# da03/torch-Attention-OCR

Hardware: AMD Instinct MI355X
Metric: image-lines/sec (train step) (higher is better)
Workload: dtype bf16; 1 GPU; c3: 32x256 crops, batch 256/GPU, VGG-7 + BiLSTM(256) + 2-layer attn decoder, L=24; global_batch=256, per_gpu_batch=256, img=32x256, decoder_steps=24, parallelism=dp1, input_feed=True

## Files before the change

torch-attention-ocr_amd/csrc/capi.hip:

```cpp
#include <cmath>
#include <cstdarg>
#include <cstdio>
#include <cstring>
#include <new>
#include <string>
#include "model.h"

using namespace aocr;

static thread_local std::string g_err;
static int fail(const char* fmt, ...) {
  char buf[512]; va_list ap; va_start(ap, fmt); vsnprintf(buf, sizeof buf, fmt, ap); va_end(ap);
  g_err = buf; return 1;
}
static int check_launch(const char* what) {
  hipError_t e = hipGetLastError();
  if (e != hipSuccess) return fail("%s: %s", what, hipGetErrorString(e));
  return 0;
}
#define REQUIRE(cond, ...) do { if (!(cond)) return fail(__VA_ARGS__); } while (0)

static int check_cfg(const aocr_config* c) {
  REQUIRE(c, "config is NULL");
  REQUIRE(c->batch_size >= 1 && c->img_h >= 32 && c->img_h % 16 == 0, "bad batch_size/img_h");
// ... 269 lines not shown
  REQUIRE(m, "NULL model");
  REQUIRE(bucket >= 0 && bucket < AOCR_GRAD_BUCKETS, "bucket %d outside 0..%d", bucket, AOCR_GRAD_BUCKETS - 1);
  REQUIRE(m->last_valid, "no train step has been enqueued yet");
  if (hipStreamWaitEvent((hipStream_t)stream, m->grad_ev[bucket], 0) != hipSuccess) return fail("hipStreamWaitEvent failed");
  return 0;
}

int aocr_sgd_step(aocr_model* m, float lr, float clip, float* norms_dev) {
  REQUIRE(m, "NULL model");
  prof_mark(m, AOCR_PROF_SGD);
  sgd_clip_update(m->s, m->params, m->grads, m->layout.group_off, lr, clip, norms_dev, m->sgd_scratch, m->cl_err, m->bn_snap ? m->bn_state : nullptr, m->bn_snap, (int)aocr_bn_state_count());
  prof_mark(m, -1);
  return check_launch("aocr_sgd_step");
}

int aocr_adadelta_step(aocr_model* m, float rho, float eps, float weight_decay, float* state_dev) {
  REQUIRE(m && state_dev, "NULL argument");
  REQUIRE(rho >= 0.f && rho < 1.f && eps > 0.f, "rho=%g eps=%g out of range", rho, eps);
  const int64_t n = m->layout.group_off[AOCR_NUM_GROUPS];
  adadelta_update(m->s, m->params, m->grads, state_dev, state_dev + n, n, rho, eps, weight_decay, m->cl_err, m->bn_snap ? m->bn_state : nullptr, m->bn_snap, (int)aocr_bn_state_count());
  return check_launch("aocr_adadelta_step");
}

int aocr_forward_logits(aocr_model* m, const float* images_dev, const int32_t* targets_dev, const int32_t* targets_eval_dev,
                        int32_t B, int32_t W, int32_t L, int32_t training, float* logits_dev, float* loss_dev) {
  Dims d; if (step_dims(m, B, W, L, d)) return 1;
  REQUIRE(images_dev && targets_dev, "NULL input");
  m->tab_valid = false;
  cnn_forward(m, images_dev, d, training, 0);
  encoder_forward(m, d);
  decoder_tf_forward(m, d, targets_dev, 1, L, false);
  if (targets_eval_dev) loss_and_dlogits(m, d, targets_eval_dev, 1, L, 0.f, false, loss_dev);
  if (logits_dev) copy2d(m->s, m->logits, LOGIT_LD, logits_dev, m->V, L * B, m->V);
  m->last = d; m->last_valid = 1; m->last_train = false;
  return check_launch("aocr_forward_logits");
}

__global__ void pad_targets_kernel(const int32_t* src, int32_t* dst, int B, int L, int Lt) {
  int i = blockIdx.x * blockDim.x + threadIdx.x;
  if (i >= B * Lt) return;
  int b = i / Lt, t = i - b * Lt;
  dst[i] = t < L ? src[b * L + t] : 1;
}

int aocr_decode(aocr_model* m, const float* images_dev, const int32_t* targets_dev, const int32_t* targets_eval_dev, int32_t B,
                int32_t W, int32_t L, int32_t beam, int32_t* labels_dev, float* scores_dev, float* gold_scores_dev, float* loss_dev) {
  return aocr_decode_dict(m, images_dev, targets_dev, targets_eval_dev, B, W, L, beam, nullptr, labels_dev, scores_dev, gold_scores_dev,
                          loss_dev);
}
static int check_trie(const aocr_trie* t, int V) {
  REQUIRE(t->child_mask_dev && t->child_base_dev && (t->child_dev || t->n_edges == 0), "trie: NULL array");
  REQUIRE(t->n_nodes >= 1 && t->n_edges >= 0, "trie: n_nodes=%d n_edges=%d", t->n_nodes, t->n_edges);
  REQUIRE(V <= 64, "dictionary decoding needs target_vocab_size <= 64 (got %d)", V);
  return 0;
}
int aocr_decode_dict(aocr_model* m, const float* images_dev, const int32_t* targets_dev, const int32_t* targets_eval_dev, int32_t B,
                     int32_t W, int32_t L, int32_t beam, const aocr_trie* trie, int32_t* labels_dev, float* scores_dev,
                     float* gold_scores_dev, float* loss_dev) {
  Dims d; if (step_dims(m, B, W, L, d)) return 1;
  REQUIRE(images_dev && targets_dev && targets_eval_dev && labels_dev && scores_dev, "NULL argument");
  if (trie && check_trie(trie, m->V)) return 1;
  if (beam > m->V) beam = m->V;
  REQUIRE(beam >= 1 && beam <= m->cfg.max_beam, "beam=%d outside 1..%d", beam, m->cfg.max_beam);
  const int Lt = m->cfg.max_decoder_l;
  hipLaunchKernelGGL(pad_targets_kernel, dim3(cdiv((int64_t)B * Lt, 256)), dim3(256), 0, m->s, targets_dev, m->tgt_pad, B, L, Lt);
  hipLaunchKernelGGL(pad_targets_kernel, dim3(cdiv((int64_t)B * Lt, 256)), dim3(256), 0, m->s, targets_eval_dev, m->tge_pad, B, L, Lt);
  d.L = Lt;
  prof_mark(m, AOCR_PROF_OTHER);
  m->tab_valid = false;
  cnn_forward(m, images_dev, d, 0, 0);
  encoder_forward(m, d);
  prof_mark(m, AOCR_PROF_DECODE);
  decode_beam(m, d, m->tgt_pad, beam, labels_dev, scores_dev, trie);
  d.L = L < Lt ? L : Lt;
  decoder_tf_forward(m, d, m->tgt_pad, 1, Lt, false);
  prof_mark(m, AOCR_PROF_OTHER);
  loss_and_dlogits(m, d, m->tge_pad, 1, Lt, 0.f, false, loss_dev);
  if (gold_scores_dev) gold_scores(m->s, m->nll_rows, gold_scores_dev, d.L, B);
  prof_mark(m, -1);
  m->last = d; m->last_valid = 1; m->last_train = false; m->tab_valid = false;
  return check_launch(trie ? "aocr_decode_dict" : "aocr_decode");
}

int aocr_recognize(aocr_model* m, const float* images_dev, int32_t B, int32_t W, int32_t beam, const aocr_trie* trie, int32_t* labels_dev,
                   float* scores_dev, float* char_logp_dev, float* attn_dev) {
  REQUIRE(m, "NULL model");
  const int Lt = m->cfg.max_decoder_l;
  Dims d; if (step_dims(m, B, W, Lt, d)) return 1;
  REQUIRE(images_dev && labels_dev && scores_dev, "NULL argument");
  if (trie && check_trie(trie, m->V)) return 1;
  if (beam > m->V) beam = m->V;
  REQUIRE(beam >= 1 && beam <= m->cfg.max_beam, "beam=%d outside 1..%d", beam, m->cfg.max_beam);
  const bool hist = char_logp_dev || attn_dev;
  fill_i32(m->s, m->tgt_pad, 2, (int64_t)B * Lt);
  prof_mark(m, AOCR_PROF_OTHER);
  m->tab_valid = false;
  cnn_forward(m, images_dev, d, 0, 0);
  encoder_forward(m, d);
  prof_mark(m, AOCR_PROF_DECODE);
  decode_beam(m, d, m->tgt_pad, beam, labels_dev, scores_dev, trie, hist ? m->attn_hist : nullptr, hist ? m->sc_hist : nullptr);
  if (hist) {
    const bool greedy = beam == 1;
    recognize_gather(m->s, labels_dev, greedy ? nullptr : m->hist_par, greedy ? nullptr : m->beam_scores, m->sc_hist, m->attn_hist, char_logp_dev,
                     attn_dev, Lt, B, beam, d.T);
  }
  prof_mark(m, -1);
  m->ctxa_fresh = false;
  m->last = d; m->last_valid = 1; m->last_train = false; m->tab_valid = false;
  return check_launch("aocr_recognize");
}

int aocr_get_tensor(aocr_model* m, const char* name, const void** ptr_dev, int32_t* ndim, int64_t shape[4]) {
  REQUIRE(m && name && ptr_dev && ndim && shape, "NULL argument");
  REQUIRE(m->last_valid, "no step has run yet");
  const Dims& d = m->last; std::string n = name;
  for (int i = 0; i < 4; ++i) shape[i] = 1;
  if (n == "feats") { *ptr_dev = m->X; *ndim = 3; shape[0] = d.T; shape[1] = d.B; shape[2] = 512; }
  else if (n == "dfeats") { *ptr_dev = m->dX; *ndim = 3; shape[0] = d.T; shape[1] = d.B; shape[2] = 512; }
  else if (n == "context") { *ptr_dev = m->context; *ndim = 3; shape[0] = d.B; shape[1] = d.T; shape[2] = m->Hd; }
  else if (n == "dcontext") { *ptr_dev = m->dctx; *ndim = 3; shape[0] = d.B; shape[1] = d.T; shape[2] = m->Hd; }
  else if (n == "logits") { *ptr_dev = m->logits; *ndim = 3; shape[0] = d.L; shape[1] = d.B; shape[2] = LOGIT_LD; }
  else if (n == "dlogits") { *ptr_dev = m->dlogits; *ndim = 3; shape[0] = d.L; shape[1] = d.B; shape[2] = LOGIT_LD; }
  else if (n == "dout_proj") { *ptr_dev = m->dout_proj; *ndim = 3; shape[0] = d.L; shape[1] = d.B; shape[2] = m->Hd; }
  else if (n == "outs") { *ptr_dev = m->out_all + (size_t)d.B * m->Hd; *ndim = 3; shape[0] = d.L; shape[1] = d.B; shape[2] = m->Hd; }
  else if (n == "conv1") { if (m->bf16) bf16_to_f32(m->s, m->A1b, m->A1, (int64_t)d.B * d.H1 * d.W1 * 64); *ptr_dev = m->A1; *ndim = 4; shape[0] = d.B; shape[1] = d.H1; shape[2] = d.W1; shape[3] = 64; }
  else if (n == "conv2") { if (m->bf16) bf16_to_f32(m->s, m->A2b, m->A2, (int64_t)d.B * d.H2 * d.W2 * 128); *ptr_dev = m->A2; *ndim = 4; shape[0] = d.B; shape[1] = d.H2; shape[2] = d.W2; shape[3] = 128; }
  else if (n == "conv6") { if (m->bf16) bf16_to_f32(m->s, m->A6b, m->A6, (int64_t)d.B * d.H6 * d.W2 * 512); *ptr_dev = m->A6; *ndim = 4; shape[0] = d.B; shape[1] = d.H6; shape[2] = d.W2; shape[3] = 512; }
  else if (n == "conv3") { if (m->bf16) bf16_to_f32(m->s, m->A3b, m->A3, (int64_t)d.B * d.H2 * d.W2 * 256); *ptr_dev = m->A3; *ndim = 4; shape[0] = d.B; shape[1] = d.H2; shape[2] = d.W2; shape[3] = 256; }
  else if (n == "conv4") { if (m->bf16) bf16_to_f32(m->s, m->A4b, m->A4, (int64_t)d.B * d.H4 * d.W2 * 256); *ptr_dev = m->A4; *ndim = 4; shape[0] = d.B; shape[1] = d.H4; shape[2] = d.W2; shape[3] = 256; }
  else if (n == "conv5") { if (m->bf16) bf16_to_f32(m->s, m->A5b, m->A5, (int64_t)d.B * d.H4 * d.W2 * 512); *ptr_dev = m->A5; *ndim = 4; shape[0] = d.B; shape[1] = d.H4; shape[2] = d.W2; shape[3] = 512; }
  else if (n == "idx2") { u8_to_f32(m->s, m->idx2, m->G0, (int64_t)d.B * d.H2 * d.W2 * 128); *ptr_dev = m->G0; *ndim = 4; shape[0] = d.B; shape[1] = d.H2; shape[2] = d.W2; shape[3] = 128; }
  else if (n == "idx4") { u8_to_f32(m->s, m->idx4, m->G0, (int64_t)d.B * d.H4 * d.W2 * 256); *ptr_dev = m->G0; *ndim = 4; shape[0] = d.B; shape[1] = d.H4; shape[2] = d.W2; shape[3] = 256; }
  else if (n == "idx6") { u8_to_f32(m->s, m->idx6, m->G0, (int64_t)d.B * d.H6 * d.W2 * 512); *ptr_dev = m->G0; *ndim = 4; shape[0] = d.B; shape[1] = d.H6; shape[2] = d.W2; shape[3] = 512; }
  else if (n == "enc_dz0" || n == "enc_dz1") {
    const int dir = n == "enc_dz1"; const int64_t cnt = (int64_t)d.T * d.B * 4 * m->He;
    REQUIRE(m->edz_b[dir][m->Le - 1], "no bf16 d z in this mode");
    bf16_to_f32(m->s, m->edz_b[dir][m->Le - 1], m->G0, cnt);
    *ptr_dev = m->G0; *ndim = 3; shape[0] = d.T; shape[1] = d.B; shape[2] = 4 * m->He;
  }
  else if (n == "enc_cs0") { *ptr_dev = m->ecs[0][m->Le - 1]; *ndim = 3; shape[0] = d.T + 2; shape[1] = d.B; shape[2] = m->He; }
  else if (n == "enc_gates0") { *ptr_dev = m->egates[0][m->Le - 1]; *ndim = 3; shape[0] = d.T; shape[1] = d.B; shape[2] = 4 * m->He; }
  else if (n == "cl_err") { *ptr_dev = m->cl_err; *ndim = 1; shape[0] = 8; REQUIRE(m->cl_err, "no cluster kernels in this configuration"); }
  else if (n == "dc_stamps") { REQUIRE(m->dc_xtab, "no decoder cluster kernel in this configuration"); *ptr_dev = m->dc_xtab + (size_t)((d.B + 31) / 32) * 32; *ndim = 1; shape[0] = 32; }
  else if (n == "ds_all") { *ptr_dev = m->ds_all; *ndim = 3; shape[0] = d.L; shape[1] = d.B; shape[2] = d.T; }
  else if (n == "dq_all") { *ptr_dev = m->dq_all; *ndim = 3; shape[0] = d.L; shape[1] = d.B; shape[2] = m->Hd; }
  else if (n == "dcat_all") { *ptr_dev = m->dcat_all; *ndim = 3; shape[0] = d.L; shape[1] = d.B; shape[2] = 2 * m->Hd; }
  else if (n == "dh_rec0" || n == "dh_rec1" || n == "dc_st0" || n == "dc_st1" || n == "dfeed0") {
    const int l = n.back() - '0'; *ptr_dev = n[1] == 'f' ? m->dfeed : (n[1] == 'h' ? m->dh_rec[l] : m->dc_st[l]); *ndim = 2; shape[0] = d.B; shape[1] = m->Hd; }
  else if (n == "dpre_all") { *ptr_dev = m->dpre_all; *ndim = 3; shape[0] = d.L; shape[1] = d.B; shape[2] = m->Hd; }
  else if (n == "dc_bstamps") { REQUIRE(m->dc_xtab, "no decoder cluster kernel in this configuration"); *ptr_dev = m->dc_xtab + (size_t)((d.B + 31) / 32) * 32 + 16; *ndim = 1; shape[0] = 32; }
  else if (n == "dc_times") { REQUIRE(m->cl_err, "no cluster kernels in this configuration"); *ptr_dev = m->cl_err + 16 + 2048; *ndim = 1; shape[0] = 32 * 4 * 16 * 2; }
  else if (n == "g0") {
    const char* e = getenv("AOCR_DBG_STOP"); const int stop = e ? atoi(e) : 0;
    const int64_t cnt = stop == 1 ? (int64_t)d.B * d.T * 512 : (int64_t)d.B * d.H4 * d.W2 * 512;
    if (m->bf16) bf16_to_f32(m->s, m->G0b, m->G0, cnt);
    *ptr_dev = m->G0; *ndim = 4; shape[0] = d.B; shape[1] = stop == 1 ? d.Ho7 : d.H4; shape[2] = stop == 1 ? d.Wo7 : d.W2; shape[3] = 512;
  }
  else return fail("unknown tensor '%s'", name);
  return 0;
}

int aocr_profile_kernel(aocr_model* m, int32_t which, int32_t iters, float* ms_per_launch, double* flops_per_launch) {
  REQUIRE(m && ms_per_launch && flops_per_launch, "NULL argument");
  REQUIRE(m->last_valid, "run a step first");
  REQUIRE(which >= 0 && which <= AOCR_PK_LAST, "unknown kernel id %d", which);
  REQUIRE(iters >= 1, "iters must be >= 1");
  REQUIRE(which < 2 || (m->bf16 && m->last_images && m->last_train), "the HBM-bound kernel ids replay the bf16 TRAINING step: run aocr_train_forward_backward in bf16 mode first");
  const Dims& d = m->last;
  const int64_t n5 = (int64_t)d.B * d.H4 * d.W2;
  REQUIRE((which != 1 && which != AOCR_PK_SPLITK) || (size_t)512 * 4608 <= m->gmax, "kernel id %d sums conv6's filter gradient (512 x 4608 floats) into the gradient-map scratch, which holds %zu floats in this configuration", which, m->gmax);
  REQUIRE((which != AOCR_PK_BN_FWD && which != AOCR_PK_BN_BWD && which != AOCR_PK_UNPOOL) || (n5 % 256 == 0 && n5 / 256 <= 512), "kernel id %d replays conv5's BatchNorm with the epilogue's 256-pixel statistics chunks: %lld pixels are not a multiple of 256 / more than 512 chunks", which, (long long)n5);
  hipEvent_t e0, e1; hipEventCreate(&e0); hipEventCreate(&e1);
  hipStream_t s = m->s; const int B = d.B;
  constexpr size_t SLAB = (size_t)4 << 20;
  double bytes = 0.0;
  const char* const nd = getenv("AOCR_DX16");
  const bool dx16 = (nd && nd[0] == '1') && !getenv("AOCR_BN_PARTIAL_OLD") && !getenv("AOCR_UNPOOL4") && !getenv("AOCR_HALO8") && B * d.H4 * d.W2 % 256 == 0;
  const bf16_t* const g1h = dx16 ? reinterpret_cast<const bf16_t*>(m->G1) : nullptr;
  const double dab = dx16 ? 2.0 : 4.0;
  auto run = [&]() {
    switch (which) {
    case 0:
      if (const char* const pl = getenv("AOCR_PROBE_LAYER")) {
        int bnc = 0, y16 = 0; const int l = atoi(pl);
        if (l == 3) { conv_forward(m->s, m->bf16, m->A2, m->conv[3].w, m->conv[3].b, m->Y3, nullptr, d.B, d.H2, d.W2, 128, 256, 3, 1, 0, 0, m->A2b, m->wb[3], nullptr, 1, nullptr, nullptr, nullptr, (double*)m->bn_scratch, &bnc, &y16); break; }
        if (l == 4) { conv_forward(m->s, m->bf16, m->A3, m->conv[4].w, m->conv[4].b, nullptr, m->idx4, d.B, d.H2, d.W2, 256, 256, 3, 1, 1, 2, m->A3b, m->wb[4], m->A4b, 1); break; }
        if (l == 5) { conv_forward(m->s, m->bf16, m->A4, m->conv[5].w, m->conv[5].b, m->Y5, nullptr, d.B, d.H4, d.W2, 256, 512, 3, 1, 0, 0, m->A4b, m->wb[5], nullptr, 1, nullptr, nullptr, nullptr, (double*)m->bn_scratch, &bnc, &y16); break; }
      }
      conv_forward(m->s, m->bf16, m->A5, m->conv[6].w, m->conv[6].b, m->bf16 ? nullptr : m->A6, m->idx6, d.B, d.H4, d.W2, 512, 512, 3, 1, 1, 2, m->A5b, m->wb[6],
                   m->A6b, 1);
      break;
    case 1:
      conv_backward_filter(m->s, m->bf16, m->A5, m->G0, m->G1, nullptr, d.B, d.H4, d.W2, 512, 512, 3, 1, m->A5b, m->G0b, m->wg_part, m->wg_part_floats, 1);
      break;
    case AOCR_PK_CONV1_FWD:
      conv1_forward(s, m->last_images, m->conv[1].w, m->conv[1].b, nullptr, B, d.H, d.W, m->A1b, m->route1_valid ? m->route1 : nullptr);
      bytes = (double)B * d.H * d.W * 4 + (double)B * d.H1 * d.W1 * 64 * 2 + (m->route1_valid ? (double)conv1_route_elems(B, d.H, d.W) * 2 : 0.0);
      break;
    case AOCR_PK_CONV1_BWD:
      conv1_backward(s, m->last_images, m->conv[1].w, m->conv[1].b, m->G1, m->conv[1].dw, m->conv[1].db, B, d.H, d.W,
                     (size_t)B * d.H1 * d.W1 * 128 >= (size_t)4096 * 640 ? m->G0 + 6 * SLAB : nullptr, nullptr, m->route1_valid ? m->route1 : nullptr);
      bytes = (double)B * d.H * d.W * 4 + (double)B * d.H1 * d.W1 * 64 * 4 + (m->route1_valid ? (double)conv1_route_elems(B, d.H, d.W) * 2 : 0.0);
      break;
    case AOCR_PK_BN_FWD:
      bn_relu_forward(s, m->Y5, nullptr, m->bn[5].w, m->bn[5].b, m->bn[5].rm, m->bn[5].rv, m->bn[5].save, m->bn_scratch, n5, 512, 1, 0, 0, m->A5b, nullptr, (int)(n5 / 256));
      bytes = (double)n5 * 512 * (4 + 2);
      break;
    case AOCR_PK_BN_BWD:
      bn_relu_backward(s, m->Y5, m->A5, m->G1, m->bn[5].w, m->bn[5].save, nullptr, m->bn[5].dw, m->bn[5].db, m->bn_scratch, n5, 512, 0, m->G0b, m->A5b,
                       m->conv[5].db, m->G0 + 2 * SLAB, nullptr, nullptr, nullptr, g1h);
      bytes = (double)n5 * 512 * ((4 + dab + 2) + (4 + dab + 2 + 2));
      break;
    case AOCR_PK_UNPOOL:
      unpool_relu_backward(s, m->G1, m->A6, m->idx6, nullptr, B, d.H4, d.W2, 512, 2, m->G0b, m->conv[6].db, m->G0 + 1 * SLAB, m->A6b, nullptr, g1h);
      bytes = (double)B * d.H6 * d.W2 * 512 * (dab + 1 + 2) + (double)n5 * 512 * 2;
      break;
    case AOCR_PK_ATTN_DCTX:
      attention_dctx(s, m->a_all, m->ds_all, m->dcat_all, 2 * m->Hd, m->q_all, m->dctx, d.L, B, d.T, m->Hd);
      bytes = (double)d.L * B * (2.0 * d.T + 2.0 * m->Hd) * 4 + (double)B * d.T * m->Hd * 4;
      break;
    case AOCR_PK_SPLITK:
      {
        const int ksl = (int)std::min<size_t>(8, m->wg_part_floats / ((size_t)512 * 4608));
        if (ksl >= 1) splitk_reduce(s, m->wg_part, ksl, (size_t)512 * 4608, m->G1);
        bytes = (double)512 * 4608 * 4 * (ksl + 2);
      }
      break;
    }
  };
  run();
  hipEventRecord(e0, m->s);
  for (int i = 0; i < iters; ++i) run();
  hipEventRecord(e1, m->s);
  hipEventSynchronize(e1);
  float ms = 0.f; hipEventElapsedTime(&ms, e0, e1);
  hipEventDestroy(e0); hipEventDestroy(e1);
  *ms_per_launch = ms / iters;
  if (which == 0 && getenv("AOCR_PROBE")) {
    unsigned long long pr[8] = {0}; kprobe_read(pr);
    if (getenv("AOCR_PROBE_LAYER")) for (int k = 1; k >= 0; --k) if (pr[4 * k + 1]) fprintf(stderr, "[aocr] probe: workgroup %d of the tagged launch: start -> K loop %.1f us, K loop %.1f us (%llu cycles = %.2f GHz), whole workgroup (last store acknowledged) %.1f us\n", k ? 17 : 300, pr[4 * k + 2] / 100.0, pr[4 * k + 1] / 100.0, pr[4 * k], pr[4 * k] / (pr[4 * k + 1] * 10.0) , pr[4 * k + 3] / 100.0);
    for (int k = 0; k < 2; ++k) if (pr[4 * k + 1]) fprintf(stderr, "[aocr] probe (%s halo kernel, conv6 forward): K loop of one workgroup %llu shader cycles in %.1f us = %.2f GHz\n", k ? "4-wave" : "8-wave", pr[4 * k], pr[4 * k + 1] / 100.0, pr[4 * k] / (pr[4 * k + 1] * 10.0)), fprintf(stderr, "[aocr]   prologue %.1f us, whole workgroup %.1f us (stores acknowledged)\n", pr[4 * k + 2] / 100.0, pr[4 * k + 3] / 100.0);
  }
  *flops_per_launch = which < 2 ? 2.0 * (double)d.B * d.H4 * d.W2 * 512.0 * (9.0 * 512.0) : bytes;
  return check_launch("aocr_profile_kernel");
}

int aocr_gemm(void* stream, int32_t compute, const float* A_dev, int64_t lda, int32_t a_kmajor, const float* B_dev, int64_t ldb,
              int32_t b_kmajor, float* C_dev, int64_t ldc, int32_t M, int32_t N, int32_t K, const float* bias_dev, int32_t accumulate) {
  REQUIRE(A_dev && B_dev && C_dev && M >= 0 && N >= 0 && K >= 0, "bad gemm arguments");
  REQUIRE((accumulate & ~7) == 0, "unknown gemm flag bits %d", accumulate);
  const int fl = ((accumulate & AOCR_GEMM_ACCUMULATE) ? EP_ACCUM : 0) | ((accumulate & AOCR_GEMM_RELU) ? EP_RELU : 0) | ((accumulate & AOCR_GEMM_TANH) ? EP_TANH : 0);
  REQUIRE(!((fl & EP_ACCUM) && (fl & (EP_RELU | EP_TANH))), "an activation on an accumulating product is not a module of the path");
  int rc = gemm((hipStream_t)stream, compute == AOCR_COMPUTE_BF16, A_dev, lda, a_kmajor != 0, B_dev, ldb, b_kmajor != 0, C_dev, ldc,
                M, N, K, bias_dev, nullptr, fl);
  REQUIRE(rc == 0, "gemm: the (A column-major, B row-major-by-K) combination is not supported");
  return check_launch("aocr_gemm");
}
int aocr_pointwise(void* stream, int32_t op, const float* a_dev, const float* b_dev, float* y_dev, int64_t n) {
  REQUIRE(a_dev && y_dev && n >= 0 && op >= 0 && op <= 3 && (b_dev || op == AOCR_PW_RELU), "bad arguments");
  pointwise((hipStream_t)stream, op, a_dev, b_dev, y_dev, n);
  return check_launch("aocr_pointwise");
}
int aocr_lookup_forward(void* stream, const float* weight_dev, const int32_t* ids_dev, float* out_dev, int32_t n, int32_t E) {
  REQUIRE(weight_dev && ids_dev && out_dev && n >= 0 && E > 0, "bad arguments");
  embedding_gather((hipStream_t)stream, weight_dev, ids_dev, 0, 1, out_dev, 1, n, E);
  return check_launch("aocr_lookup_forward");
}
int aocr_lookup_backward(void* stream, const float* grad_out_dev, const int32_t* ids_dev, float* grad_weight_dev, int32_t n, int32_t E, int32_t V) {
  REQUIRE(grad_out_dev && ids_dev && grad_weight_dev && n >= 0 && E > 0 && E <= 256 && V > 0, "bad arguments");
  embedding_scatter_accum((hipStream_t)stream, grad_out_dev, ids_dev, 0, 1, grad_weight_dev, 1, n, E, V);
  return check_launch("aocr_lookup_backward");
}
int aocr_conv2d_forward(void* stream, int32_t compute, const float* x_dev, const float* w_dev, const float* bias_dev, float* y_dev,
                        uint8_t* idx_dev, int32_t B, int32_t H, int32_t W, int32_t Cin, int32_t Cout, int32_t ksize, int32_t pad,
                        int32_t relu, int32_t pool) {
  REQUIRE(x_dev && w_dev && y_dev, "NULL argument");
  REQUIRE(Cin % 16 == 0 && Cout % 16 == 0, "Cin and Cout must be multiples of 16 (the 1-channel first layer has its own entry point)");
  REQUIRE(pool >= 0 && pool <= 2 && (pool == 0 || idx_dev), "bad pool mode / missing idx");
  conv_forward((hipStream_t)stream, compute == AOCR_COMPUTE_BF16, x_dev, w_dev, bias_dev, y_dev, idx_dev, B, H, W, Cin, Cout, ksize, pad,
               relu, pool);
  return check_launch("aocr_conv2d_forward");
}
int aocr_conv2d_backward_data(void* stream, int32_t compute, const float* dy_dev, const float* w_dev, float* dx_dev, int32_t B, int32_t H,
                              int32_t W, int32_t Cin, int32_t Cout, int32_t ksize, int32_t pad) {
  REQUIRE(dy_dev && w_dev && dx_dev && Cin % 16 == 0 && Cout % 16 == 0, "bad arguments");
  conv_backward_data((hipStream_t)stream, compute == AOCR_COMPUTE_BF16, dy_dev, w_dev, dx_dev, B, H, W, Cin, Cout, ksize, pad);
  return check_launch("aocr_conv2d_backward_data");
}
int aocr_conv2d_backward_filter(void* stream, int32_t compute, const float* x_dev, const float* dy_dev, float* dw_dev, float* dbias_dev,
                                int32_t B, int32_t H, int32_t W, int32_t Cin, int32_t Cout, int32_t ksize, int32_t pad) {
  REQUIRE(x_dev && dy_dev && dw_dev && Cin % 16 == 0 && Cout % 16 == 0, "bad arguments");
  conv_backward_filter((hipStream_t)stream, compute == AOCR_COMPUTE_BF16, x_dev, dy_dev, dw_dev, dbias_dev, B, H, W, Cin, Cout, ksize, pad);
  return check_launch("aocr_conv2d_backward_filter");
}
int aocr_unpool_relu_backward(void* stream, const float* dpooled_dev, const float* pooled_dev, const uint8_t* idx_dev, float* dy_dev,
                              int32_t B, int32_t Ho, int32_t Wo, int32_t C, int32_t pool) {
  REQUIRE(dpooled_dev && pooled_dev && idx_dev && dy_dev && (pool == 1 || pool == 2) && C % 4 == 0, "bad arguments");
  unpool_relu_backward((hipStream_t)stream, dpooled_dev, pooled_dev, idx_dev, dy_dev, B, Ho, Wo, C, pool);
  return check_launch("aocr_unpool_relu_backward");
}
int aocr_conv1_forward(void* stream, const float* x_dev, const float* w_dev, const float* bias_dev, float* y_dev, int32_t B, int32_t H,
                       int32_t W) {
  REQUIRE(x_dev && w_dev && bias_dev && y_dev, "NULL argument");
  conv1_forward((hipStream_t)stream, x_dev, w_dev, bias_dev, y_dev, B, H, W);
  return check_launch("aocr_conv1_forward");
}
int aocr_conv1_backward(void* stream, const float* x_dev, const float* w_dev, const float* bias_dev, const float* dy_pooled_dev,
                        float* dw_dev, float* dbias_dev, int32_t B, int32_t H, int32_t W) {
  REQUIRE(x_dev && w_dev && bias_dev && dy_pooled_dev && dw_dev && dbias_dev, "NULL argument");
// ... 160 lines not shown
```

torch-attention-ocr_amd/csrc/epilogues.h:

```cpp
#pragma once
#include "mfma_gemm.h"

namespace aocr {

enum : int { EP_RELU = 1, EP_TANH = 2, EP_ACCUM = 4, EP_ATOMIC = 8 };

__device__ __forceinline__ float fast_exp_(float x) { return __builtin_amdgcn_exp2f(x * 1.44269504088896341f); }
__device__ __forceinline__ float sigmoidf_(float x) { return __builtin_amdgcn_rcpf(1.f + fast_exp_(-x)); }
__device__ __forceinline__ float tanhf_(float x) {
  const float ax = fminf(fabsf(x), 15.f);
  const float e = fast_exp_(2.f * ax);
  const float t = 1.f - 2.f * __builtin_amdgcn_rcpf(e + 1.f);
  return copysignf(t, x);
}

__host__ __device__ __forceinline__ unsigned long long splitmix64_(unsigned long long x) {
  x += 0x9E3779B97F4A7C15ull;
  unsigned long long z = x;
  z = (z ^ (z >> 30)) * 0xBF58476D1CE4E5B9ull;
  z = (z ^ (z >> 27)) * 0x94D049BB133111EBull;
  return z ^ (z >> 31);
}
struct DropSpec {
  unsigned long long base = 0, thr = 0; float scale = 1.f; long long off = 0;
  __device__ __forceinline__ bool on() const { return thr != 0; }
  __device__ __forceinline__ float mask(long long idx) const { return ((splitmix64_(base + (unsigned long long)(off + idx)) >> 11) >= thr) ? scale : 0.f; }
};

struct EpStore {
  float* C; int64_t ldc; int M, N;
  const float* bias; const float* bias2;
  int flags;
  float* C1; int64_t ldc1; int N0;
  bf16_t* Cb = nullptr; int64_t ldcb = 0;
  const float* dg = nullptr; const float* dout = nullptr; int64_t ldd = 0;
  const float* bnb_x = nullptr; const bf16_t* bnb_yb = nullptr; const float* bnb_save = nullptr; double* bnb_part = nullptr;
  template <int NT> __device__ __forceinline__ void quad(int m, int n, int nstep, const float (&v)[NT][4]) const {
#pragma unroll
    for (int ni = 0; ni < NT; ++ni) {
      int col = n + nstep * ni;
      if (col >= N) continue;
      float bb = 0.f;
      if (bias) bb = bias[col];
      if (bias2) bb += bias2[col];
      float* base; int64_t ld; int cc;
      if (C1 && col >= N0) { base = C1; ld = ldc1; cc = col - N0; } else { base = C; ld = ldc; cc = col; }
#pragma unroll
      for (int i = 0; i < 4; ++i) {
        int row = m + i;
        if (row >= M) continue;
        float x = v[ni][i] + bb;
        if (flags & EP_RELU) x = fmaxf(x, 0.f);
        if (flags & EP_TANH) x = tanhf_(x);
        if (dg) { const float o = dout[(int64_t)row * ldd + col]; x = (x + dg[(int64_t)row * ldd + col]) * (1.f - o * o); }
        float* p = base + (int64_t)row * ld + cc;
        if (flags & EP_ATOMIC) atomicAdd(p, x);
        else if (flags & EP_ACCUM) *p += x;
        else { *p = x; if (Cb && base == C) Cb[(int64_t)row * ldcb + cc] = (bf16_t)x; }
      }
    }
  }
  struct Pre { float dg, dout, b, b2, old; };
  __device__ __forceinline__ Pre prefetch(int row, int n) const {
    Pre p; p.dg = p.dout = p.b = p.b2 = p.old = 0.f;
    const int rr = max(min(row, M - 1), 0), col = min(n, N - 1);
    if (bias) p.b = bias[col];
    if (bias2) p.b2 = bias2[col];
    if (dg) { p.dg = dg[(int64_t)rr * ldd + col]; p.dout = dout[(int64_t)rr * ldd + col]; }
    if (flags & EP_ACCUM) p.old = *((C1 && col >= N0) ? C1 + (int64_t)rr * ldc1 + (col - N0) : C + (int64_t)rr * ldc + col);
    return p;
  }
  __device__ __forceinline__ void prefetch_zx(Pre&, int, int) const {}
  static constexpr bool kCell4 = false; struct Pre4 {};
  __device__ __forceinline__ bool cell4_ok() const { return false; }
  template <int NT> __device__ __forceinline__ void elem(int row, int n, int nstep, const float (&v)[NT], const Pre& pre) const {
    if (row >= M) return;
    if constexpr (NT == 1) {
      const int col = n;
      if (col >= N) return;
      float x = v[0];
      if (bias) x += pre.b;
      if (bias2) x += pre.b2;
      if (flags & EP_RELU) x = fmaxf(x, 0.f);
      if (flags & EP_TANH) x = tanhf_(x);
      if (dg) x = (x + pre.dg) * (1.f - pre.dout * pre.dout);
      float* p = (C1 && col >= N0) ? C1 + (int64_t)row * ldc1 + (col - N0) : C + (int64_t)row * ldc + col;
      if (flags & EP_ATOMIC) atomicAdd(p, x);
      else if (flags & EP_ACCUM) *p = pre.old + x;
      else { *p = x; if (Cb && !(C1 && col >= N0)) Cb[(int64_t)row * ldcb + col] = (bf16_t)x; }
      return;
    }
#pragma unroll
    for (int ni = 0; ni < NT; ++ni) {
      int col = n + nstep * ni;
      if (col >= N) continue;
      float x = v[ni];
      if (bias) x += bias[col];
      if (bias2) x += bias2[col];
      if (flags & EP_RELU) x = fmaxf(x, 0.f);
      if (flags & EP_TANH) x = tanhf_(x);
      if (dg) { const float o = dout[(int64_t)row * ldd + col]; x = (x + dg[(int64_t)row * ldd + col]) * (1.f - o * o); }
      float* p = (C1 && col >= N0) ? C1 + (int64_t)row * ldc1 + (col - N0) : C + (int64_t)row * ldc + col;
      if (flags & EP_ATOMIC) atomicAdd(p, x);
      else if (flags & EP_ACCUM) *p += x;
      else { *p = x; if (Cb && !(C1 && col >= N0)) Cb[(int64_t)row * ldcb + col] = (bf16_t)x; }
    }
  }
};

template <int NT, class EPT>
__device__ __forceinline__ bool narrow_store_staged(const EPT& ep, const f32x16 (&acc)[2][NT], unsigned char* lds, int m_blk, int n_blk, int wm, int wn, int r, int h, int tid) {
  constexpr int BN = 64 * NT, PITCH = BN * 4;
  if ((ep.flags & (EP_ATOMIC | EP_ACCUM)) || ep.C1 || ep.dg || n_blk + BN > ep.N) return false;
  float bb[NT];
#pragma unroll
  for (int ni = 0; ni < NT; ++ni) { const int col = n_blk + wn * 32 * NT + ni * 32 + r; bb[ni] = (ep.bias ? ep.bias[col] : 0.f) + (ep.bias2 ? ep.bias2[col] : 0.f); }
  __syncthreads();
  for (int p = 0; p < 2; ++p) {
    if ((wm >> 1) == p) {
#pragma unroll
      for (int mi = 0; mi < 2; ++mi)
#pragma unroll
        for (int ni = 0; ni < NT; ++ni)
#pragma unroll
          for (int q = 0; q < 4; ++q)
#pragma unroll
            for (int i = 0; i < 4; ++i) {
              float x = acc[mi][ni][4 * q + i] + bb[ni];
              if (ep.flags & EP_RELU) x = fmaxf(x, 0.f);
              if (ep.flags & EP_TANH) x = tanhf_(x);
              *reinterpret_cast<float*>(lds + ((wm & 1) * 64 + mi * 32 + 8 * q + 4 * h + i) * PITCH + (wn * 32 * NT + ni * 32 + r) * 4) = x;
            }
    }
    __syncthreads();
    const int row_base = m_blk + p * 128;
#pragma unroll 4
    for (int it = 0; it < (128 * BN / 4) / 512; ++it) {
      const int idx = it * 512 + tid, row = idx / (BN / 4), c = idx % (BN / 4);
      if (row_base + row < ep.M) {
        const float4 v = *reinterpret_cast<const float4*>(lds + row * PITCH + c * 16);
        if (ep.C) *reinterpret_cast<float4*>(ep.C + (int64_t)(row_base + row) * ep.ldc + n_blk + c * 4) = v;
        if (ep.Cb) {
          typedef __bf16 bf16x4_ __attribute__((ext_vector_type(4)));
          bf16x4_ o; o[0] = (__bf16)v.x; o[1] = (__bf16)v.y; o[2] = (__bf16)v.z; o[3] = (__bf16)v.w;
          *reinterpret_cast<bf16x4_*>(ep.Cb + (int64_t)(row_base + row) * ep.ldcb + n_blk + c * 4) = o;
        }
      }
    }
    __syncthreads();
  }
  return true;
}

struct EpConv {
  float* y; uint8_t* idx; const float* bias; int Cout; int rows; int pmode; int relu;
  bf16_t* yb;
  const float* bn_save = nullptr; const float* bn_w = nullptr; const float* bn_b = nullptr;
  double* bn_part = nullptr;
  bf16_t* y16 = nullptr;
  template <int NT> __device__ __forceinline__ void quad(int m, int n, int nstep, const float (&v)[NT][4]) const {
#pragma unroll
    for (int ni = 0; ni < NT; ++ni) {
      int col = n + nstep * ni;
      if (col >= Cout) continue;
      float bb = bias ? bias[col] : 0.f;
      float x[4];
#pragma unroll
      for (int i = 0; i < 4; ++i) { x[i] = v[ni][i] + bb; if (relu) x[i] = fmaxf(x[i], 0.f); }
      if (bn_save) {
        const float mu = bn_save[col], iv = bn_save[Cout + col], ww = bn_w[col], b2 = bn_b[col];
#pragma unroll
        for (int i = 0; i < 4; ++i) x[i] = fmaxf((x[i] - mu) * iv * ww + b2, 0.f);
      }
      if (pmode == 0) {
#pragma unroll
        for (int i = 0; i < 4; ++i) if (m + i < rows) {
          if (y) y[(int64_t)(m + i) * Cout + col] = x[i];
          if (yb) yb[(int64_t)(m + i) * Cout + col] = (bf16_t)x[i];
        }
      } else if (pmode == 1) {
        if (m < rows) {
          float best = x[0]; int bi = 0;
#pragma unroll
          for (int i = 1; i < 4; ++i) if (x[i] > best) { best = x[i]; bi = i; }
          int64_t o = (int64_t)(m >> 2) * Cout + col;
          if (y) y[o] = best;
          if (idx) idx[o] = (uint8_t)bi; if (yb) yb[o] = (bf16_t)best;
        }
      } else {
#pragma unroll
        for (int w = 0; w < 2; ++w) {
          int row = m + 2 * w;
          if (row < rows) {
            float a = x[2 * w], b = x[2 * w + 1];
            int64_t o = (int64_t)(row >> 1) * Cout + col;
            if (y) y[o] = (b > a) ? b : a;
            if (idx) idx[o] = (uint8_t)(b > a); if (yb) yb[o] = (bf16_t)((b > a) ? b : a);
          }
        }
      }
    }
  }
};

struct EpGatesFwd {
  const float* zx; int64_t ldzx;
  const float* b1; const float* b2;
  const float* c_prev; int64_t ldcp;
  float* c_out; int64_t ldc;
  float* h_out; int64_t ldh;
  float* h_out2; int64_t ldh2;
  float* gates; int64_t ldg;
  int M, H;
  bf16_t* hb = nullptr; int64_t ldhb = 0;
  bf16_t* hb2 = nullptr; int64_t ldhb2 = 0;
  const int32_t* zx_tok = nullptr; int64_t zx_tok_stride = 1;
  DropSpec drop;
  __device__ __forceinline__ int64_t zrow(int row) const { return zx_tok ? (int64_t)(zx_tok[(int64_t)row * zx_tok_stride] - 1) : (int64_t)row; }
  template <int NT> __device__ __forceinline__ void quad(int m, int j, int, const float (&v)[NT][4]) const {
    static_assert(NT == 4, "gate epilogue needs the 4 gate tiles");
    if (j >= H) return;
    float bb[4] = {0.f, 0.f, 0.f, 0.f};
    if (b1) {
#pragma unroll
      for (int g = 0; g < 4; ++g) bb[g] = b1[g * H + j] + b2[g * H + j];
    }
#pragma unroll
    for (int i = 0; i < 4; ++i) {
      int row = m + i;
      if (row >= M) continue;
      float z[4];
#pragma unroll
      for (int g = 0; g < 4; ++g) {
        z[g] = v[g][i] + bb[g];
        if (zx) z[g] += zx[zrow(row) * ldzx + g * H + j];
      }
      float ig = sigmoidf_(z[0]), fg = sigmoidf_(z[1]), og = sigmoidf_(z[2]), gg = tanhf_(z[3]);
      float c = fg * c_prev[(int64_t)row * ldcp + j] + ig * gg;
      float hh = og * tanhf_(c);
      c_out[(int64_t)row * ldc + j] = c;
      h_out[(int64_t)row * ldh + j] = hh;
      const float hh2 = drop.on() ? hh * drop.mask((long long)row * H + j) : hh;
      if (h_out2) h_out2[(int64_t)row * ldh2 + j] = hh2;
      if (hb) hb[(int64_t)row * ldhb + j] = (bf16_t)hh;
      if (hb2) hb2[(int64_t)row * ldhb2 + j] = (bf16_t)hh2;
      if (gates) {
        float* gp = gates + (int64_t)row * ldg + j;
        gp[0] = ig; gp[H] = fg; gp[2 * H] = og; gp[3 * H] = gg;
      }
    }
  }
  struct Pre { float zx[4]; float b1[4]; float b2[4]; float cp; int32_t tok; };
  __device__ __forceinline__ Pre prefetch(int row, int j) const {
    Pre p;
    const int rr = max(min(row, M - 1), 0), jj = min(j, H - 1);
    const float* const cpp = c_prev + (int64_t)rr * ldcp + jj;
    const int32_t* const tp = zx_tok ? zx_tok + (int64_t)rr * zx_tok_stride : reinterpret_cast<const int32_t*>(cpp);
    p.tok = *tp;
    const float* const b1p = b1 ? b1 + jj : cpp; const float* const b2p = b1 ? b2 + jj : cpp; const int bs = b1 ? H : 0;
#pragma unroll
    for (int g = 0; g < 4; ++g) { p.b1[g] = b1p[g * bs]; p.b2[g] = b2p[g * bs]; }
    p.cp = *cpp;
    return p;
  }
  __device__ __forceinline__ void prefetch_zx(Pre& p, int row, int j) const {
    const int rr = max(min(row, M - 1), 0), jj = min(j, H - 1);
    const float* const cpp = c_prev + (int64_t)rr * ldcp + jj;
    const int64_t zr = zx_tok ? (int64_t)(p.tok - 1) : (int64_t)rr;
    const float* const zp = zx ? zx + zr * ldzx + jj : cpp; const int zs = zx ? H : 0;
#pragma unroll
    for (int g = 0; g < 4; ++g) p.zx[g] = zp[g * zs];
  }
  template <int NT> __device__ __forceinline__ void elem(int row, int j, int, const float (&v)[NT], const Pre& pre) const {
    static_assert(NT == 4, "gate epilogue needs the 4 gate tiles");
    if (j >= H || row >= M) return;
    float z[4];
#pragma unroll
    for (int g = 0; g < 4; ++g) {
      float zin = 0.f;
      if (b1) zin = pre.b1[g] + pre.b2[g];
      if (zx) zin += pre.zx[g];
      z[g] = v[g] + zin;
    }
    float ig = sigmoidf_(z[0]), fg = sigmoidf_(z[1]), og = sigmoidf_(z[2]), gg = tanhf_(z[3]);
    float c = fg * pre.cp + ig * gg;
    float hh = og * tanhf_(c);
    c_out[(int64_t)row * ldc + j] = c;
    h_out[(int64_t)row * ldh + j] = hh;
    const float hh2 = drop.on() ? hh * drop.mask((long long)row * H + j) : hh;
    if (h_out2) h_out2[(int64_t)row * ldh2 + j] = hh2;
    if (hb) hb[(int64_t)row * ldhb + j] = (bf16_t)hh;
    if (hb2) hb2[(int64_t)row * ldhb2 + j] = (bf16_t)hh2;
    if (gates) {
      float* gp = gates + (int64_t)row * ldg + j;
      gp[0] = ig; gp[H] = fg; gp[2 * H] = og; gp[3 * H] = gg;
    }
  }
  static constexpr bool kCell4 = true;
  typedef float v4f __attribute__((ext_vector_type(4)));
  typedef bf16_t v4h __attribute__((ext_vector_type(4)));
  struct Pre4 { v4f zx[4]; v4f b1[4]; v4f b2[4]; v4f cp; int32_t tok; };
  __device__ __forceinline__ bool cell4_ok() const {
// ... 146 lines not shown
```

torch-attention-ocr_amd/csrc/mfma_gemm.h:

```cpp
#pragma once
#include <hip/hip_runtime.h>
#include <stdint.h>
#include <type_traits>
#include <utility>

namespace aocr {

typedef float f32x16 __attribute__((ext_vector_type(16)));
typedef float f32x4 __attribute__((ext_vector_type(4)));
typedef __bf16 bf16x8 __attribute__((ext_vector_type(8)));

template <int NV> struct Frag { float v[NV]; };

template <bool BF16> struct Mode {
  static constexpr int NV = BF16 ? 8 : 4;
  static constexpr int CHUNK = BF16 ? 16 : 8;
};


struct LoadK {
  const float* p0; int64_t ld0; int K0;
  const float* p1; int64_t ld1;
  int rows; int K; int vec;
  struct Ctx { const float* b0; const float* b1; bool ok; };
// ... 776 lines not shown
#pragma unroll
      for (int i = 0; i < NI; ++i) bf[set][i] = *reinterpret_cast<const float4*>(lb + i * 32 * PITCH + 32 * c);
    };
    rd(0, 0);
#pragma unroll
    for (int c = 0; c < 4; ++c) {
      if (c < 3) rd((c + 1) & 1, c + 1);
#pragma unroll
      for (int s = 0; s < 4; ++s)
#pragma unroll
        for (int mi = 0; mi < MI; ++mi)
#pragma unroll
          for (int ni = 0; ni < NI; ++ni) {
            const float4& A = af[c & 1][mi]; const float4& B = bf[c & 1][ni];
            const float x = s == 0 ? A.x : s == 1 ? A.y : s == 2 ? A.z : A.w;
            const float y = s == 0 ? B.x : s == 1 ? B.y : s == 2 ? B.z : B.w;
            acc[mi][ni] = __builtin_amdgcn_mfma_f32_32x32x2f32(x, y, acc[mi][ni], 0, 0, 0);
          }
    }
    if (kt + 1 < nk) { sa.store(&lds[buf ^ 1][0]); sb.store(&lds[buf ^ 1][BM * PITCH]); }
    __syncthreads();
  }
  const int m0 = m_blk + wm * (BM / 2), n0 = n_blk + wn * (BN / 2);
#pragma unroll
  for (int mi = 0; mi < MI; ++mi)
#pragma unroll
    for (int q = 0; q < 4; ++q) {
      float v[NI][4];
#pragma unroll
      for (int ni = 0; ni < NI; ++ni)
#pragma unroll
        for (int i = 0; i < 4; ++i) v[ni][i] = acc[mi][ni][4 * q + i];
      ep.template quad<NI>(m0 + 32 * mi + 8 * q + 4 * h, n0 + r, 32, v);
    }
}
constexpr int F32W_PITCH = 136 * 4;
template <class LD> struct StagerW;
template <> struct StagerW<LoadMN> {
  const float* pk; int64_t ld8; bool mok; int k; f32x4 reg[4]; bool ok[4];
  __device__ __forceinline__ void init(const LoadMN& l, int mbase, int tid, int kbeg) {
    const int m = mbase + 4 * (tid & 31); mok = m + 3 < l.rows; k = kbeg + (tid >> 5);
    pk = l.p + (mok ? m : 0) + (int64_t)k * l.ld; ld8 = 8 * l.ld;
  }
  __device__ __forceinline__ void load(const LoadMN& l) {
    const float* q = pk;
#pragma unroll
    for (int i = 0; i < 4; ++i) {
      ok[i] = mok && k + 8 * i < l.K;
      reg[i] = *reinterpret_cast<const f32x4*>(ok[i] ? q : l.p);
      q += ld8;
    }
    pk = q; k += 32;
  }
};
template <> struct StagerW<LoadConvXcol> {
  LoadConvXcol::Ctx4 c; int px, py, k, linc, cbase, dxc, dyc; f32x4 reg[4]; bool ok[4];
  __device__ __forceinline__ void init(const LoadConvXcol& l, int nbase, int tid, int kbeg) {
    c = l.row4(nbase + 4 * (tid & 31)); k = kbeg + (tid >> 5);
    px = k % l.Wo; const int t = k / l.Wo; py = t % l.Ho; const int b = t / l.Ho;
    linc = ((b * l.H + py) * l.W + px) * l.Cin; cbase = ((c.kh - l.pad) * l.W + (c.kw - l.pad)) * l.Cin + c.ci;
    dxc = (l.W - l.Wo) * l.Cin; dyc = (l.H - l.Ho) * l.W * l.Cin;
  }
  __device__ __forceinline__ void load(const LoadConvXcol& l) {
#pragma unroll
    for (int i = 0; i < 4; ++i) {
      const int sy = py + c.kh - l.pad, sx = px + c.kw - l.pad;
      ok[i] = c.ok && k < l.K && (unsigned)sy < (unsigned)l.H && (unsigned)sx < (unsigned)l.W;
      reg[i] = *reinterpret_cast<const f32x4*>(l.x + (ok[i] ? linc + cbase : 0));
      k += 8; px += 8; linc += 8 * l.Cin;
      const bool wx = px >= l.Wo; px -= wx ? l.Wo : 0; py += wx ? 1 : 0; linc += wx ? dxc : 0;
      const bool wy = py >= l.Ho; py = wy ? 0 : py; linc += wy ? dyc : 0;
    }
  }
};
template <class ST> __device__ __forceinline__ void stagerw_store(const ST& st, unsigned char* tile, int tid) {
  const f32x4 z = {0.f, 0.f, 0.f, 0.f};
#pragma unroll
  for (int i = 0; i < 4; ++i) *reinterpret_cast<f32x4*>(tile + ((tid >> 5) + 8 * i) * F32W_PITCH + (tid & 31) * 16) = st.ok[i] ? st.reg[i] : z;
}
template <class AL, class BL, class EP>
__global__ __launch_bounds__(256, 2) void gemm_f32w_kernel(AL a, BL b, EP ep, int K, int kper, int gx, int gy) {
  constexpr int PK = F32W_PITCH, OPB = 32 * PK;
  __shared__ __attribute__((aligned(16))) unsigned char lds[2][2 * OPB];
  const int nwg = gx * gy, orig = blockIdx.x;
  const int q8 = nwg >> 3, r8 = nwg & 7, xcd = orig & 7;
  const int bid = (xcd < r8 ? xcd * (q8 + 1) : r8 * (q8 + 1) + (xcd - r8) * q8) + (orig >> 3);
  const int m_blk = (bid / gx) * 128, n_blk = (bid % gx) * 128;
  const int kbeg = blockIdx.z * kper, kend = min(K, kbeg + kper);
  const int tid = threadIdx.x, lane = tid & 63, wave = tid >> 6;
  const int r = lane & 31, h = lane >> 5;
  const int wm = wave >> 1, wn = wave & 1;
  const int nk = (kend - kbeg + 31) / 32;
  StagerW<AL> sa; StagerW<BL> sb;
  sa.init(a, m_blk, tid, kbeg); sb.init(b, n_blk, tid, kbeg);
  f32x16 acc[2][2];
#pragma unroll
  for (int i = 0; i < 2; ++i)
#pragma unroll
    for (int j = 0; j < 2; ++j)
#pragma unroll
      for (int e = 0; e < 16; ++e) acc[i][j][e] = 0.f;
  if (nk > 0) { sa.load(a); sb.load(b); stagerw_store(sa, &lds[0][0], tid); stagerw_store(sb, &lds[0][OPB], tid); }
  __syncthreads();
  for (int kt = 0; kt < nk; ++kt) {
    const int buf = kt & 1;
    if (kt + 1 < nk) { sa.load(a); sb.load(b); }
    const unsigned char* la = &lds[buf][h * PK + (wm * 64 + r) * 4];
    const unsigned char* lb = &lds[buf][OPB + h * PK + (wn * 64 + r) * 4];
#pragma unroll
    for (int j = 0; j < 16; ++j) {
      float av[2], bv[2];
#pragma unroll
      for (int i = 0; i < 2; ++i) { av[i] = *reinterpret_cast<const float*>(la + 2 * j * PK + i * 128); bv[i] = *reinterpret_cast<const float*>(lb + 2 * j * PK + i * 128); }
#pragma unroll
      for (int mi = 0; mi < 2; ++mi)
#pragma unroll
        for (int ni = 0; ni < 2; ++ni) acc[mi][ni] = __builtin_amdgcn_mfma_f32_32x32x2f32(av[mi], bv[ni], acc[mi][ni], 0, 0, 0);
    }
    if (kt + 1 < nk) { stagerw_store(sa, &lds[buf ^ 1][0], tid); stagerw_store(sb, &lds[buf ^ 1][OPB], tid); }
    __syncthreads();
  }
  const int m0 = m_blk + wm * 64, n0 = n_blk + wn * 64;
#pragma unroll
  for (int mi = 0; mi < 2; ++mi)
#pragma unroll
    for (int q = 0; q < 4; ++q) {
      float v[2][4];
#pragma unroll
      for (int ni = 0; ni < 2; ++ni)
#pragma unroll
        for (int i = 0; i < 4; ++i) v[ni][i] = acc[mi][ni][4 * q + i];
      ep.template quad<2>(m0 + 32 * mi + 8 * q + 4 * h, n0 + r, 32, v);
    }
}
template <class L> struct HasStagerW { static constexpr bool v = false; };
template <> struct HasStagerW<LoadMN> { static constexpr bool v = true; };
template <> struct HasStagerW<LoadConvXcol> { static constexpr bool v = true; };

template <class L> struct HasPtr8 { static constexpr bool v = false; };
template <> struct HasPtr8<LoadK> { static constexpr bool v = true; };
template <> struct HasPtr8<LoadConvK> { static constexpr bool v = true; };

template <class AL, class BL, class EP, int BK = 32>
__global__ __launch_bounds__(256, (SrcBf16<AL>::v && SrcBf16<BL>::v) ? 4 : 1)
void gemm_lds_bf16_kernel(AL a, BL b, EP ep, int K, int kper, int gx, int gy) {
  __shared__ __attribute__((aligned(16))) unsigned char lds[2][2][128 * (BK * 2 + 16)];
  const int nwg = gx * gy, orig = blockIdx.x;
  const int q8 = nwg >> 3, r8 = nwg & 7, xcd = orig & 7;
  const int bid = (xcd < r8 ? xcd * (q8 + 1) : r8 * (q8 + 1) + (xcd - r8) * q8) + (orig >> 3);
  const int kbeg = blockIdx.z * kper;
  lds_tile<BK>(a, b, ep, (bid / gx) * 128, (bid % gx) * 128, kbeg, min(K, kbeg + kper), lds);
}

struct EpConv; struct EpStore;
template <int NI, int NTH>
__device__ __forceinline__ void tile256_store_f32(float* dst, int64_t ldc, const float* bias, bool relu, const f32x16 (&acc)[4][NI], unsigned char* lds,
                                                  int m_blk, int n_blk, int wm, int wn, int r, int h, int tid, double* part = nullptr, int C = 0, const float* bias2 = nullptr,
                                                  const float* bnb_x = nullptr, const bf16_t* bnb_yb = nullptr, const float* bnb_save = nullptr) {
  constexpr int PITCH = 1024;
  float bmean[4] = {0.f, 0.f, 0.f, 0.f}, binv[4] = {0.f, 0.f, 0.f, 0.f};
  if (bnb_x) {
    const float4 m4 = *reinterpret_cast<const float4*>(bnb_save + n_blk + (tid & 63) * 4), i4 = *reinterpret_cast<const float4*>(bnb_save + C + n_blk + (tid & 63) * 4);
    bmean[0] = m4.x; bmean[1] = m4.y; bmean[2] = m4.z; bmean[3] = m4.w; binv[0] = i4.x; binv[1] = i4.y; binv[2] = i4.z; binv[3] = i4.w;
  }
  float bb[NI];
#pragma unroll
  for (int ni = 0; ni < NI; ++ni) bb[ni] = (bias ? bias[n_blk + wn * 32 * NI + ni * 32 + r] : 0.f) + (bias2 ? bias2[n_blk + wn * 32 * NI + ni * 32 + r] : 0.f);
  float ps[8] = {0.f, 0.f, 0.f, 0.f, 0.f, 0.f, 0.f, 0.f};
  __syncthreads();
  for (int p = 0; p < 2; ++p) {
    if (wm == p) {
#pragma unroll
      for (int mi = 0; mi < 4; ++mi)
#pragma unroll
        for (int ni = 0; ni < NI; ++ni)
#pragma unroll
          for (int q = 0; q < 4; ++q)
#pragma unroll
            for (int i = 0; i < 4; ++i) {
              float x = acc[mi][ni][4 * q + i] + bb[ni];
              if (relu) x = fmaxf(x, 0.f);
              *reinterpret_cast<float*>(lds + (mi * 32 + 8 * q + 4 * h + i) * PITCH + (wn * 32 * NI + ni * 32 + r) * 4) = x;
            }
    }
    __syncthreads();
    float* const d0 = dst + (int64_t)(m_blk + p * 128) * ldc + n_blk;
#pragma unroll 4
    for (int it = 0; it < 8192 / NTH; ++it) {
      const int idx = it * NTH + tid, row = idx >> 6, c = idx & 63;
      const float4 v = *reinterpret_cast<const float4*>(lds + row * PITCH + c * 16);
      *reinterpret_cast<float4*>(d0 + (int64_t)row * ldc + c * 4) = v;
      if (part && bnb_x) {
        const int64_t gofs = (int64_t)(m_blk + p * 128 + row) * C + n_blk + c * 4;
        const float4 x4 = *reinterpret_cast<const float4*>(bnb_x + gofs);
        typedef __bf16 bf16x4_ __attribute__((ext_vector_type(4)));
        const bf16x4_ y4 = *reinterpret_cast<const bf16x4_*>(bnb_yb + gofs);
        const float dv[4] = {(float)y4[0] > 0.f ? v.x : 0.f, (float)y4[1] > 0.f ? v.y : 0.f, (float)y4[2] > 0.f ? v.z : 0.f, (float)y4[3] > 0.f ? v.w : 0.f};
        const float xs[4] = {x4.x, x4.y, x4.z, x4.w};
#pragma unroll
        for (int k = 0; k < 4; ++k) { ps[k] += dv[k]; ps[4 + k] = fmaf(dv[k], (xs[k] - bmean[k]) * binv[k], ps[4 + k]); }
      } else if (part) {
        ps[0] += v.x; ps[1] += v.y; ps[2] += v.z; ps[3] += v.w;
        ps[4] = fmaf(v.x, v.x, ps[4]); ps[5] = fmaf(v.y, v.y, ps[5]); ps[6] = fmaf(v.z, v.z, ps[6]); ps[7] = fmaf(v.w, v.w, ps[7]);
      }
    }
    __syncthreads();
  }
  if (part) {
    float* const red = reinterpret_cast<float*>(lds);
#pragma unroll
    for (int k = 0; k < 8; ++k) red[((tid >> 6) * 64 + (tid & 63)) * 8 + k] = ps[k];
    __syncthreads();
    if (tid < 64) {
      double S[8] = {0, 0, 0, 0, 0, 0, 0, 0};
      for (int g = 0; g < NTH / 64; ++g)
#pragma unroll
        for (int k = 0; k < 8; ++k) S[k] += (double)red[(g * 64 + tid) * 8 + k];
      double* o = part + ((int64_t)(m_blk >> 8) * C + n_blk + tid * 4) * 2;
#pragma unroll
      for (int j = 0; j < 4; ++j) { o[2 * j] = S[j]; o[2 * j + 1] = S[4 + j]; }
    }
  }
}
template <int NI, int NTH>
__device__ __forceinline__ void tile256_store_pooled(bf16_t* yb, uint8_t* idxp, int Cout, const float* bias, bool relu, const f32x16 (&acc)[4][NI], unsigned char* lds,
                                                     int m_blk, int n_blk, int wm, int wn, int r, int h, int tid) {
  constexpr int PB = 528, PI = 272, IOFF = 128 * PB;
  float bb[NI];
#pragma unroll
  for (int ni = 0; ni < NI; ++ni) bb[ni] = bias ? bias[n_blk + wn * 32 * NI + ni * 32 + r] : 0.f;
  __syncthreads();
#pragma unroll
  for (int mi = 0; mi < 4; ++mi)
#pragma unroll
    for (int ni = 0; ni < NI; ++ni)
#pragma unroll
      for (int q = 0; q < 4; ++q) {
        float x[4];
#pragma unroll
        for (int i = 0; i < 4; ++i) { x[i] = acc[mi][ni][4 * q + i] + bb[ni]; if (relu) x[i] = fmaxf(x[i], 0.f); }
#pragma unroll
        for (int w = 0; w < 2; ++w) {
          const float a_ = x[2 * w], b_ = x[2 * w + 1];
          const int prow = wm * 64 + mi * 16 + 4 * q + 2 * h + w, col = wn * 32 * NI + ni * 32 + r;
          *reinterpret_cast<bf16_t*>(lds + prow * PB + col * 2) = (bf16_t)((b_ > a_) ? b_ : a_);
          *reinterpret_cast<uint8_t*>(lds + IOFF + prow * PI + col) = (uint8_t)(b_ > a_);
        }
      }
  __syncthreads();
  const int64_t prow0 = m_blk >> 1;
#pragma unroll 4
  for (int it = 0; it < 4096 / NTH; ++it) {
    const int idx = it * NTH + tid, row = idx >> 5, c = idx & 31;
    const uint4 v = *reinterpret_cast<const uint4*>(lds + row * PB + c * 16);
    *reinterpret_cast<uint4*>(yb + (prow0 + row) * Cout + n_blk + c * 8) = v;
  }
#pragma unroll 4
  for (int it = 0; it < 2048 / NTH; ++it) {
    const int idx = it * NTH + tid, row = idx >> 4, c = idx & 15;
    const uint4 v = *reinterpret_cast<const uint4*>(lds + IOFF + row * PI + c * 16);
    *reinterpret_cast<uint4*>(idxp + (prow0 + row) * Cout + n_blk + c * 16) = v;
  }
}
template <int NI, int NTH>
__device__ __forceinline__ void tile256_store_bf16(bf16_t* yb, int Cout, const float* bias, bool relu, const float* bn_save, const float* bn_w, const float* bn_b,
                                                   const f32x16 (&acc)[4][NI], unsigned char* lds, int m_blk, int n_blk, int wm, int wn, int r, int h, int tid, double* part = nullptr) {
  float bb[NI], mu[NI], iv[NI], ww[NI], b2[NI];
#pragma unroll
  for (int ni = 0; ni < NI; ++ni) {
    const int col = n_blk + wn * 32 * NI + ni * 32 + r;
    bb[ni] = bias ? bias[col] : 0.f;
    mu[ni] = bn_save ? bn_save[col] : 0.f; iv[ni] = bn_save ? bn_save[Cout + col] : 1.f; ww[ni] = bn_save ? bn_w[col] : 1.f; b2[ni] = bn_save ? bn_b[col] : 0.f;
  }
  float ps[NI], pss[NI];
#pragma unroll
  for (int ni = 0; ni < NI; ++ni) { ps[ni] = 0.f; pss[ni] = 0.f; }
  __syncthreads();
#pragma unroll
  for (int mi = 0; mi < 4; ++mi)
#pragma unroll
    for (int ni = 0; ni < NI; ++ni)
#pragma unroll
      for (int q = 0; q < 4; ++q)
#pragma unroll
        for (int i = 0; i < 4; ++i) {
          float x = acc[mi][ni][4 * q + i] + bb[ni];
          if (relu) x = fmaxf(x, 0.f);
          if (bn_save) x = fmaxf((x - mu[ni]) * iv[ni] * ww[ni] + b2[ni], 0.f);
          ps[ni] += x; pss[ni] = fmaf(x, x, pss[ni]);
          *reinterpret_cast<bf16_t*>(lds + (wm * 128 + mi * 32 + 8 * q + 4 * h + i) * 512 + (wn * 32 * NI + ni * 32 + r) * 2) = (bf16_t)x;
        }
  __syncthreads();
#pragma unroll 4
  for (int it = 0; it < 8192 / NTH; ++it) {
    const int idx = it * NTH + tid, row = idx >> 5, c = idx & 31;
    const uint4 v = *reinterpret_cast<const uint4*>(lds + row * 512 + c * 16);
    *reinterpret_cast<uint4*>(yb + (int64_t)(m_blk + row) * Cout + n_blk + c * 8) = v;
  }
  if (part) {
    __syncthreads();
    float* const red = reinterpret_cast<float*>(lds);
#pragma unroll
    for (int ni = 0; ni < NI; ++ni) {
      float* o = red + (((wm * 2 + h) * 256) + wn * 32 * NI + ni * 32 + r) * 2;
      o[0] = ps[ni]; o[1] = pss[ni];
    }
    __syncthreads();
    if (tid < 256) {
      double S = 0.0, SS = 0.0;
#pragma unroll
      for (int g = 0; g < 4; ++g) { S += (double)red[((g * 256) + tid) * 2]; SS += (double)red[((g * 256) + tid) * 2 + 1]; }
      double* o = part + ((int64_t)(m_blk >> 8) * Cout + n_blk + tid) * 2;
      o[0] = S; o[1] = SS;
    }
  }
}
template <int NI, int NTH, class EP>
__device__ __forceinline__ bool tile256_store_staged(const EP& ep, const f32x16 (&acc)[4][NI], unsigned char* lds, int m_blk, int n_blk, int wm, int wn, int r, int h, int tid, int opt) {
  if constexpr (std::is_same<EP, EpConv>::value) {
    if (m_blk + 256 > ep.rows || n_blk + 256 > ep.Cout) return false;
    if (ep.pmode == 0 && ep.y16 && ep.bn_part && !ep.yb && !ep.bn_save && (opt & 2)) {
      tile256_store_bf16<NI, NTH>(ep.y16, ep.Cout, ep.bias, ep.relu != 0, nullptr, nullptr, nullptr, acc, lds, m_blk, n_blk, wm, wn, r, h, tid, ep.bn_part); return true; }
    if (ep.pmode == 0 && ep.yb && !ep.y && (opt & 2)) { tile256_store_bf16<NI, NTH>(ep.yb, ep.Cout, ep.bias, ep.relu != 0, ep.bn_save, ep.bn_w, ep.bn_b, acc, lds, m_blk, n_blk, wm, wn, r, h, tid); return true; }
    if (ep.bn_save) return false;
    if (ep.pmode == 2 && ep.yb && ep.idx && !ep.y && (opt & 4)) { tile256_store_pooled<NI, NTH>(ep.yb, ep.idx, ep.Cout, ep.bias, ep.relu != 0, acc, lds, m_blk, n_blk, wm, wn, r, h, tid); return true; }
    if (ep.pmode == 0 && ep.y && !ep.yb && (opt & 2)) { tile256_store_f32<NI, NTH>(ep.y, ep.Cout, ep.bias, ep.relu != 0, acc, lds, m_blk, n_blk, wm, wn, r, h, tid, ep.bn_part, ep.Cout); return true; }
    return false;
  } else if constexpr (std::is_same<EP, EpStore>::value) {
    if (!ep.C && ep.Cb && !ep.flags && !ep.bias && !ep.bias2 && !ep.C1 && !ep.dg) {
      tile256_store_bf16<NI, NTH>(ep.Cb, (int)ep.ldcb, nullptr, false, nullptr, nullptr, nullptr, acc, lds, m_blk, n_blk, wm, wn, r, h, tid); return true; }
    if (ep.flags || ep.bias || ep.bias2 || ep.C1 || ep.Cb || ep.dg || !(opt & 1) || m_blk + 256 > ep.M || n_blk + 256 > ep.N) return false;
    if (ep.bnb_part) tile256_store_f32<NI, NTH>(ep.C, ep.ldc, nullptr, false, acc, lds, m_blk, n_blk, wm, wn, r, h, tid, ep.bnb_part, ep.N, nullptr, ep.bnb_x, ep.bnb_yb, ep.bnb_save);
    else tile256_store_f32<NI, NTH>(ep.C, ep.ldc, nullptr, false, acc, lds, m_blk, n_blk, wm, wn, r, h, tid);
    return true;
  } else return false;
}

template <int NT, class EPT>
__device__ __forceinline__ bool narrow_store_staged(const EPT& ep, const f32x16 (&acc)[2][NT], unsigned char* lds, int m_blk, int n_blk, int wm, int wn, int r, int h, int tid);

__device__ __forceinline__ void dma16(const void* g, unsigned char* l) {
  __builtin_amdgcn_global_load_lds((const __attribute__((address_space(1))) void*)g, (__attribute__((address_space(3))) void*)l, 16, 0, 0);
}

template <class AL, class BL, class EP, int ABL = 0, bool PIPE = false, bool PAIRS = false, int TAG = 0>
__global__ __launch_bounds__(512, 1)
void gemm_dma_bf16_kernel(AL a, BL b, EP ep, int K, int gx, int gy, const bf16_t* zero, int opt = 0) {
  __shared__ __attribute__((aligned(1024))) unsigned char lds[4 * 32768];
  const int nwg = gx * gy, orig = blockIdx.x;
  const int q8 = nwg >> 3, r8 = nwg & 7, xcd = orig & 7;
  const int bid = (xcd < r8 ? xcd * (q8 + 1) : r8 * (q8 + 1) + (xcd - r8) * q8) + (orig >> 3);
  const int m_blk = (bid / gx) * 256, n_blk = (bid % gx) * 256;
  const int tid = threadIdx.x, lane = tid & 63, wave = tid >> 6;
  const int r = lane & 31, h = lane >> 5, wm = wave >> 2, wn = wave & 3;

  const int srow = tid >> 2, chunk = (tid & 3) ^ ((tid >> 4) & 3);
  typename AL::DRow ra[2]; typename BL::DRow rb[2];
#pragma unroll
  for (int j = 0; j < 2; ++j) { ra[j] = a.drow(m_blk + 128 * j + srow, chunk); rb[j] = b.drow(n_blk + 128 * j + srow, chunk); }
  typename AL::DCur ca = a.dseek(0); typename BL::DCur cb = b.dseek(0);
  const int nk = K >> 5;
  unsigned char* const wbase = lds + __builtin_amdgcn_readfirstlane(wave) * 1024;
  int slot = 0;
  auto issue_a = [&]() {
#pragma unroll
    for (int j = 0; j < 2; ++j) if constexpr (!(ABL & 32)) dma16((ABL & 16) ? zero : a.dsrc(ra[j], ca, zero), wbase + slot * 32768 + j * 8192);
    a.dadvance(ca);
  };
  auto issue_b = [&]() {
#pragma unroll
    for (int j = 0; j < 2; ++j) dma16((ABL & 128) ? zero : b.dsrc(rb[j], cb, zero), wbase + slot * 32768 + 16384 + j * 8192);
    b.dadvance(cb); slot = (slot + 1) & 3;
  };

  f32x16 acc[4][2];
#pragma unroll
  for (int i = 0; i < 4; ++i)
#pragma unroll
    for (int j = 0; j < 2; ++j)
#pragma unroll
      for (int e = 0; e < 16; ++e) acc[i][j][e] = 0.f;

  const int swz = (r >> 2) & 3;
  unsigned aoff[2], boff[2];
#pragma unroll
  for (int s = 0; s < 2; ++s) {
    aoff[s] = (wm * 128 + r) * 64 + (((2 * s + h) ^ swz) << 4);
    boff[s] = 16384 + (wn * 64 + r) * 64 + (((2 * s + h) ^ swz) << 4);
  }

  const unsigned lbase = (unsigned)(uintptr_t)((__attribute__((address_space(3))) unsigned char*)lds);
  bf16x8 fa0[4], fb0[2], fa1[4], fb1[2];
#define AOCR_DSR(dst, addr, OFF) asm volatile("ds_read_b128 %0, %1 offset:" #OFF : "=v"(dst) : "v"(addr))
  auto read0 = [&](int sl) {
    const unsigned pa = lbase + sl * 32768 + aoff[0], pb = lbase + sl * 32768 + boff[0];
    AOCR_DSR(fa0[0], pa, 0); AOCR_DSR(fa0[1], pa, 2048); AOCR_DSR(fb0[0], pb, 0); AOCR_DSR(fb0[1], pb, 2048);
    AOCR_DSR(fa0[2], pa, 4096); AOCR_DSR(fa0[3], pa, 6144);
  };
  auto read1 = [&](int sl) {
    const unsigned pa = lbase + sl * 32768 + aoff[1], pb = lbase + sl * 32768 + boff[1];
    AOCR_DSR(fa1[0], pa, 0); AOCR_DSR(fa1[1], pa, 2048); AOCR_DSR(fb1[0], pb, 0); AOCR_DSR(fb1[1], pb, 2048);
    AOCR_DSR(fa1[2], pa, 4096); AOCR_DSR(fa1[3], pa, 6144);
  };
#undef AOCR_DSR
  if constexpr (!PIPE && PAIRS) {
    const int npairs = (nk + 1) >> 1;
    issue_a(); issue_b(); issue_a(); issue_b();
    for (int pr = 0; pr < npairs; ++pr) {
      asm volatile("s_waitcnt vmcnt(0)" ::: "memory");
      __builtin_amdgcn_s_barrier();
      if constexpr (!(ABL & 1)) { issue_a(); issue_b(); issue_a(); issue_b(); }
#pragma unroll
      for (int half = 0; half < 2; ++half) {
        const unsigned char* L = lds + (((pr & 1) << 1) + half) * 32768;
        bf16x8 af[2][4], bf[2][2];
#pragma unroll
        for (int s2 = 0; s2 < 2; ++s2) {
#pragma unroll
          for (int mi = 0; mi < 4; ++mi) af[s2][mi] = *reinterpret_cast<const bf16x8*>(L + aoff[s2] + mi * 2048);
#pragma unroll
          for (int ni = 0; ni < 2; ++ni) bf[s2][ni] = *reinterpret_cast<const bf16x8*>(L + boff[s2] + ni * 2048);
        }
#pragma unroll
        for (int s2 = 0; s2 < 2; ++s2)
#pragma unroll
          for (int mi = 0; mi < 4; ++mi)
#pragma unroll
            for (int ni = 0; ni < 2; ++ni)
              acc[mi][ni] = __builtin_amdgcn_mfma_f32_32x32x16_bf16(af[s2][mi], bf[s2][ni], acc[mi][ni], 0, 0, 0);
      }
    }
  } else if constexpr (!PIPE) {
#pragma unroll
    for (int t = 0; t < 3; ++t) { issue_a(); issue_b(); }
    for (int kt = 0; kt < nk; ++kt) {
      if constexpr (ABL & 32) asm volatile("s_waitcnt vmcnt(4)" ::: "memory"); else
      asm volatile("s_waitcnt vmcnt(8)" ::: "memory");
      __builtin_amdgcn_s_barrier();
      const unsigned char* L = lds + (kt & 3) * 32768;
      bf16x8 af[2][4], bf[2][2];
#pragma unroll
      for (int s2 = 0; s2 < 2; ++s2) {
#pragma unroll
        for (int mi = 0; mi < 4; ++mi) af[s2][mi] = *reinterpret_cast<const bf16x8*>(L + aoff[s2] + mi * 2048);
#pragma unroll
        for (int ni = 0; ni < 2; ++ni) bf[s2][ni] = *reinterpret_cast<const bf16x8*>(L + boff[s2] + ni * 2048);
      }
      if constexpr (!(ABL & 1)) issue_a();
      if constexpr (ABL & 8) __builtin_amdgcn_s_setprio(1);
#pragma unroll
      for (int mi = 0; mi < 4; ++mi)
#pragma unroll
        for (int ni = 0; ni < 2; ++ni)
          acc[mi][ni] = __builtin_amdgcn_mfma_f32_32x32x16_bf16(af[0][mi], bf[0][ni], acc[mi][ni], 0, 0, 0);
      if constexpr (ABL & 8) __builtin_amdgcn_s_setprio(0);
      if constexpr (!(ABL & 1)) issue_b();
      if constexpr (ABL & 8) __builtin_amdgcn_s_setprio(1);
#pragma unroll
      for (int mi = 0; mi < 4; ++mi)
#pragma unroll
        for (int ni = 0; ni < 2; ++ni)
          acc[mi][ni] = __builtin_amdgcn_mfma_f32_32x32x16_bf16(af[1][mi], bf[1][ni], acc[mi][ni], 0, 0, 0);
      if constexpr (ABL & 8) __builtin_amdgcn_s_setprio(0);
    }
  } else {
#pragma unroll
  for (int t = 0; t < 3; ++t) { issue_a(); issue_b(); }
  asm volatile("s_waitcnt vmcnt(8)" ::: "memory");
  __builtin_amdgcn_s_barrier();
  issue_a(); issue_b();
  read0(0);
  for (int kt = 0; kt < nk; ++kt) {
    if constexpr (!(ABL & 4)) read1(kt & 3);
    asm volatile("s_waitcnt lgkmcnt(6)" ::: "memory");
    __builtin_amdgcn_sched_barrier(0);
    if constexpr (!(ABL & 2)) {
#pragma unroll
      for (int mi = 0; mi < 4; ++mi)
#pragma unroll
        for (int ni = 0; ni < 2; ++ni)
          acc[mi][ni] = __builtin_amdgcn_mfma_f32_32x32x16_bf16(fa0[mi], fb0[ni], acc[mi][ni], 0, 0, 0);
    }
    __builtin_amdgcn_sched_barrier(0);
    asm volatile("s_waitcnt vmcnt(8) lgkmcnt(0)" ::: "memory");
    __builtin_amdgcn_s_barrier();
    __builtin_amdgcn_sched_barrier(0);
    if constexpr (!(ABL & 1)) issue_a();
    if constexpr (!(ABL & 4)) read0((kt + 1) & 3);
    if constexpr (!(ABL & 1)) issue_b();
    __builtin_amdgcn_sched_barrier(0);
    if constexpr (!(ABL & 2)) {
#pragma unroll
// ... 275 lines not shown
  unsigned long long pc0 = 0, pw0 = 0; if constexpr (TAG == 1) { pc0 = __builtin_readcyclecounter(); pw0 = wall_clock64(); }
  for (int chunk = 0; chunk < NC; ++chunk) {
    const unsigned hb = (chunk & 1) * HMAX, hbn = ((chunk + 1) & 1) * HMAX;
    const int chn = chunk + 1 < NC ? chunk + 1 : chunk;
    auto step_fn = [&](auto tapc) {
      constexpr int TAP = decltype(tapc)::value;
      constexpr int TN = (TAP + 1) % 9;
      constexpr int HT = TAP <= 4, HT1 = ((TAP + 8) % 9) <= 4, HT2 = ((TAP + 7) % 9) <= 4;
      constexpr int NVM = 6 + HT2 + 2 * HT1 + HT;
      const int step = chunk * 9 + TAP;
      constexpr int T3 = (TAP + 3) % 9, DC3 = (TAP + 3) / 9;
      const unsigned k3 = chunk + DC3 < NC ? (unsigned)(T3 * C + ((chunk + DC3) << 5)) * 2u : (unsigned)(8 * C + ((NC - 1) << 5)) * 2u;
      const unsigned bs1 = (unsigned)((step & 3) * BSLOT), bs0n = (unsigned)(((step + 1) & 3) * BSLOT);
      asm volatile("s_waitcnt lgkmcnt(0)" ::: "memory");
      AOCR_SB();
#pragma unroll
      for (int mi = 0; mi < 4; ++mi) {
#pragma unroll
        for (int ni = 0; ni < 4; ++ni) {
          acc[mi][ni] = __builtin_amdgcn_mfma_f32_32x32x16_bf16(a0[mi], b0[ni], acc[mi][ni], 0, 0, 0);
          AOCR_SB();
          if (ni == 0) AOCR_DSR(a1[mi], a_addr(mi, TAP, 1), 0);
          if (ni == 2) { if (mi == 0) AOCR_DSR(b1[0], boff[1] + bs1, 0); else if (mi == 1) AOCR_DSR(b1[1], boff[1] + bs1, 2048); else if (mi == 2) AOCR_DSR(b1[2], boff[1] + bs1, 4096); else AOCR_DSR(b1[3], boff[1] + bs1, 6144); }
          if (ni == 3 && mi < 2) issue_b1(step + 3, k3, mi);
          if (ni == 3 && mi == 2 && HT) issue_halo_i(2 * TAP, chn, hbn);
          AOCR_SB();
        }
      }
      asm volatile("s_waitcnt vmcnt(%0) lgkmcnt(0)" ::"n"(NVM) : "memory");
      __builtin_amdgcn_s_barrier();
      AOCR_SB();
      if (TN % 3 == 0) { set_ab(TN == 0 ? hbn : hb, TN / 3); AOCR_SB(); }
#pragma unroll
      for (int mi = 0; mi < 4; ++mi) {
#pragma unroll
        for (int ni = 0; ni < 4; ++ni) {
          acc[mi][ni] = __builtin_amdgcn_mfma_f32_32x32x16_bf16(a1[mi], b1[ni], acc[mi][ni], 0, 0, 0);
          AOCR_SB();
          if (ni == 0) AOCR_DSR(a0[mi], a_addr(mi, TN, 0), 0);
          if (ni == 2) { if (mi == 0) AOCR_DSR(b0[0], boff[0] + bs0n, 0); else if (mi == 1) AOCR_DSR(b0[1], boff[0] + bs0n, 2048); else if (mi == 2) AOCR_DSR(b0[2], boff[0] + bs0n, 4096); else AOCR_DSR(b0[3], boff[0] + bs0n, 6144); }
          if (ni == 3 && mi < 2) issue_b1(step + 3, k3, 2 + mi);
          if (ni == 3 && mi == 2 && HT) issue_halo_i(2 * TAP + 1, chn, hbn);
          AOCR_SB();
        }
      }
    };
    step_fn(std::integral_constant<int, 0>{}); step_fn(std::integral_constant<int, 1>{}); step_fn(std::integral_constant<int, 2>{});
    step_fn(std::integral_constant<int, 3>{}); step_fn(std::integral_constant<int, 4>{}); step_fn(std::integral_constant<int, 5>{});
    step_fn(std::integral_constant<int, 6>{}); step_fn(std::integral_constant<int, 7>{}); step_fn(std::integral_constant<int, 8>{});
  }
#undef AOCR_DSR
#undef AOCR_SB
  asm volatile("s_waitcnt vmcnt(0) lgkmcnt(0)" ::: "memory");
#pragma unroll
  for (int i = 0; i < 4; ++i) asm volatile("" ::"v"(a0[i]), "v"(b0[i]), "v"(a1[i]), "v"(b1[i]));
  if constexpr (TAG == 1) { if ((blockIdx.x == 17 || blockIdx.x == 300) && tid == 0) { const int o = blockIdx.x == 17 ? 4 : 0; g_kprobe[o] = __builtin_readcyclecounter() - pc0; g_kprobe[o + 1] = wall_clock64() - pw0; g_kprobe[o + 2] = pw0 - pe0; } }
  const int m0 = m_blk + wm * 128, n0 = n_blk + wn * 128;
  if (tile256_store_staged<4, 256>(ep, acc, lds, m_blk, n_blk, wm, wn, r, h, tid, opt)) {
    if constexpr (TAG == 1) { asm volatile("s_waitcnt vmcnt(0)" ::: "memory"); if ((blockIdx.x == 17 || blockIdx.x == 300) && tid == 0) g_kprobe[blockIdx.x == 17 ? 7 : 3] = wall_clock64() - pe0; }
    return;
  }
  auto store_mi = [&](auto mic) {
    constexpr int mi = decltype(mic)::value;
#pragma unroll
    for (int q = 0; q < 4; ++q) {
      float v[4][4];
#pragma unroll
      for (int ni = 0; ni < 4; ++ni)
#pragma unroll
        for (int i = 0; i < 4; ++i) v[ni][i] = acc[mi][ni][4 * q + i];
      ep.template quad<4>(m0 + 32 * mi + 8 * q + 4 * h, n0 + r, 32, v);
    }
  };
  store_mi(std::integral_constant<int, 0>{}); store_mi(std::integral_constant<int, 1>{});
  store_mi(std::integral_constant<int, 2>{}); store_mi(std::integral_constant<int, 3>{});
  if constexpr (TAG == 1) { asm volatile("s_waitcnt vmcnt(0)" ::: "memory"); if (blockIdx.x == 17 && tid == 0) g_kprobe[7] = wall_clock64() - pe0; }
}

template <class AL, class BL, class EP, int NT>
__global__ __launch_bounds__(512, 2)
void gemm_dma_narrow_kernel(AL a, BL b, EP ep, int K, int gx, int gy, const bf16_t* zero, int staged) {
  constexpr int BN = 64 * NT, SLOT = 16384 + BN * 64;
  __shared__ __attribute__((aligned(1024))) unsigned char lds[3 * SLOT];
  const int nwg = gx * gy, orig = blockIdx.x;
  const int q8 = nwg >> 3, r8 = nwg & 7, xcd = orig & 7;
  const int bid = (xcd < r8 ? xcd * (q8 + 1) : r8 * (q8 + 1) + (xcd - r8) * q8) + (orig >> 3);
  const int m_blk = (bid / gx) * 256, n_blk = (bid % gx) * BN;
  const int tid = threadIdx.x, lane = tid & 63, wave = __builtin_amdgcn_readfirstlane(tid >> 6);
  const int r = lane & 31, h = lane >> 5, wm = wave >> 1, wn = wave & 1;

  const int srow = tid >> 2, chunk = (tid & 3) ^ ((tid >> 4) & 3);
  const bool stage_b = NT == 2 || wave < 4;
  typename AL::DRow ra[2]; typename BL::DRow rb;
#pragma unroll
  for (int j = 0; j < 2; ++j) ra[j] = a.drow(m_blk + 128 * j + srow, chunk);
  rb = b.drow(n_blk + srow, chunk);
  typename AL::DCur ca = a.dseek(0); typename BL::DCur cb = b.dseek(0);
  const int nk = K >> 5;
  unsigned char* const wbase = lds + wave * 1024;
  int slot = 0;
  auto issue = [&]() {
#pragma unroll
    for (int j = 0; j < 2; ++j) dma16(a.dsrc(ra[j], ca, zero), wbase + slot * SLOT + j * 8192);
    a.dadvance(ca);
    if (stage_b) dma16(b.dsrc(rb, cb, zero), wbase + slot * SLOT + 16384);
    b.dadvance(cb);
    slot = slot == 2 ? 0 : slot + 1;
  };

  f32x16 acc[2][NT];
#pragma unroll
  for (int i = 0; i < 2; ++i)
#pragma unroll
    for (int j = 0; j < NT; ++j)
#pragma unroll
      for (int e = 0; e < 16; ++e) acc[i][j][e] = 0.f;

  const int swz = (r >> 2) & 3;
  unsigned aoff[2], boff[2];
#pragma unroll
  for (int s = 0; s < 2; ++s) {
    aoff[s] = (wm * 64 + r) * 64 + (((2 * s + h) ^ swz) << 4);
    boff[s] = 16384 + (wn * 32 * NT + r) * 64 + (((2 * s + h) ^ swz) << 4);
  }

  issue(); issue();
  int rslot = 0;
  for (int kt = 0; kt < nk; ++kt) {
    if (stage_b) asm volatile("s_waitcnt vmcnt(3)" ::: "memory");
    else asm volatile("s_waitcnt vmcnt(2)" ::: "memory");
    __builtin_amdgcn_s_barrier();
    const unsigned char* L = lds + rslot * SLOT;
    rslot = rslot == 2 ? 0 : rslot + 1;
    bf16x8 af[2][2], bf[2][NT];
#pragma unroll
    for (int s2 = 0; s2 < 2; ++s2) {
#pragma unroll
      for (int mi = 0; mi < 2; ++mi) af[s2][mi] = *reinterpret_cast<const bf16x8*>(L + aoff[s2] + mi * 2048);
#pragma unroll
      for (int ni = 0; ni < NT; ++ni) bf[s2][ni] = *reinterpret_cast<const bf16x8*>(L + boff[s2] + ni * 2048);
    }
    issue();
#pragma unroll
    for (int s2 = 0; s2 < 2; ++s2)
#pragma unroll
      for (int mi = 0; mi < 2; ++mi)
#pragma unroll
        for (int ni = 0; ni < NT; ++ni)
          acc[mi][ni] = __builtin_amdgcn_mfma_f32_32x32x16_bf16(af[s2][mi], bf[s2][ni], acc[mi][ni], 0, 0, 0);
  }
  asm volatile("s_waitcnt vmcnt(0)" ::: "memory");
  if constexpr (std::is_same<EP, EpStore>::value) {
    if (staged && narrow_store_staged<NT, EP>(ep, acc, lds, m_blk, n_blk, wm, wn, r, h, tid)) return;
  }
  const int m0 = m_blk + wm * 64, n0 = n_blk + wn * 32 * NT;
#pragma unroll
  for (int mi = 0; mi < 2; ++mi)
#pragma unroll
    for (int q = 0; q < 4; ++q) {
      float v[NT][4];
#pragma unroll
      for (int ni = 0; ni < NT; ++ni)
#pragma unroll
        for (int i = 0; i < 4; ++i) v[ni][i] = acc[mi][ni][4 * q + i];
      ep.template quad<NT>(m0 + 32 * mi + 8 * q + 4 * h, n0 + r, 32, v);
    }
}

template <class AL, class BL, class EP, int NS, int NW>
__global__ __launch_bounds__(64 * NW, (NS == 4 && NW == 4) ? 2 : 1)
void gemm_dma128_kernel(AL a, BL b, EP ep, int K, int gx, int gy, const bf16_t* zero) {
  constexpr int SLOT = 16384, NI = NW == 4 ? 2 : 1, PPW = 16 / NW;
  __shared__ __attribute__((aligned(1024))) unsigned char lds[NS * SLOT];
  const int nwg = gx * gy, orig = blockIdx.x;
  const int q8 = nwg >> 3, r8 = nwg & 7, xcd = orig & 7;
  const int bid = (xcd < r8 ? xcd * (q8 + 1) : r8 * (q8 + 1) + (xcd - r8) * q8) + (orig >> 3);
  const int m_blk = (bid / gx) * 128, n_blk = (bid % gx) * 128;
  const int tid = threadIdx.x, lane = tid & 63, wave = __builtin_amdgcn_readfirstlane(tid >> 6);
  const int r = lane & 31, h = lane >> 5, wm = NW == 4 ? wave >> 1 : wave >> 2, wn = NW == 4 ? wave & 1 : wave & 3;

  constexpr int NJ = 8 / NW;
  const int srow = tid >> 2, chunk = (tid & 3) ^ ((tid >> 4) & 3);
  typename AL::DRow ra[NJ]; typename BL::DRow rb[NJ];
#pragma unroll
  for (int j = 0; j < NJ; ++j) { ra[j] = a.drow(m_blk + 16 * NW * j + srow, chunk); rb[j] = b.drow(n_blk + 16 * NW * j + srow, chunk); }
  typename AL::DCur ca = a.dseek(0); typename BL::DCur cb = b.dseek(0);
  const int nk = K >> 5;
  unsigned char* const wbase = lds + wave * 1024;
  int slot = 0;
  auto issue = [&]() {
#pragma unroll
    for (int j = 0; j < NJ; ++j) dma16(a.dsrc(ra[j], ca, zero), wbase + slot * SLOT + j * (1024 * NW));
    a.dadvance(ca);
#pragma unroll
    for (int j = 0; j < NJ; ++j) dma16(b.dsrc(rb[j], cb, zero), wbase + slot * SLOT + 8192 + j * (1024 * NW));
    b.dadvance(cb);
    slot = slot == NS - 1 ? 0 : slot + 1;
  };
  (void)PPW;

  f32x16 acc[2][NI];
#pragma unroll
  for (int i = 0; i < 2; ++i)
#pragma unroll
    for (int j = 0; j < NI; ++j)
#pragma unroll
      for (int e = 0; e < 16; ++e) acc[i][j][e] = 0.f;

  const int swz = (r >> 2) & 3;
  unsigned aoff[2], boff[2];
#pragma unroll
  for (int s = 0; s < 2; ++s) {
    aoff[s] = (wm * 64 + r) * 64 + (((2 * s + h) ^ swz) << 4);
    boff[s] = 8192 + (wn * 32 * NI + r) * 64 + (((2 * s + h) ^ swz) << 4);
  }

#pragma unroll
  for (int i = 0; i < NS - 1; ++i) issue();
  int rslot = 0;
  for (int kt = 0; kt < nk; ++kt) {
    asm volatile("s_waitcnt vmcnt(%0)" ::"n"(2 * NJ * (NS - 2)) : "memory");
    __builtin_amdgcn_s_barrier();
    const unsigned char* L = lds + rslot * SLOT;
    rslot = rslot == NS - 1 ? 0 : rslot + 1;
    bf16x8 af[2][2], bf[2][NI];
#pragma unroll
    for (int s2 = 0; s2 < 2; ++s2) {
#pragma unroll
      for (int mi = 0; mi < 2; ++mi) af[s2][mi] = *reinterpret_cast<const bf16x8*>(L + aoff[s2] + mi * 2048);
#pragma unroll
      for (int ni = 0; ni < NI; ++ni) bf[s2][ni] = *reinterpret_cast<const bf16x8*>(L + boff[s2] + ni * 2048);
    }
    issue();
#pragma unroll
    for (int s2 = 0; s2 < 2; ++s2)
#pragma unroll
      for (int mi = 0; mi < 2; ++mi)
#pragma unroll
        for (int ni = 0; ni < NI; ++ni)
          acc[mi][ni] = __builtin_amdgcn_mfma_f32_32x32x16_bf16(af[s2][mi], bf[s2][ni], acc[mi][ni], 0, 0, 0);
  }
  asm volatile("s_waitcnt vmcnt(0)" ::: "memory");
  const int m0 = m_blk + wm * 64, n0 = n_blk + wn * 32 * NI;
#pragma unroll
  for (int mi = 0; mi < 2; ++mi)
#pragma unroll
    for (int q = 0; q < 4; ++q) {
      float v[NI][4];
#pragma unroll
      for (int ni = 0; ni < NI; ++ni)
#pragma unroll
        for (int i = 0; i < 4; ++i) v[ni][i] = acc[mi][ni][4 * q + i];
      ep.template quad<NI>(m0 + 32 * mi + 8 * q + 4 * h, n0 + r, 32, v);
    }
}

constexpr int TR_PITCH = 320;
typedef short s16x4 __attribute__((ext_vector_type(4)));
__device__ __forceinline__ s16x4 lds_tr_read(const unsigned char* p) {
  return __builtin_amdgcn_ds_read_tr16_b64_v4i16((s16x4 __attribute__((address_space(3)))*)p);
}

template <class BL, class EP>
__device__ __forceinline__ void tr_tile(const LoadMNh& a, const BL& b, const EP& ep, int m_blk, int n_blk, int kbeg, int kend,
                                        unsigned char (&lds)[2][2][32 * TR_PITCH]) {
  const int tid = threadIdx.x, lane = tid & 63, wave = tid >> 6;
  const int h = lane >> 5, wm = wave >> 1, wn = wave & 1;
  const int nk = (kend - kbeg + 31) >> 5;

  const int krow = tid >> 4, piece = tid & 15;
  LoadMNh::Ctx8 ca = a.row8(m_blk + piece * 8);
  typename BL::Ctx8 cb = b.row8(n_blk + piece * 8);
  typename BL::Cur cur0 = b.seek(cb, kbeg + krow), cur1 = b.seek(cb, kbeg + krow + 16);
  int ka = kbeg + krow;
  const bf16_t* pa = ca.b + (int64_t)ka * a.ld;
  const int64_t a16 = 16 * a.ld;
  uint4 ra[2], rb[2];
  auto gload = [&]() {
    ra[0] = (ca.ok && ka < a.K) ? *reinterpret_cast<const uint4*>(pa) : make_uint4(0, 0, 0, 0);
    ra[1] = (ca.ok && ka + 16 < a.K) ? *reinterpret_cast<const uint4*>(pa + a16) : make_uint4(0, 0, 0, 0);
    rb[0] = b.load8(cb, cur0); rb[1] = b.load8(cb, cur1);
    ka += 32; pa += 2 * a16; b.advance(cb, cur0); b.advance(cb, cur1);
  };
  auto lwrite = [&](int buf) {
    *reinterpret_cast<uint4*>(&lds[buf][0][krow * TR_PITCH + piece * 16]) = ra[0];
    *reinterpret_cast<uint4*>(&lds[buf][0][(krow + 16) * TR_PITCH + piece * 16]) = ra[1];
    *reinterpret_cast<uint4*>(&lds[buf][1][krow * TR_PITCH + piece * 16]) = rb[0];
    *reinterpret_cast<uint4*>(&lds[buf][1][(krow + 16) * TR_PITCH + piece * 16]) = rb[1];
  };

  f32x16 acc[2][2];
#pragma unroll
  for (int i = 0; i < 2; ++i)
#pragma unroll
    for (int j = 0; j < 2; ++j)
#pragma unroll
      for (int e = 0; e < 16; ++e) acc[i][j][e] = 0.f;

  const int g = lane >> 4, q = (lane >> 2) & 3, p = lane & 3;
  const int tr_off = (8 * h + q) * TR_PITCH + (16 * (g & 1) + 4 * p) * 2;

  if (nk > 0) { gload(); lwrite(0); }
  __syncthreads();
  for (int kt = 0; kt < nk; ++kt) {
    const int buf = kt & 1;
    if (kt + 1 < nk) gload();
// ... 839 lines not shown
```

torch-attention-ocr_amd/csrc/model.h:

```cpp
#pragma once
#include <string>
#include <vector>
#include "../../include/aocr.h"
#include "ops.h"

namespace aocr {

constexpr int MAXL = 4;
constexpr int LOGIT_LD = 40;

struct ParamEntry { std::string name; int group; int64_t offset; int ndim; int64_t shape[4]; int64_t numel; };
struct Layout { std::vector<ParamEntry> e; int64_t group_off[AOCR_NUM_GROUPS + 1]; };
Layout build_layout(const aocr_config& c);

struct ConvP { float *w, *b, *dw, *db; int cin, cout, ks, pad; };
struct BnP { float *w, *b, *dw, *db, *rm, *rv, *save; int C; };
struct ShW { const float* w; int64_t ld; int R, C; bf16_t* wb; bf16_t* wtb; float* wtf; };
struct LstmP { float *wi, *bi, *wh, *bh, *dwi, *dbi, *dwh, *dbh; int in; ShW swi, swh; };

struct Arena {
  char* base; size_t off;
  template <class T> T* get(size_t n) {
    off = (off + 255) & ~(size_t)255;
    T* p = base ? reinterpret_cast<T*>(base + off) : nullptr;
    off += n * sizeof(T);
    return p;
  }
};

struct CommState {
  int nranks = 1; bool sync_bn = false; int provider = 0;
  void* rccl = nullptr; void* rccl_bn = nullptr; aocr_allreduce_fn fn = nullptr; void* user = nullptr;
  hipStream_t stream = nullptr; hipEvent_t done = nullptr;
  hipEvent_t wait0 = nullptr, wait1 = nullptr; bool timed = false;
};

struct Dims {
  int B, H, W, L, T;
  int H1, W1, H2, W2, H4, H6, Ho7, Wo7;
};
bool make_dims(const aocr_config& c, int B, int W, int L, Dims& d);

}

struct aocr_model {
  aocr_config cfg;
  hipStream_t s;
  bool bf16;
  float *params, *grads, *bn_state;
  aocr::Layout layout;
  aocr::ConvP conv[8];
  aocr::BnP bn[8];
  aocr::LstmP enc[2][aocr::MAXL], dec[aocr::MAXL];
  float *lookup, *dlookup, *wa, *dwa, *wc, *dwc, *wo, *bo, *dwo, *dbo;
  aocr::ShW swa, swc;
  int He, Hd, Le, Ld, E, V;

  size_t ws_bytes;
  float *A1, *A2, *Y3, *A3, *A4, *Y5, *A5, *A6, *Y7, *X;
  uint8_t *idx2, *idx4, *idx6;
  uint16_t* route1 = nullptr; bool route1_valid = false;
  float *G0, *G1, *dX; size_t gmax = 0;
  aocr::bf16_t *A1b, *A2b, *A3b, *A4b, *A5b, *A6b, *G0b, *G2b = nullptr;
  hipEvent_t cw_map[2] = {nullptr, nullptr}, cw_done[2] = {nullptr, nullptr}, cw_main = nullptr;
  aocr::bf16_t *wb[8], *wtb[8];
  float* wtf[8];
  aocr::bf16_t *Xb, *ehs_b[2][aocr::MAXL], *edz_b[2][aocr::MAXL], *dhs_b[aocr::MAXL], *ddz_b[aocr::MAXL], *out_b, *cat_b, *dpre_b, *dq_b;
  void* bn_scratch; float* bn_save;
  int y16[2] = {0, 0};
  float *ezx[2][aocr::MAXL], *ehs[2][aocr::MAXL], *ecs[2][aocr::MAXL], *egates[2][aocr::MAXL], *edz[2][aocr::MAXL], *edc[2][aocr::MAXL];
  float *edxl[2];
  float *context, *dctx;
  aocr::bf16_t* context_b;
  float* emb_seg = nullptr; int* emb_index = nullptr; bool emb_table = false, tab_valid = false;
  hipEvent_t tab_done = nullptr, zero_done = nullptr, shadow_done = nullptr, shadow2_done = nullptr; bool tab_ready = false, zero_pending = false, shadow_pending = false, shadow2_pending = false;
  int shadow_tiles_conv2 = 0;
  bool proj_fused = false, dout_ready = false;
  float* loss_pending = nullptr;
  hipEvent_t q_go = nullptr, q_done = nullptr; bool q_pending = false;
  hipEvent_t enc_ev = nullptr;
  float *emb_all, *zx1_all, *dhs[aocr::MAXL], *dcs[aocr::MAXL], *dgates[aocr::MAXL], *ddz[aocr::MAXL];
  float *out_all, *cat_all, *q_all, *a_all, *logits, *dlogits, *nll_rows;
  float *dout_proj, *dpre_all, *dcat_all, *ds_all, *dq_all, *demb_all;
  float *dh_rec[aocr::MAXL], *dc_st[aocr::MAXL], *dfeed, *loss_tmp;
  float *bc[2][aocr::MAXL], *bh[2][aocr::MAXL], *bfeed[2], *bc_new[aocr::MAXL], *bh_new[aocr::MAXL];
  aocr::bf16_t *bh_b[2][aocr::MAXL] = {}, *bfeed_b[2] = {}, *bh_new_b[aocr::MAXL] = {}, *bcat_b = nullptr;
  float *bzx1, *bzx_tab, *bq, *ba, *bcat, *bout, *blogits, *blogp, *beam_scores;
  int32_t *hist_tok, *hist_par, *tgt_pad, *tge_pad, *trie_loc[2];
  float *attn_hist = nullptr, *sc_hist = nullptr;
  void* sgd_scratch;
  float* wg_part = nullptr; size_t wg_part_floats = 0;

  std::vector<aocr::ShadowJob> shadow_host;
  aocr::ShadowJob* shadow_dev; int shadow_tiles;
  hipEvent_t grad_ev[4];
  hipStream_t lay_s[aocr::MAXL] = {}; std::vector<hipEvent_t> lay_ev;
  hipStream_t side2 = nullptr; hipEvent_t side2_done = nullptr;
  hipStream_t side = nullptr; hipEvent_t side_go = nullptr, side_done = nullptr; bool side_busy = false;
  int64_t conv5_off;
  aocr::Dims last;
  int last_valid;
  const float* last_images = nullptr; bool last_train = false;
  unsigned long long *cl_xbuf = nullptr, *cl_pbuf = nullptr, *cl_xtab = nullptr; int* cl_err = nullptr; size_t cl_xbytes = 0, cl_pbytes = 0, cl_tbytes = 0; unsigned cl_epoch = 0;
  unsigned long long *dc_xbuf = nullptr, *dc_xtab = nullptr; size_t dc_xbytes = 0, dc_tbytes = 0; aocr::bf16_t* ctxa_b = nullptr; bool ctxa_fresh = false;  bool dgates_il = false; unsigned long long* dc_bxbuf = nullptr; size_t dc_bxbytes = 0; float* dc_pbuf = nullptr;
  double drop_p = 0.0; unsigned long long drop_thr = 0, drop_seed = 0, drop_step = 0; bool drop_on = false;
  float* dhm[aocr::MAXL] = {}; aocr::bf16_t* dhm_b[aocr::MAXL] = {}; float* ehm[2][aocr::MAXL] = {}; aocr::bf16_t* ehm_b[2][aocr::MAXL] = {};
  aocr::CommState comm;
  float* bn_snap = nullptr;
  bool prof_on = false;
  std::vector<hipEvent_t> prof_ev; std::vector<int> prof_tag; size_t prof_n = 0;
};

namespace aocr {
const char* comm_unique_id(char id[128]);
const char* comm_init_rccl(aocr_model* m, const char id[128], int nranks, int rank, int sync_bn);
const char* comm_init_callback(aocr_model* m, aocr_allreduce_fn fn, void* user, int nranks, int sync_bn);
void comm_destroy(aocr_model* m);
int comm_allreduce(aocr_model* m, void* buf, int64_t count, int dtype, hipStream_t stream, int channel);
int comm_allreduce_grads(aocr_model* m, float* loss_dev);
inline bool sync_bn_on(const aocr_model* m) { return m->comm.provider != 0 && m->comm.sync_bn; }
inline bool env_on(const char* name) { const char* e = getenv(name); return e && e[0] == '1'; }
inline bool comm_early_bucket0() { return env_on("AOCR_COMM_EARLY_BUCKET0"); }
inline bool comm_holds_bucket0(const aocr_model* m) { return m->comm.provider != 0 && !comm_early_bucket0(); }
inline int comm_reserved_cus(const aocr_model* m) {
  if (m->comm.provider == 0 || !comm_early_bucket0()) return 0;
  const char* e = getenv("AOCR_COMM_RESERVE_CUS");
  const int n = e ? atoi(e) : 32;
  return n < 0 ? 0 : (n > 128 ? 128 : n);
}
void prof_mark_slow(aocr_model* m, int tag);
inline void prof_mark(aocr_model* m, int tag) { if (m->prof_on) prof_mark_slow(m, tag); }
void step_prologue(aocr_model* m, size_t grad_bytes);
void build_shadow_jobs(aocr_model* m);
int model_carve(aocr_model* m, void* base, size_t bytes);
void cnn_forward(aocr_model* m, const float* images, const Dims& d, int training, int update_running);
void encoder_forward(aocr_model* m, const Dims& d);
void decoder_tf_forward(aocr_model* m, const Dims& d, const int32_t* tgt, int64_t st, int64_t sb, bool keep_gates);
void loss_and_dlogits(aocr_model* m, const Dims& d, const int32_t* tge, int64_t st, int64_t sb, float grad_scale, bool want_grad,
                      float* loss_dev);
void backward_all(aocr_model* m, const float* images, const int32_t* tgt, const Dims& d);
void decode_beam(aocr_model* m, const Dims& d, const int32_t* tgt, int beam, int32_t* labels, float* scores,
                 const aocr_trie* trie = nullptr, float* attn_hist = nullptr, float* sc_hist = nullptr);
}
```

torch-attention-ocr_amd/csrc/model.hip:

```cpp
#include "model.h"
#include <cmath>
#include <cstdio>
#include <cstring>
#include <cstdlib>

namespace aocr {

static void add_entry(Layout& L, int64_t& off, const std::string& name, int group, std::initializer_list<int64_t> shape) {
  ParamEntry e; e.name = name; e.group = group; e.offset = off; e.ndim = (int)shape.size(); e.numel = 1;
  int i = 0; for (int64_t v : shape) { e.shape[i++] = v; e.numel *= v; }
  for (; i < 4; ++i) e.shape[i] = 1;
  off += e.numel; L.e.push_back(e);
}
Layout build_layout(const aocr_config& c) {
  Layout L; int64_t off = 0;
  const int He = c.enc_hidden, Hd = 2 * He;
  static const int convs[7][4] = {{1, 64, 3, 1}, {64, 128, 3, 1}, {128, 256, 3, 1}, {256, 256, 3, 1},
                                  {256, 512, 3, 1}, {512, 512, 3, 1}, {512, 512, 2, 0}};
  L.group_off[0] = 0;
  for (int i = 0; i < 7; ++i) {
    char nm[64];
    snprintf(nm, 64, "cnn.conv%d.w", i + 1); add_entry(L, off, nm, 0, {convs[i][1], convs[i][2], convs[i][2], convs[i][0]});
    snprintf(nm, 64, "cnn.conv%d.b", i + 1); add_entry(L, off, nm, 0, {convs[i][1]});
    if (i == 2 || i == 4 || i == 6) {
// ... 187 lines not shown
  for (int dir = 0; dir < 2; ++dir) for (int l = 0; l < m->Le; ++l) { up(m->enc[dir][l].swh); up(m->enc[dir][l].swi); }
  for (int l = 0; l < m->Ld; ++l) { if (l > 0 || m->cfg.input_feed) up(m->dec[l].swi); up(m->dec[l].swh); }
  up(m->swa); up(m->swc);
}
static LoadK bnt_f(const ShW* w0, const ShW* w1) {
  return w1 ? make_loadk2(w0->w, w0->ld, w0->C, w1->w, w1->ld, w1->C, w0->R) : make_loadk(w0->w, w0->ld, w0->R, w0->C);
}
static LoadKh2 bnt_h(const ShW* w0, const ShW* w1) {
  return w1 ? make_loadkh2(w0->wb, w0->C, w0->C, w1->wb, w1->C, w1->C, w0->R) : make_loadkh(w0->wb, w0->C, w0->R, w0->C);
}
static bool hh_ok(const LoadKh2* ah, int nz, int ncols) {
  if (!ah || ncols % 32 != 0) return false;
  for (int i = 0; i < nz; ++i) if (!ah[i].p0 || ah[i].K <= 0 || ah[i].K % 64 != 0 || ah[i].K0 % 64 != 0) return false;
  return true;
}
static void run_gates_fwd(aocr_model* m, int nz, const LoadK* a, const ShW* const* w0, const ShW* const* w1, const EpGatesFwd* ep,
                          int M, int H, const LoadKh2* ah = nullptr) {
  if (m->bf16 && hh_ok(ah, nz, H)) {
    if (nz == 1 && big_step_gates_fwd(m->s, ah[0], bnt_h(w0[0], w1[0]), ep[0], M, H, m->ddz[0], (size_t)m->cfg.max_decoder_l * m->cfg.batch_size * 4 * m->Hd)) return;
    GatesFwdArgsHH z[2];
    for (int i = 0; i < nz; ++i) { z[i].a = ah[i]; z[i].b = bnt_h(w0[i], w1[i]); z[i].ep = ep[i]; z[i].K = ah[i].K; }
    launch_small_gates_fwd_hh(m->s, nz, z, M, H);
  } else if (m->bf16) {
    GatesFwdArgsH z[2];
    for (int i = 0; i < nz; ++i) { z[i].a = a[i]; z[i].b = bnt_h(w0[i], w1[i]); z[i].ep = ep[i]; z[i].K = a[i].K; }
    launch_small_gates_fwd_h(m->s, nz, z, M, H);
  } else {
    GatesFwdArgs z[2];
    for (int i = 0; i < nz; ++i) { z[i].a = a[i]; z[i].b = bnt_f(w0[i], w1[i]); z[i].ep = ep[i]; z[i].K = a[i].K; }
    launch_small_gates_fwd(m->s, false, nz, z, M, H);
  }
}
static void run_store_nt(aocr_model* m, const LoadK& a, const ShW& w, const EpStore& ep, int M, const LoadKh2* ah = nullptr) {
  if (m->bf16 && hh_ok(ah, 1, w.R)) { if (big_step_store(m->s, *ah, bnt_h(&w, nullptr), ep, M, w.R)) return; SmallArgsHH z; z.a = *ah; z.b = bnt_h(&w, nullptr); z.ep = ep; z.K = ah->K; launch_small_hh(m->s, 1, &z, M, w.R); }
  else if (m->bf16) { SmallArgsH z; z.a = a; z.b = bnt_h(&w, nullptr); z.ep = ep; z.K = a.K; launch_small_h(m->s, 1, &z, M, w.R); }
  else { SmallKKArgs z; z.a = a; z.b = bnt_f(&w, nullptr); z.ep = ep; z.K = a.K; launch_small_kk(m->s, false, 1, &z, M, w.R); }
}
static void run_store_nn(aocr_model* m, const LoadK& a, const ShW& w, const EpStore& ep, int M, const LoadKh2* ah = nullptr) {
  if (m->bf16 && hh_ok(ah, 1, w.C)) { if (big_step_store(m->s, *ah, make_loadkh(w.wtb, w.R, w.C, w.R), ep, M, w.C)) return; SmallArgsHH z; z.a = *ah; z.b = make_loadkh(w.wtb, w.R, w.C, w.R); z.ep = ep; z.K = ah->K; launch_small_hh(m->s, 1, &z, M, w.C); }
  else if (m->bf16) { SmallArgsH z; z.a = a; z.b = make_loadkh(w.wtb, w.R, w.C, w.R); z.ep = ep; z.K = a.K; launch_small_h(m->s, 1, &z, M, w.C); }
  else if (w.wtf) { SmallKKArgs z; z.a = a; z.b = make_loadk(w.wtf, w.R, w.C, w.R); z.ep = ep; z.K = a.K; launch_small_kk(m->s, false, 1, &z, M, w.C); }
  else { SmallKMNArgs z; z.a = a; z.b = make_loadmn(w.w, w.ld, w.C, a.K); z.ep = ep; z.K = a.K; launch_small_kmn(m->s, false, 1, &z, M, w.C); }
}
static void run_store_nn_group(aocr_model* m, int n, const LoadK* a, const ShW* const* w, const EpStore* ep, int M, const LoadKh2* ah) {
  bool same = m->bf16 && hh_ok(ah, n, w[0]->C);
  for (int i = 1; i < n && same; ++i) same = w[i]->C == w[0]->C;
  if (same) {
    SmallArgsHH z[3];
    for (int i = 0; i < n; ++i) { z[i].a = ah[i]; z[i].b = make_loadkh(w[i]->wtb, w[i]->R, w[i]->C, w[i]->R); z[i].ep = ep[i]; z[i].K = ah[i].K; }
    launch_small_hh(m->s, n, z, M, w[0]->C);
    return;
  }
  bool same32 = !m->bf16;
  for (int i = 0; i < n && same32; ++i) same32 = w[i]->wtf != nullptr && w[i]->C == w[0]->C;
  if (same32) {
    SmallKKArgs z[3];
    for (int i = 0; i < n; ++i) { z[i].a = a[i]; z[i].b = make_loadk(w[i]->wtf, w[i]->R, w[i]->C, w[i]->R); z[i].ep = ep[i]; z[i].K = a[i].K; }
    launch_small_kk(m->s, false, n, z, M, w[0]->C);
    return;
  }
  for (int i = 0; i < n; ++i) run_store_nn(m, a[i], *w[i], ep[i], M, ah ? &ah[i] : nullptr);
}
static void run_gates_bwd(aocr_model* m, int nz, const LoadK* a, const ShW* const* w, const EpGatesBwd* ep, int M, int H,
                          const LoadKh2* ah = nullptr) {
  if (nz == 1 && a[0].K == 0 && ep[0].drop.thr == 0) { gates_elem_bwd(m->s, ep[0], M, H); return; }
  if (m->bf16 && hh_ok(ah, nz, H)) {
    GatesBwdArgsHH z[2];
    for (int i = 0; i < nz; ++i) { z[i].a = ah[i]; z[i].b = make_loadkh(w[i]->wtb, w[i]->R, w[i]->C, ah[i].K); z[i].ep = ep[i]; z[i].K = ah[i].K; }
    launch_small_gates_bwd_hh(m->s, nz, z, M, H);
  } else if (m->bf16) {
    GatesBwdArgsH z[2];
    for (int i = 0; i < nz; ++i) { z[i].a = a[i]; z[i].b = make_loadkh(w[i]->wtb, w[i]->R, w[i]->C, a[i].K); z[i].ep = ep[i]; z[i].K = a[i].K; }
    launch_small_gates_bwd_h(m->s, nz, z, M, H);
  } else {
    if (w[0]->wtf) {
      GatesBwdKKArgs z[2];
      for (int i = 0; i < nz; ++i) { z[i].a = a[i]; z[i].b = make_loadk(w[i]->wtf, w[i]->R, w[i]->C, a[i].K); z[i].ep = ep[i]; z[i].K = a[i].K; }
      launch_small_gates_bwd_kk(m->s, nz, z, M, H);
      return;
    }
    GatesBwdArgs z[2];
    for (int i = 0; i < nz; ++i) { z[i].a = a[i]; z[i].b = make_loadmn(w[i]->w, w[i]->ld, w[i]->C, a[i].K); z[i].ep = ep[i]; z[i].K = a[i].K; }
    launch_small_gates_bwd(m->s, false, nz, z, M, H);
  }
}

static int bn_sync_allreduce(void* ctx, void* buf, int64_t count, int dtype, hipStream_t s) { return comm_allreduce((aocr_model*)ctx, buf, count, dtype, s, 1); }

void cnn_forward(aocr_model* m, const float* images, const Dims& d, int training, int update_running) {
  hipStream_t s = m->s; const bool bf = m->bf16; const int B = d.B;
  m->y16[0] = m->y16[1] = 0;
  const BnSync bsync_v{bn_sync_allreduce, m}; const BnSync* bsync = (training && sync_bn_on(m)) ? &bsync_v : nullptr;
  if (bf && !m->shadow_host.empty()) {
    if (!m->shadow_pending) shadow_jobs(s, m->shadow_dev, (int)m->shadow_host.size(), m->shadow_tiles);
  } else {
    refresh_rnn_shadows(m);
    for (int i = 2; i <= 7; ++i) {
      if (bf) conv_weight_shadows(s, m->conv[i].w, m->wb[i], m->wtb[i], m->conv[i].cout, m->conv[i].ks * m->conv[i].ks, m->conv[i].cin);
      else conv_weight_transpose_f32(s, m->conv[i].w, m->wtf[i], m->conv[i].cout, m->conv[i].ks * m->conv[i].ks, m->conv[i].cin);
    }
  }
  prof_mark(m, AOCR_PROF_POOL_CONV1); conv1_forward(s, images, m->conv[1].w, m->conv[1].b, bf ? nullptr : m->A1, B, d.H, d.W, m->A1b, training ? m->route1 : nullptr);
  m->route1_valid = training;
  if (m->shadow_pending && m->shadow2_pending) { hipStreamWaitEvent(s, m->shadow2_done, 0); m->shadow2_pending = false; }
  else if (m->shadow_pending) { hipStreamWaitEvent(s, m->shadow_done, 0); m->shadow_pending = false; }
  prof_mark(m, AOCR_PROF_CONV_FWD); conv_forward(s, bf, m->A1, m->conv[2].w, m->conv[2].b, bf ? nullptr : m->A2, m->idx2, B, d.H1, d.W1, 64, 128, 3, 1, 1, 1, m->A1b, m->wb[2], m->A2b);
  if (m->shadow_pending) { hipStreamWaitEvent(s, m->shadow_done, 0); m->shadow_pending = false; }
  const bool fold = bf && !training && !getenv("AOCR_NO_BN_FOLD");
  if (fold) {
    prof_mark(m, AOCR_PROF_BN); bn_eval_prepare(s, m->bn[3].rm, m->bn[3].rv, m->bn[3].save, 256);
    prof_mark(m, AOCR_PROF_CONV_FWD); conv_forward(s, bf, m->A2, m->conv[3].w, m->conv[3].b, nullptr, nullptr, B, d.H2, d.W2, 128, 256, 3, 1, 0, 0, m->A2b, m->wb[3], m->A3b, 0,
                                                   m->bn[3].save, m->bn[3].w, m->bn[3].b);
  } else {
  int bnc = 0;
  prof_mark(m, AOCR_PROF_CONV_FWD); conv_forward(s, bf, m->A2, m->conv[3].w, m->conv[3].b, m->Y3, nullptr, B, d.H2, d.W2, 128, 256, 3, 1, 0, 0, m->A2b, m->wb[3], nullptr, 0,
                                                 nullptr, nullptr, nullptr, training ? (double*)m->bn_scratch : nullptr, &bnc, &m->y16[0]);
  prof_mark(m, AOCR_PROF_BN); bn_relu_forward(s, m->Y3, bf ? nullptr : m->A3, m->bn[3].w, m->bn[3].b, m->bn[3].rm, m->bn[3].rv, m->bn[3].save, m->bn_scratch,
                  (int64_t)B * d.H2 * d.W2, 256, training, update_running, 0, m->A3b, bsync, bnc, m->y16[0] ? reinterpret_cast<const bf16_t*>(m->Y3) : nullptr);
  }
  prof_mark(m, AOCR_PROF_CONV_FWD); conv_forward(s, bf, m->A3, m->conv[4].w, m->conv[4].b, bf ? nullptr : m->A4, m->idx4, B, d.H2, d.W2, 256, 256, 3, 1, 1, 2, m->A3b, m->wb[4], m->A4b);
  if (fold) {
    prof_mark(m, AOCR_PROF_BN); bn_eval_prepare(s, m->bn[5].rm, m->bn[5].rv, m->bn[5].save, 512);
    prof_mark(m, AOCR_PROF_CONV_FWD); conv_forward(s, bf, m->A4, m->conv[5].w, m->conv[5].b, nullptr, nullptr, B, d.H4, d.W2, 256, 512, 3, 1, 0, 0, m->A4b, m->wb[5], m->A5b, 0,
                                                   m->bn[5].save, m->bn[5].w, m->bn[5].b);
  } else {
  int bnc = 0;
  prof_mark(m, AOCR_PROF_CONV_FWD); conv_forward(s, bf, m->A4, m->conv[5].w, m->conv[5].b, m->Y5, nullptr, B, d.H4, d.W2, 256, 512, 3, 1, 0, 0, m->A4b, m->wb[5], nullptr, 0,
                                                 nullptr, nullptr, nullptr, training ? (double*)m->bn_scratch : nullptr, &bnc, &m->y16[1]);
  prof_mark(m, AOCR_PROF_BN); bn_relu_forward(s, m->Y5, bf ? nullptr : m->A5, m->bn[5].w, m->bn[5].b, m->bn[5].rm, m->bn[5].rv, m->bn[5].save, m->bn_scratch,
                  (int64_t)B * d.H4 * d.W2, 512, training, update_running, 0, m->A5b, bsync, bnc, m->y16[1] ? reinterpret_cast<const bf16_t*>(m->Y5) : nullptr);
  }
  prof_mark(m, AOCR_PROF_CONV_FWD); conv_forward(s, bf, m->A5, m->conv[6].w, m->conv[6].b, bf ? nullptr : m->A6, m->idx6, B, d.H4, d.W2, 512, 512, 3, 1, 1, 2, m->A5b, m->wb[6], m->A6b);
  prof_mark(m, AOCR_PROF_CONV_FWD); conv_forward(s, bf, m->A6, m->conv[7].w, m->conv[7].b, m->Y7, nullptr, B, d.H6, d.W2, 512, 512, 2, 0, 0, 0, m->A6b, m->wb[7], nullptr);
  prof_mark(m, AOCR_PROF_BN); bn_relu_forward(s, m->Y7, m->X, m->bn[7].w, m->bn[7].b, m->bn[7].rm, m->bn[7].rv, m->bn[7].save, m->bn_scratch,
                  (int64_t)B * d.T, 512, training, update_running, B, m->Xb, bsync);
}

static bool cnn_wgrad_on_side(aocr_model* m) {
  auto evok = [](hipEvent_t& e) { return e || hipEventCreateWithFlags(&e, hipEventDisableTiming) == hipSuccess; };
  return m->bf16 && m->G2b && !getenv("AOCR_DBG_STOP") && !m->prof_on && m->side && m->side_done && !getenv("AOCR_NO_SIDE_WGRAD") && !env_on("AOCR_NO_CNN_WGRAD_SIDE") &&
         evok(m->cw_map[0]) && evok(m->cw_map[1]) && evok(m->cw_done[0]) && evok(m->cw_done[1]) && evok(m->cw_main);
}

static void cnn_backward(aocr_model* m, const float* images, const Dims& d) {
  hipStream_t s = m->s; const bool bf = m->bf16; const int B = d.B;
  const BnSync bsync_v{bn_sync_allreduce, m}; const BnSync* bsync = sync_bn_on(m) ? &bsync_v : nullptr;
  float *G0 = m->G0, *G1 = m->G1;
  bf16_t* Gb[2] = {m->G0b, m->G2b}; int gp = 0;
  const char* dbg_stop = getenv("AOCR_DBG_STOP");
  const int stop = dbg_stop ? atoi(dbg_stop) : 0;
  const bool ws = !stop && cnn_wgrad_on_side(m);
  hipStream_t sw = ws ? m->side : s;
  const bool wg_after = ws && env_on("AOCR_CNN_WGRAD_AFTER_DGRAD");
  if (!ws) Gb[1] = Gb[0];
  auto map_ready = [&]() { if (ws) { hipEventRecord(m->cw_map[gp], s); hipStreamWaitEvent(sw, m->cw_map[gp], 0); } };
  auto wgrad_done = [&]() { if (ws) hipEventRecord(m->cw_done[gp], sw); };
  auto next_map = [&]() { if (ws) { gp ^= 1; hipStreamWaitEvent(s, m->cw_done[gp], 0); } };
  int bnbc = 0;
  int g16 = 0; const bf16_t* const G1h = reinterpret_cast<const bf16_t*>(G1);
  constexpr size_t SLAB = (size_t)4 << 20;
  ColsumJobs cj; cj.n = 0; cj.total = 0;
  ColsumJobs* defer = (bf && m->gmax >= 8 * SLAB && !getenv("AOCR_NO_COLSUM_DEFER")) ? &cj : nullptr;
  auto slab = [&](int k) { return defer ? G0 + (size_t)k * SLAB : G0; };
  prof_mark(m, AOCR_PROF_BN); bn_relu_backward(s, m->Y7, m->X, m->dX, m->bn[7].w, m->bn[7].save, bf ? nullptr : G0, m->bn[7].dw, m->bn[7].db, m->bn_scratch,
                   (int64_t)B * d.T, 512, B, Gb[gp], bf ? m->Xb : nullptr, bf ? m->conv[7].db : nullptr, bf ? slab(0) : nullptr, bsync, defer);
  if (stop == 1) { if (defer) colsum_flush(s, cj); return; }
  { auto W = [&]() { prof_mark(m, AOCR_PROF_CONV_WGRAD); conv_backward_filter(sw, bf, m->A6, G0, m->conv[7].dw, bf ? nullptr : m->conv[7].db, B, d.H6, d.W2, 512, 512, 2, 0, m->A6b, Gb[gp], m->wg_part, m->wg_part_floats); };
    auto D = [&]() { prof_mark(m, AOCR_PROF_CONV_DGRAD); conv_backward_data(s, bf, G0, m->conv[7].w, G1, B, d.H6, d.W2, 512, 512, 2, 0, Gb[gp], m->wtb[7], m->wtf[7], bf ? &g16 : nullptr); };
    if (wg_after) { D(); map_ready(); W(); wgrad_done(); } else { map_ready(); W(); wgrad_done(); D(); } }
  next_map(); prof_mark(m, AOCR_PROF_POOL_CONV1); unpool_relu_backward(s, G1, m->A6, m->idx6, bf ? nullptr : G0, B, d.H4, d.W2, 512, 2, Gb[gp], bf ? m->conv[6].db : nullptr, bf ? slab(1) : nullptr, bf ? m->A6b : nullptr, defer, g16 ? G1h : nullptr);
  if (stop == 2) { if (defer) colsum_flush(s, cj); return; }
  { auto W = [&]() { prof_mark(m, AOCR_PROF_CONV_WGRAD); conv_backward_filter(sw, bf, m->A5, G0, m->conv[6].dw, bf ? nullptr : m->conv[6].db, B, d.H4, d.W2, 512, 512, 3, 1, m->A5b, Gb[gp], m->wg_part, m->wg_part_floats); };
    auto D = [&]() { prof_mark(m, AOCR_PROF_CONV_DGRAD); { const BnBwdFuse bf5{m->Y5, m->A5b, m->bn[5].save, (double*)m->bn_scratch}; conv_backward_data(s, bf, G0, m->conv[6].w, G1, B, d.H4, d.W2, 512, 512, 3, 1, Gb[gp], m->wtb[6], m->wtf[6], bf ? &g16 : nullptr, (bf && !m->y16[1]) ? &bf5 : nullptr, &bnbc); } };
    if (wg_after) { D(); map_ready(); W(); wgrad_done(); } else { map_ready(); W(); wgrad_done(); D(); } }
  next_map(); prof_mark(m, AOCR_PROF_BN); bn_relu_backward(s, m->Y5, m->A5, G1, m->bn[5].w, m->bn[5].save, bf ? nullptr : G0, m->bn[5].dw, m->bn[5].db, m->bn_scratch,
                   (int64_t)B * d.H4 * d.W2, 512, 0, Gb[gp], bf ? m->A5b : nullptr, bf ? m->conv[5].db : nullptr, bf ? slab(2) : nullptr, bsync, defer, m->y16[1] ? reinterpret_cast<const bf16_t*>(m->Y5) : nullptr, g16 ? G1h : nullptr, bnbc); bnbc = 0;
  { auto W = [&]() { prof_mark(m, AOCR_PROF_CONV_WGRAD); conv_backward_filter(sw, bf, m->A4, G0, m->conv[5].dw, bf ? nullptr : m->conv[5].db, B, d.H4, d.W2, 256, 512, 3, 1, m->A4b, Gb[gp], m->wg_part, m->wg_part_floats); };
    auto D = [&]() { prof_mark(m, AOCR_PROF_CONV_DGRAD); conv_backward_data(s, bf, G0, m->conv[5].w, G1, B, d.H4, d.W2, 256, 512, 3, 1, Gb[gp], m->wtb[5], m->wtf[5], bf ? &g16 : nullptr); };
    if (wg_after) { D(); map_ready(); W(); wgrad_done(); } else { map_ready(); W(); wgrad_done(); }
  if (defer) colsum_flush(s, cj);
  if (ws) { hipEventRecord(m->cw_main, s); hipStreamWaitEvent(sw, m->cw_main, 0); hipEventRecord(m->grad_ev[2], sw); }
  else hipEventRecord(m->grad_ev[2], s);
    if (!wg_after) D(); }
  next_map(); prof_mark(m, AOCR_PROF_POOL_CONV1); unpool_relu_backward(s, G1, m->A4, m->idx4, bf ? nullptr : G0, B, d.H2, d.W2, 256, 2, Gb[gp], bf ? m->conv[4].db : nullptr, bf ? slab(3) : nullptr, bf ? m->A4b : nullptr, defer, g16 ? G1h : nullptr);
  { auto W = [&]() { prof_mark(m, AOCR_PROF_CONV_WGRAD); conv_backward_filter(sw, bf, m->A3, G0, m->conv[4].dw, bf ? nullptr : m->conv[4].db, B, d.H2, d.W2, 256, 256, 3, 1, m->A3b, Gb[gp], m->wg_part, m->wg_part_floats); };
    auto D = [&]() { prof_mark(m, AOCR_PROF_CONV_DGRAD); { const BnBwdFuse bf3{m->Y3, m->A3b, m->bn[3].save, (double*)m->bn_scratch}; conv_backward_data(s, bf, G0, m->conv[4].w, G1, B, d.H2, d.W2, 256, 256, 3, 1, Gb[gp], m->wtb[4], m->wtf[4], bf ? &g16 : nullptr, (bf && !m->y16[0]) ? &bf3 : nullptr, &bnbc); } };
    if (wg_after) { D(); map_ready(); W(); wgrad_done(); } else { map_ready(); W(); wgrad_done(); D(); } }
  next_map(); prof_mark(m, AOCR_PROF_BN); bn_relu_backward(s, m->Y3, m->A3, G1, m->bn[3].w, m->bn[3].save, bf ? nullptr : G0, m->bn[3].dw, m->bn[3].db, m->bn_scratch,
                   (int64_t)B * d.H2 * d.W2, 256, 0, Gb[gp], bf ? m->A3b : nullptr, bf ? m->conv[3].db : nullptr, bf ? slab(4) : nullptr, bsync, defer, m->y16[0] ? reinterpret_cast<const bf16_t*>(m->Y3) : nullptr, g16 ? G1h : nullptr, bnbc); bnbc = 0;
  { auto W = [&]() { prof_mark(m, AOCR_PROF_CONV_WGRAD); conv_backward_filter(sw, bf, m->A2, G0, m->conv[3].dw, bf ? nullptr : m->conv[3].db, B, d.H2, d.W2, 128, 256, 3, 1, m->A2b, Gb[gp], m->wg_part, m->wg_part_floats); };
    auto D = [&]() { prof_mark(m, AOCR_PROF_CONV_DGRAD); conv_backward_data(s, bf, G0, m->conv[3].w, G1, B, d.H2, d.W2, 128, 256, 3, 1, Gb[gp], m->wtb[3], m->wtf[3]); };
    if (wg_after) { D(); map_ready(); W(); wgrad_done(); } else { map_ready(); W(); wgrad_done(); D(); } }
  next_map(); prof_mark(m, AOCR_PROF_POOL_CONV1); unpool_relu_backward(s, G1, m->A2, m->idx2, bf ? nullptr : G0, B, d.H1, d.W1, 128, 1, Gb[gp], bf ? m->conv[2].db : nullptr, bf ? slab(5) : nullptr, bf ? m->A2b : nullptr, defer);
  { auto W = [&]() { prof_mark(m, AOCR_PROF_CONV_WGRAD); conv_backward_filter(sw, bf, m->A1, G0, m->conv[2].dw, bf ? nullptr : m->conv[2].db, B, d.H1, d.W1, 64, 128, 3, 1, m->A1b, Gb[gp], m->wg_part, m->wg_part_floats); };
    auto D = [&]() { prof_mark(m, AOCR_PROF_CONV_DGRAD); conv_backward_data(s, bf, G0, m->conv[2].w, G1, B, d.H1, d.W1, 64, 128, 3, 1, Gb[gp], m->wtb[2], m->wtf[2]); };
    if (wg_after) { D(); map_ready(); W(); wgrad_done(); } else { map_ready(); W(); wgrad_done(); D(); } }
  prof_mark(m, AOCR_PROF_POOL_CONV1); conv1_backward(s, images, m->conv[1].w, m->conv[1].b, G1, m->conv[1].dw, m->conv[1].db, B, d.H, d.W,
                 (size_t)B * d.H1 * d.W1 * 128 >= (size_t)4096 * 640 ? slab(6) : nullptr, defer,
                 m->route1_valid && !getenv("AOCR_CONV1_RECOMPUTE") ? m->route1 : nullptr);
  if (defer) colsum_flush(s, cj);
  if (ws) { hipEventRecord(m->side_done, sw); hipStreamWaitEvent(s, m->side_done, 0); }
}

static bool seq_kernels_ok(const aocr_model* m, int B) {
  if (!m->bf16 || !m->ehs_b[0][0] || !m->enc[0][0].swh.wb) return false;
  const char* e = getenv("AOCR_NO_SEQ");
  if (e && e[0] == '1') return false;
  static const int cus = [] { int n = 0, dev = 0; (void)hipGetDevice(&dev); (void)hipDeviceGetAttribute(&n, hipDeviceAttributeMultiprocessorCount, dev); return n; }();
  return enc_seq_supported(B, m->He, cus);
}

static bool cluster_ok(const aocr_model* m, int B, int T, int& G, int& RT, int& groups) {
  if (!m->bf16 || !m->cl_xbuf || !m->ehs_b[0][0] || !m->enc[0][0].swh.wb || !m->edz_b[0][0]) return false;
  const char* e = getenv("AOCR_NO_CLUSTER");
  if (e && e[0] == '1') return false;
  e = getenv("AOCR_NO_SEQ");
  if (e && e[0] == '1') return false;
  static const int cus = [] { int n = 0, dev = 0; (void)hipGetDevice(&dev); (void)hipDeviceGetAttribute(&n, hipDeviceAttributeMultiprocessorCount, dev); return n; }();
  return enc_cluster_plan(B, m->He, T, cus - comm_reserved_cus(m), G, RT, groups);
}
static unsigned next_epoch(aocr_model* m) {
  if (++m->cl_epoch >= (1u << 20)) {
    hipMemsetAsync(m->cl_xbuf, 0, m->cl_xbytes, m->s); hipMemsetAsync(m->cl_pbuf, 0, m->cl_pbytes, m->s); m->cl_epoch = 1;
    hipMemsetAsync(m->cl_xtab, 0, m->cl_tbytes, m->s);
    if (m->dc_xbuf) { hipMemsetAsync(m->dc_xbuf, 0, m->dc_xbytes, m->s); hipMemsetAsync(m->dc_xtab, 0, m->dc_tbytes, m->s); hipMemsetAsync(m->dc_bxbuf, 0, m->dc_bxbytes, m->s); }
  }
  return m->cl_epoch;
}

static DropSpec drop_site(const aocr_model* m, int site, long long off) {
  DropSpec d;
  if (!m->drop_on) return d;
  const unsigned long long stream = m->drop_step * 64ull + (unsigned long long)site;
  d.base = splitmix64_(m->drop_seed ^ (stream * 0xD1342543DE82EF95ull)); d.thr = m->drop_thr; d.scale = (float)(1.0 / (1.0 - m->drop_p)); d.off = off;
  return d;
}

static int layer_pipe_chunks(const aocr_model* m, int T, int G, int groups) {
  if (m->Le < 2 || m->prof_on || getenv("AOCR_NO_LAYER_PIPE")) return 0;
  static const int cus = [] { int n = 0, dev = 0; (void)hipGetDevice(&dev); (void)hipDeviceGetAttribute(&n, hipDeviceAttributeMultiprocessorCount, dev); return n; }();
  if (2 * groups * G * m->Le > cus) return 0;
  int C = std::min(8, T / 48);
  if (const char* e = getenv("AOCR_LAYER_PIPE_CHUNKS")) C = std::min(atoi(e), T);
  return C >= 2 ? C : 0;
}
static bool layer_pipe_streams(aocr_model* m, int n_events) {
  for (int l = 1; l < m->Le; ++l)
    if (!m->lay_s[l] && hipStreamCreateWithFlags(&m->lay_s[l], hipStreamNonBlocking) != hipSuccess) { m->lay_s[l] = nullptr; return false; }
  while ((int)m->lay_ev.size() < n_events) {
    hipEvent_t e; if (hipEventCreateWithFlags(&e, hipEventDisableTiming) != hipSuccess) return false;
    m->lay_ev.push_back(e);
  }
  return true;
}
static void reserve_epochs(aocr_model* m, unsigned n) { if (m->cl_epoch + n + 1 >= (1u << 20)) { m->cl_epoch = (1u << 20); (void)next_epoch(m); } }

static void encoder_forward_pipe(aocr_model* m, const Dims& d, int C, int clG, int clRT, int clGroups) {
  hipStream_t s0 = m->s;
  const int B = d.B, T = d.T, He = m->He, Hd = m->Hd, Le = m->Le;
  const size_t slot = (size_t)B * He;
  for (int l = 0; l < Le; ++l) {
    ZeroList zl;
    for (int dir = 0; dir < 2; ++dir) {
      zl.add(m->ehs[dir][l], slot * sizeof(float)); zl.add(m->ehs[dir][l] + (size_t)(T + 1) * slot, slot * sizeof(float));
      zl.add(m->ecs[dir][l], slot * sizeof(float)); zl.add(m->ecs[dir][l] + (size_t)(T + 1) * slot, slot * sizeof(float));
      zl.add(m->ehs_b[dir][l], slot * sizeof(bf16_t)); zl.add(m->ehs_b[dir][l] + (size_t)(T + 1) * slot, slot * sizeof(bf16_t));
    }
    zero_many(s0, zl);
  }
  for (int dir = 0; dir < 2; ++dir) {
    const LstmP& p = m->enc[dir][0];
    gemm_hh(s0, m->Xb, p.in, p.swi.wb, p.in, m->ezx[dir][0], 4 * He, T * B, 4 * He, p.in, p.bi, p.bh, 0);
  }
  reserve_epochs(m, (unsigned)(C * Le));
  hipEvent_t* ev = m->lay_ev.data();
  hipEventRecord(ev[Le * C], s0);
  for (int l = 1; l < Le; ++l) hipStreamWaitEvent(m->lay_s[l], ev[Le * C], 0);
  const int Tc = (T + C - 1) / C;
  for (int c = 0; c < C; ++c) {
    const int it0 = c * Tc, it1 = std::min(T, it0 + Tc);
    if (it0 >= it1) break;
    for (int l = 0; l < Le; ++l) {
      hipStream_t sl = l == 0 ? s0 : m->lay_s[l];
      if (l > 0) {
        hipStreamWaitEvent(sl, ev[(l - 1) * C + c], 0);
        for (int dir = 0; dir < 2; ++dir) {
          const LstmP& p = m->enc[dir][l];
          const int t_lo = dir ? T - it1 : it0, n = it1 - it0;
          const bf16_t* xinb = m->ehs_b[dir][l - 1] + (size_t)(t_lo + 1) * slot;
          if (m->drop_on) {
            dropout_apply_b(sl, xinb, m->ehm[dir][l - 1] + (size_t)t_lo * slot, m->ehm_b[dir][l - 1] + (size_t)t_lo * slot, (int64_t)n * slot,
                            drop_site(m, (dir ? 48 : 32) + l + 1, (long long)t_lo * (long long)slot));
            xinb = m->ehm_b[dir][l - 1] + (size_t)t_lo * slot;
          }
          gemm_hh(sl, xinb, p.in, p.swi.wb, p.in, m->ezx[dir][l] + (size_t)t_lo * B * 4 * He, 4 * He, n * B, 4 * He, p.in, p.bi, p.bh, 0);
        }
      }
      const bool top = l == Le - 1;
      EncClFwdArgs a; a.B = B; a.T = T; a.He = He; a.Hd = Hd; a.groups = clGroups; a.epoch = next_epoch(m); a.xbuf = m->cl_xbuf; a.err = m->cl_err; a.xtab = m->cl_xtab;
      a.it0 = it0; a.it1 = it1; a.gslot = l * 2 * clGroups;
      for (int dir = 0; dir < 2; ++dir) {
        EncSeqDir& e = a.d[dir];
        e.w = m->enc[dir][l].swh.wb; e.zx = m->ezx[dir][l]; e.hs = m->ehs[dir][l]; e.cs = m->ecs[dir][l]; e.hsb = m->ehs_b[dir][l];
        e.gates = m->egates[dir][l]; e.ctx = top ? m->context + dir * He : nullptr; e.reverse = dir;
      }
      enc_cluster_forward(sl, a, clG, clRT, comm_reserved_cus(m), Le);
      if (!top) hipEventRecord(ev[l * C + c], sl);
    }
  }
  for (int l = 1; l < Le; ++l) { hipEventRecord(ev[Le * C + l], m->lay_s[l]); hipStreamWaitEvent(s0, ev[Le * C + l], 0); }
}

void encoder_forward(aocr_model* m, const Dims& d) {
  m->ctxa_fresh = false;
  hipStream_t s = m->s; const bool bf = m->bf16;
  const int B = d.B, T = d.T, He = m->He, Hd = m->Hd;
  const size_t slot = (size_t)B * He;
  int clG = 0, clRT = 0, clGroups = 0;
  const bool cluster = cluster_ok(m, B, T, clG, clRT, clGroups);
  const int pipeC = cluster ? layer_pipe_chunks(m, T, clG, clGroups) : 0;
  if (pipeC && layer_pipe_streams(m, (m->Le + 1) * pipeC + m->Le + 1)) {
    if (getenv("AOCR_TRACE")) fprintf(stderr, "[aocr] encoder forward: cluster kernels, layer wavefront of %d chunks\n", pipeC);
    encoder_forward_pipe(m, d, pipeC, clG, clRT, clGroups);
    if (m->context_b) copy2d_bf16(s, m->context, Hd, m->context_b, Hd, B * T, Hd);
    return;
  }
  for (int l = 0; l < m->Le; ++l) {
    ZeroList zl;
    for (int dir = 0; dir < 2; ++dir) {
      const LstmP& p = m->enc[dir][l];
      const float* xin = l == 0 ? m->X : m->ehs[dir][l - 1] + slot;
      const bf16_t* xinb = l == 0 ? m->Xb : (m->ehs_b[dir][l - 1] ? m->ehs_b[dir][l - 1] + slot : nullptr);
      prof_mark(m, AOCR_PROF_RNN_GEMM);
      if (l > 0 && m->drop_on) {
        if (cluster && xinb)
          dropout_apply_b(s, xinb, m->ehm[dir][l - 1], m->ehm_b[dir][l - 1], (int64_t)T * B * He, drop_site(m, (dir ? 48 : 32) + l + 1, 0));
        else
        dropout_apply(s, xin, m->ehm[dir][l - 1], m->ehm_b[dir][l - 1], (int64_t)T * B * He, drop_site(m, (dir ? 48 : 32) + l + 1, 0));
        xin = m->ehm[dir][l - 1]; xinb = m->ehm_b[dir][l - 1];
      }
      if (bf && xinb && p.swi.wb && p.in % 32 == 0)
        gemm_hh(s, xinb, p.in, p.swi.wb, p.in, m->ezx[dir][l], 4 * He, T * B, 4 * He, p.in, p.bi, p.bh, 0);
      else
        gemm(s, bf, xin, p.in, true, p.wi, p.in, true, m->ezx[dir][l], 4 * He, T * B, 4 * He, p.in, p.bi, p.bh, 0);
      zl.add(m->ehs[dir][l], slot * sizeof(float)); zl.add(m->ehs[dir][l] + (size_t)(T + 1) * slot, slot * sizeof(float));
      zl.add(m->ecs[dir][l], slot * sizeof(float)); zl.add(m->ecs[dir][l] + (size_t)(T + 1) * slot, slot * sizeof(float));
// ... 749 lines not shown
```

torch-attention-ocr_amd/csrc/ops.h:

```cpp
#pragma once
#include <hip/hip_runtime.h>
#include <stdint.h>
#include "aocr.h"
#include "epilogues.h"
#include "mfma_gemm.h"

namespace aocr {

inline int cdiv(int64_t a, int64_t b) { return (int)((a + b - 1) / b); }

inline LoadK make_loadk(const float* p, int64_t ld, int rows, int K) {
  LoadK l; l.p0 = p; l.ld0 = ld; l.K0 = K; l.p1 = nullptr; l.ld1 = 0; l.rows = rows; l.K = K;
  l.vec = (((uintptr_t)p & 15) == 0) && (ld % 4 == 0);
  return l;
}
inline LoadK make_loadk2(const float* p0, int64_t ld0, int K0, const float* p1, int64_t ld1, int K1, int rows) {
  LoadK l; l.p0 = p0; l.ld0 = ld0; l.K0 = K0; l.p1 = p1; l.ld1 = ld1; l.rows = rows; l.K = K0 + K1;
  l.vec = (((uintptr_t)p0 & 15) == 0) && (ld0 % 4 == 0) && (((uintptr_t)p1 & 15) == 0) && (ld1 % 4 == 0) && (K0 % 16 == 0);
  return l;
}
inline LoadMN make_loadmn(const float* p, int64_t ld, int rows, int K) {
  LoadMN l; l.p = p; l.ld = ld; l.rows = rows; l.K = K;
  l.vec = (((uintptr_t)p & 15) == 0) && (ld % 4 == 0);
  return l;
}
inline EpStore make_store(float* C, int64_t ldc, int M, int N, const float* bias = nullptr, const float* bias2 = nullptr,
                          int flags = 0) {
  EpStore e; e.C = C; e.ldc = ldc; e.M = M; e.N = N; e.bias = bias; e.bias2 = bias2; e.flags = flags;
  e.C1 = nullptr; e.ldc1 = 0; e.N0 = N; return e;
}

void launch_big_kk(hipStream_t s, bool bf16, const LoadK& a, const LoadK& b, const EpStore& ep, int M, int N, int K, int ksplit);
void launch_big_kmn(hipStream_t s, bool bf16, const LoadK& a, const LoadMN& b, const EpStore& ep, int M, int N, int K, int ksplit);
void launch_big_mnmn(hipStream_t s, bool bf16, const LoadMN& a, const LoadMN& b, const EpStore& ep, int M, int N, int K, int ksplit);
void launch_conv_fwd(hipStream_t s, bool bf16, const LoadConvK& a, const LoadK& b, const EpConv& ep, int M, int N, int K);
void launch_conv_dgrad(hipStream_t s, bool bf16, const LoadConvK& a, const LoadConvWT& b, const EpStore& ep, int M, int N, int K);
void launch_conv_wgrad(hipStream_t s, bool bf16, const LoadMN& a, const LoadConvXcol& b, const EpStore& ep, int M, int N, int K, int ksplit);

typedef SmallArgs<LoadK, LoadK, EpGatesFwd> GatesFwdArgs;
typedef SmallArgs<LoadK, LoadK, EpStore> SmallKKArgs;
typedef SmallArgs<LoadK, LoadMN, EpStore> SmallKMNArgs;
typedef SmallArgs<LoadK, LoadMN, EpGatesBwd> GatesBwdArgs;
void launch_small_gates_fwd(hipStream_t s, bool bf16, int nz, const GatesFwdArgs* z, int M, int H);
void launch_small_kk(hipStream_t s, bool bf16, int nz, const SmallKKArgs* z, int M, int N);
void launch_small_kmn(hipStream_t s, bool bf16, int nz, const SmallKMNArgs* z, int M, int N);
void launch_small_gates_bwd(hipStream_t s, bool bf16, int nz, const GatesBwdArgs* z, int M, int H);
typedef SmallArgs<LoadK, LoadK, EpGatesBwd> GatesBwdKKArgs;
void launch_small_gates_bwd_kk(hipStream_t s, int nz, const GatesBwdKKArgs* z, int M, int H);
typedef SmallArgs<LoadK, LoadKh2, EpGatesFwd> GatesFwdArgsH;
typedef SmallArgs<LoadK, LoadKh2, EpStore> SmallArgsH;
typedef SmallArgs<LoadK, LoadKh2, EpGatesBwd> GatesBwdArgsH;
typedef SmallArgs<LoadKh2, LoadKh2, EpGatesFwd> GatesFwdArgsHH;
typedef SmallArgs<LoadKh2, LoadKh2, EpStore> SmallArgsHH;
typedef SmallArgs<LoadKh2, LoadKh2, EpGatesBwd> GatesBwdArgsHH;
void launch_small_gates_fwd_hh(hipStream_t s, int nz, const GatesFwdArgsHH* z, int M, int H);
bool big_step_store(hipStream_t s, const LoadKh2& a, const LoadKh2& b, const EpStore& ep, int M, int N);
bool big_step_gates_fwd(hipStream_t s, const LoadKh2& a, const LoadKh2& b, const EpGatesFwd& ep, int M, int H, float* zbuf, size_t zbuf_floats);
void launch_small_hh(hipStream_t s, int nz, const SmallArgsHH* z, int M, int N);
void launch_small_gates_bwd_hh(hipStream_t s, int nz, const GatesBwdArgsHH* z, int M, int H);
void launch_small_gates_fwd_h(hipStream_t s, int nz, const GatesFwdArgsH* z, int M, int H);
void launch_small_h(hipStream_t s, int nz, const SmallArgsH* z, int M, int N);
void launch_small_gates_bwd_h(hipStream_t s, int nz, const GatesBwdArgsH* z, int M, int H);
inline LoadKh2 make_loadkh(const bf16_t* p, int64_t ld, int rows, int K) {
  LoadKh2 l; l.p0 = p; l.ld0 = ld; l.K0 = K; l.p1 = nullptr; l.ld1 = 0; l.rows = rows; l.K = K; return l;
}
inline LoadKh2 make_loadkh2(const bf16_t* p0, int64_t ld0, int K0, const bf16_t* p1, int64_t ld1, int K1, int rows) {
  LoadKh2 l; l.p0 = p0; l.ld0 = ld0; l.K0 = K0; l.p1 = p1; l.ld1 = ld1; l.rows = rows; l.K = K0 + K1; return l;
}
void weight_shadows(hipStream_t s, const float* w, int64_t ld, int R, int C, bf16_t* wb, bf16_t* wtb);
void transpose_f32(hipStream_t s, const float* w, int64_t ld, int R, int C, float* wt);
void conv_weight_transpose_f32(hipStream_t s, const float* w, float* wt, int Cout, int KK, int Cin);

bool project_loss_ok(int rows, int V, int Hd);
void project_loss(hipStream_t s, const float* out, int64_t ldo, const float* wo, const float* bo, float* logits, float* dlogits, int64_t ld, float* nll, float* dout,
                  const int32_t* tgt, int64_t st, int64_t sb, int Bt, int rows, int V, int Hd, float scale);
int gemm(hipStream_t s, bool bf16, const float* A, int64_t lda, bool a_kmajor, const float* B, int64_t ldb, bool b_kmajor,
          float* C, int64_t ldc, int M, int N, int K, const float* bias, const float* bias2, int flags);

struct WGradProblem { const float* A; int64_t lda; const float* B; int64_t ldb; float* C; int64_t ldc; int M, N, K;
                      const bf16_t* Ab = nullptr; const bf16_t* Bb = nullptr; };
void grouped_wgrad(hipStream_t s, bool bf16, const WGradProblem* p, int n, float* part = nullptr, size_t part_floats = 0);
void kprobe_read(unsigned long long out[8]);

bool gemm_hh_cat(hipStream_t s, const bf16_t* A0, const bf16_t* A1, int64_t lda, const bf16_t* B0, const bf16_t* B1, int64_t ldb, float* C, int64_t ldc, int M, int N, int K0, int K1);
void gemm_hh(hipStream_t s, const bf16_t* A, int64_t lda, const bf16_t* B, int64_t ldb, float* C, int64_t ldc, int M, int N, int K,
             const float* bias, const float* bias2, int flags);
void gemm_hh_shadow(hipStream_t s, const bf16_t* A, int64_t lda, const bf16_t* B, int64_t ldb, float* C, int64_t ldc, bf16_t* Cb, int64_t ldcb,
                    int M, int N, int K);

void conv_forward(hipStream_t s, bool bf16, const float* x, const float* w, const float* bias, float* y, uint8_t* idx,
                  int B, int H, int W, int Cin, int Cout, int ks, int pad, int relu, int pool,
                  const bf16_t* xb = nullptr, const bf16_t* wb = nullptr, bf16_t* yb = nullptr, int profile_tag = 0,
                  const float* bn_save = nullptr, const float* bn_w = nullptr, const float* bn_b = nullptr,
                  double* bn_part = nullptr, int* bn_chunks = nullptr, int* y_bf16 = nullptr);
void bn_eval_prepare(hipStream_t s, const float* rm, const float* rv, float* save, int C);
struct BnBwdFuse { const float* x; const bf16_t* yb; const float* save; double* part; };
void conv_backward_data(hipStream_t s, bool bf16, const float* dy, const float* w, float* dx, int B, int H, int W, int Cin,
                        int Cout, int ks, int pad, const bf16_t* dyb = nullptr, const bf16_t* wtb = nullptr, const float* wtf = nullptr,
                        int* dx16 = nullptr ,
                        const struct BnBwdFuse* bnb = nullptr, int* bnb_chunks = nullptr );
void conv_backward_filter(hipStream_t s, bool bf16, const float* x, const float* dy, float* dw, float* dbias, int B, int H,
                          int W, int Cin, int Cout, int ks, int pad, const bf16_t* xb = nullptr, const bf16_t* dyb = nullptr,
                          float* part = nullptr, size_t part_floats = 0, int profile_tag = 0);
void splitk_reduce(hipStream_t s, const float* part, int ks, size_t n, float* out);

void conv1_forward(hipStream_t s, const float* x, const float* w, const float* bias, float* y, int B, int H, int W,
                   bf16_t* yb = nullptr, uint16_t* route = nullptr);
size_t conv1_route_elems(int B, int H, int W);
void conv_weight_shadows(hipStream_t s, const float* w, bf16_t* wb, bf16_t* wtb, int Cout, int KK, int Cin);
struct ColsumJobs;
void conv1_backward(hipStream_t s, const float* x, const float* w, const float* bias, const float* dyp, float* dw, float* db,
                    int B, int H, int W, float* scratch = nullptr, ColsumJobs* defer = nullptr,
                    const uint16_t* route = nullptr );
void unpool_relu_backward(hipStream_t s, const float* dpooled, const float* pooled, const uint8_t* idx, float* dy, int B,
                          int Ho, int Wo, int C, int pool, bf16_t* dyb = nullptr, float* dbias = nullptr,
                          float* partial = nullptr, const bf16_t* pooledb = nullptr, ColsumJobs* defer = nullptr,
                          const bf16_t* dpooled16 = nullptr );
void bf16_to_f32(hipStream_t s, const bf16_t* src, float* dst, int64_t n);
size_t bn_scratch_bytes(int C);
struct BnSync { int (*allreduce)(void* ctx, void* buf, int64_t count, int dtype, hipStream_t s); void* ctx; };
void bn_relu_forward(hipStream_t s, const float* x, float* y, const float* w, const float* b, float* rm, float* rv,
                     float* save, void* scratch, int64_t rows, int C, int training, int update_running, int tb_rows,
                     bf16_t* yb = nullptr, const BnSync* sync = nullptr, int stats_chunks = 0 ,
                     const bf16_t* xh = nullptr );
void bn_relu_backward(hipStream_t s, const float* x, const float* y, const float* dA, const float* w, const float* save,
                      float* dx, float* dw, float* db, void* scratch, int64_t rows, int C, int tb_rows, bf16_t* dxb = nullptr,
                      const bf16_t* yb = nullptr, float* conv_dbias = nullptr, float* partial = nullptr, const BnSync* sync = nullptr,
                      ColsumJobs* defer = nullptr, const bf16_t* xh = nullptr ,
                      const bf16_t* dAh = nullptr ,
                      int sums_chunks = 0 );
void attention_forward(hipStream_t s, const float* ctx, const float* q, float* a, float* c, int64_t ldc, int B, int T, int Hd,
                       int ctx_div = 1, bf16_t* cb = nullptr, int64_t ldcb = 0, const bf16_t* ctxb = nullptr);
void gates_elem_bwd(hipStream_t s, const EpGatesBwd& ep, int M, int H);
bool attention_dual_ok(int T, int Hd, const bf16_t* ctxb, const bf16_t* ctxab);
void attention_forward_dual(hipStream_t s, const float* h_top, int64_t ldh, float* a, float* c, int64_t ldc, int B, int T, int ctx_div, bf16_t* cb, int64_t ldcb,
                            const bf16_t* ctxb, const bf16_t* ctxab);
void attention_backward_dual(hipStream_t s, const float* a, const float* dc, int64_t lddc, float* ds, float* dq, bf16_t* dqb, float* dh_attn, int B, int T,
                             const bf16_t* ctxb, const bf16_t* ctxab);
void attention_backward(hipStream_t s, const float* ctx, const float* q, const float* a, const float* dc, int64_t lddc,
                        float* ds, float* dq, int B, int T, int Hd, bf16_t* dqb = nullptr, const bf16_t* ctxb = nullptr,
                        const float* cfwd = nullptr, int64_t ldcf = 0);
void attention_dctx(hipStream_t s, const float* a_all, const float* ds_all, const float* dc_all, int64_t lddc,
                    const float* q_all, float* dctx, int L, int B, int T, int Hd);
void logsoftmax_nll(hipStream_t s, const float* logits, int64_t ld, const int32_t* tgt, int64_t tgt_stride_t,
                    int64_t tgt_stride_b, int Bt, float* logp, float* dlogits, float* nll_rows, int64_t rows, int V,
                    float grad_scale);
void sum_to_scalar(hipStream_t s, const float* x, int64_t n, float* out);
void gold_scores(hipStream_t s, const float* nll_rows, float* gold, int L, int B);
struct ZeroList { void* p[16]; size_t bytes[16]; int n = 0;
  void add(void* q, size_t b) { if (q && b && n < 16) { p[n] = q; bytes[n] = b; ++n; } } };
void zero_many(hipStream_t s, const ZeroList& z);
void colsum_accum(hipStream_t s, const float* A, int64_t ld, int64_t rows, int N, float* out, float* out2 = nullptr);
struct ColsumJob { const float* A; int64_t ld, rows; int N; float* out; float* out2; int first, nb, chunks; };
struct ColsumJobs { int n, total; ColsumJob j[8]; };
void colsum_defer(ColsumJobs& g, const float* A, int64_t ld, int64_t rows, int N, float* out, float* out2 = nullptr);
void colsum_flush(hipStream_t s, ColsumJobs& g);
void embedding_gather(hipStream_t s, const float* table, const int32_t* tok, int64_t stride_t, int64_t stride_b, float* out,
                      int L, int B, int E);
bool segsum_supported(int ncols, int V, int E);
size_t segsum_index_ints(int rows, int V);
void segsum_by_token(hipStream_t s, const float* dz, int64_t ld, const int32_t* tok, int64_t st, int64_t sb, int L, int B, int ncols, int V, float* S, int* index,
                     float* db1, float* db2, const float* W, int64_t ldw, const float* lookup, int E, float* dlookup, float* dW);
void embedding_scatter_accum(hipStream_t s, const float* demb, const int32_t* tok, int64_t stride_t, int64_t stride_b,
                             float* dtable, int L, int B, int E, int V);
void dpre_tanh(hipStream_t s, const float* g1, const float* g2, const float* out, float* dpre, int64_t n, bf16_t* dpreb = nullptr, const DropSpec* drop = nullptr);
void pointwise(hipStream_t s, int op, const float* a, const float* b, float* y, int64_t n);
void u8_to_f32(hipStream_t s, const uint8_t* src, float* dst, int64_t n);
void dropout_apply(hipStream_t s, const float* src, float* dst, bf16_t* dstb, int64_t n, const DropSpec& drop);
void dropout_apply_b(hipStream_t s, const bf16_t* src, float* dst, bf16_t* dstb, int64_t n, const DropSpec& drop);
void copy2d_bf16(hipStream_t s, const float* src, int64_t lds, bf16_t* dst, int64_t ldd, int rows, int cols);
void copy2d(hipStream_t s, const float* src, int64_t lds, float* dst, int64_t ldd, int rows, int cols);
void copy2d_pair(hipStream_t s, const float* s0, const float* s1, int64_t lds, float* d0, float* d1, int64_t ldd, int rows, int cols);
struct DecInitArgs { float* c0[4]; float* h0[4]; bf16_t* hb[4]; float* feed0; bf16_t* outb; const float *cfw, *cbw, *hfw, *hbw; int B, He, Hd, Ld, copy_h; };
void dec_init(hipStream_t s, const DecInitArgs& a);
void sgd_clip_update(hipStream_t s, float* params, float* grads, const int64_t* group_off , float lr,
                     float clip, float* norms_out, void* scratch, int* err = nullptr,
                     float* bn_state = nullptr, const float* bn_snap = nullptr, int bn_n = 0);
constexpr int CL_ERR_LATCH = 12, CL_ERR_STICKY = 13;
void step_snapshot(hipStream_t s, const float* bn_state, float* bn_snap, int n, int* err);
size_t sgd_scratch_bytes();
void adadelta_update(hipStream_t s, float* params, float* grads, float* var, float* acc, int64_t n, float rho, float eps, float wd, int* err = nullptr,
                     float* bn_state = nullptr, const float* bn_snap = nullptr, int bn_n = 0);
struct ShadowJob { const float* w; bf16_t* wb; bf16_t* wtb; int64_t ld, ldb, ldt; int R, C, tile0, tx; };
void shadow_jobs(hipStream_t s, const ShadowJob* jobs_dev, int njobs, int total_tiles, int tile_off = 0);
struct TrieView { const unsigned long long* mask; const int32_t* base; const int32_t* child; const int32_t* loc_in; int32_t* loc_out; };
void beam_select(hipStream_t s, const float* logp, const int32_t* prev_tok, float* beam_scores, int32_t* tokens,
                 int32_t* parents, int B, int kin, int kout, int V, const float* logits = nullptr, int64_t ldl = 0,
                 const TrieView* tv = nullptr, float* sc_out = nullptr);
void project_select(hipStream_t s, const float* h, int64_t ldh, const float* wo, const float* bo, int Hd, const int32_t* prev_tok,
                    float* beam_scores, int32_t* tokens, int32_t* parents, int B, int kin, int kout, int V,
                    const TrieView* tv = nullptr, float* sc_out = nullptr);
void token_rows(hipStream_t s, const float* table, const int32_t* tok, int64_t stride, float* dst, int R, int width);
void gather_beam_rows_many(hipStream_t s, int n, const float* const* src, float* const* dst, int64_t ld, const int32_t* parents, int B, int kin, int kout, int width,
                           bf16_t* const* dstb = nullptr);
void gather_beam_rows(hipStream_t s, const float* src, int64_t lds, float* dst, int64_t ldd, const int32_t* parents, int B,
                      int kin, int kout, int width);
void beam_backtrace(hipStream_t s, const int32_t* hist_tok, const int32_t* hist_par, const float* beam_scores,
                    int32_t* labels, float* scores, int Lt, int B, int k);
void recognize_gather(hipStream_t s, const int32_t* labels, const int32_t* hist_par, const float* beam_scores, const float* sc_hist,
                      const float* attn_hist, float* char_logp, float* attn, int Lt, int B, int k, int T);
void fill_i32(hipStream_t s, int32_t* p, int32_t v, int64_t n);
void edit_distance(hipStream_t s, const int32_t* labels, const int32_t* targets, int B, int L, int32_t* dist, int32_t* target_len);
int lexicon_slices(int n_words);
void lexicon_nearest(hipStream_t s, const int32_t* labels, int B, int L, const uint8_t* words, int n_words, int stride,
                     const int32_t* row_begin, void* scratch, int32_t* index, int32_t* dist);

struct EncSeqDir {
  const bf16_t* w;
  const float* zx;
  float* hs; float* cs;
  bf16_t* hsb;
  float* gates;
  float* ctx;
  int reverse;
};
struct EncSeqFwdArgs { EncSeqDir d[2]; int B, T, He, Hd; int abl = 0; unsigned long long* dbg = nullptr; };
struct EncSeqBwdDir {
  const bf16_t* wt;
  const float* dh1;
  int64_t dh1_row, dh1_t;
  const float* dh2;
  int64_t dh2_row;
  float* dc;
  const float* dc_in = nullptr; int64_t dc_in_row = 0;
  const float* gates;
  const float* cs;
  float* dz; bf16_t* dzb;
  float* dbi = nullptr; float* dbh = nullptr;
  int forward_dir;
};
struct EncSeqBwdArgs { EncSeqBwdDir d[2]; int B, T, He; };
bool enc_seq_supported(int B, int He, int blocks_limit);
struct EncClFwdArgs { EncSeqDir d[2]; int B, T, He, Hd, groups; unsigned epoch; unsigned long long* xbuf; int* err; int gid0 = 0, ngid = 0; unsigned long long* xtab = nullptr; int force_remote = 0; int it0 = 0, it1 = 0 , gslot = 0 ; int rh = 16 ; };
struct EncClBwdArgs { EncSeqBwdDir d[2]; int B, T, He, groups; unsigned epoch; unsigned long long* pbuf; int* err; int gid0 = 0, ngid = 0; unsigned long long* xtab = nullptr; int force_remote = 0; int it0 = 0, it1 = 0, gslot = 0; int rh = 16 ; };
bool enc_cluster_plan(int B, int He, int T, int cus, int& G, int& RT, int& groups);
size_t enc_cluster_xbuf_bytes(int B, int He);
size_t enc_cluster_pbuf_bytes(int B, int He);
void enc_cluster_forward(hipStream_t s, const EncClFwdArgs& a, int G, int RT, int reserve_cus = 0, int concurrent = 1);
void enc_cluster_backward(hipStream_t s, const EncClBwdArgs& a, int G, int RT, int reserve_cus = 0, int concurrent = 1);
struct DecClFwdArgs {
  int B, T, L; unsigned epoch; int group0 = 0, ngroups = 0, force_remote = 0; int no_early = 0;
  const bf16_t *w1i, *w1h, *w2i, *w2h, *wc;
  const float *b2i, *b2h;
  const float* zx1;
  const bf16_t *ctxb, *ctxa;
  float* cs[2]; bf16_t* hsb[2];
  float* gates[2];
  float *a_all, *out; bf16_t *cat_b, *out_b;
  unsigned long long *xbuf, *xtab; int* err; unsigned long long* stamps = nullptr;
  const int32_t* tok0 = nullptr; int tok0_stride = 0; const float *wo = nullptr, *bo = nullptr; int V = 0;
  float* pbuf = nullptr; unsigned* tokx = nullptr; int32_t* labels = nullptr; float* scores = nullptr; int pgroups = 0;
  const unsigned long long* trie_mask = nullptr; const int32_t* trie_base = nullptr; const int32_t* trie_child = nullptr;
  int beam = 0, rows_slot = 0; int32_t *hist_tok = nullptr, *hist_par = nullptr; float* beam_scores = nullptr;
// ... 40 lines not shown
```

torch-attention-ocr_amd/csrc/ops_gemm.hip:

```cpp
#include "ops.h"
#include "stepl.h"

namespace aocr {

static void split_k(int K, int chunk, int& ksplit, int& kper) {
  if (ksplit < 1) ksplit = 1;
  kper = cdiv(cdiv(K, ksplit), chunk) * chunk;
  if (kper < chunk) kper = chunk;
  ksplit = cdiv(K, kper); if (ksplit < 1) ksplit = 1;
}
static thread_local const char* t_trace_fn = nullptr;
struct TraceScope { explicit TraceScope(const char* fn) { t_trace_fn = fn; } ~TraceScope() { t_trace_fn = nullptr; } };
static void trace_launch(const char* kernel, const char* inst, long long M, long long N, long long K) {
  if (t_trace_fn && getenv("AOCR_TRACE")) fprintf(stderr, "[aocr] %s: %s[%s] %lld %lld %lld\n", t_trace_fn, kernel, inst, M, N, K);
}
static void trace_step(int nt, int gates, int waves, int mt, long long M, long long N, long long K) {
  if (!t_trace_fn || !getenv("AOCR_TRACE")) return;
  char inst[32]; snprintf(inst, sizeof inst, "%d,%d,w%d%s", nt, gates, waves, mt == 2 ? ",mt2" : "");
  trace_launch("gemm_step_kernel", inst, M, N, K);
}
template <class AL, class BL, class EP>
static void launch_lds(hipStream_t s, const AL& a, const BL& b, const EP& ep, int M, int N, int K, int ksplit) {
  if (M <= 0 || N <= 0) return;
  int kper; split_k(K, 32, ksplit, kper);
// ... 529 lines not shown
                  const int32_t* tgt, int64_t st, int64_t sb, int Bt, int rows, int V, int Hd, float scale) {
  ProjLossArgs g; g.a = make_loadk(out, ldo, rows, Hd); g.b = make_loadk(wo, Hd, V, Hd); g.bias = bo; g.wo = wo; g.ldw = Hd;
  g.logits = logits; g.dlogits = dlogits; g.ld = ld; g.nll = nll; g.dout = dout; g.lddo = Hd; g.tgt = tgt; g.st = st; g.sb = sb; g.Bt = Bt; g.rows = rows; g.V = V; g.K = Hd; g.scale = scale;
  hipLaunchKernelGGL(project_loss_kernel, dim3(1, cdiv(rows, 32)), dim3(256), 0, s, g);
}

void gemm_hh(hipStream_t s, const bf16_t* A, int64_t lda, const bf16_t* B, int64_t ldb, float* C, int64_t ldc, int M, int N, int K,
             const float* bias, const float* bias2, int flags) {
  const TraceScope ts("gemm_hh");
  LoadKh a; a.p = A; a.ld = lda; a.rows = M; a.K = K;
  LoadKh b; b.p = B; b.ld = ldb; b.rows = N; b.K = K;
  if (!getenv("AOCR_NO_HH_NARROW") && !dma_disabled() && (M % 256 == 0 || (M >= 256 && !env_is_1("AOCR_HH_NARROW_FULL_ONLY"))) && N % 128 == 0 && K % 32 == 0 && cdiv(M, 256) * (N / 128) >= 200) { launch_dma_narrow(s, a, b, make_store(C, ldc, M, N, bias, bias2, flags), M, N, K); return; }
  if (dma128_eligible(M, N, K, 32)) { launch_dma128(s, a, b, make_store(C, ldc, M, N, bias, bias2, flags), M, N, K); return; }
  launch_lds(s, a, b, make_store(C, ldc, M, N, bias, bias2, flags), M, N, K, 1);
}

bool gemm_hh_cat(hipStream_t s, const bf16_t* A0, const bf16_t* A1, int64_t lda, const bf16_t* B0, const bf16_t* B1, int64_t ldb, float* C, int64_t ldc, int M, int N, int K0, int K1) {
  if (getenv("AOCR_NO_HH_NARROW") || env_is_1("AOCR_NO_HH_CAT") || dma_disabled() || (M % 256 && (M < 256 || env_is_1("AOCR_HH_NARROW_FULL_ONLY"))) || N % 128 || K0 % 32 || K1 % 32 || cdiv(M, 256) * (N / 128) < 200) return false;
  const TraceScope ts("gemm_hh_cat");
  LoadKhCat a; a.p0 = A0; a.p1 = A1; a.ld0 = a.ld1 = lda; a.rows = M; a.K0 = K0; a.K = K0 + K1;
  LoadKhCat b; b.p0 = B0; b.p1 = B1; b.ld0 = b.ld1 = ldb; b.rows = N; b.K0 = K0; b.K = K0 + K1;
  launch_dma_narrow(s, a, b, make_store(C, ldc, M, N, nullptr, nullptr, 0), M, N, K0 + K1);
  return true;
}

void gemm_hh_shadow(hipStream_t s, const bf16_t* A, int64_t lda, const bf16_t* B, int64_t ldb, float* C, int64_t ldc, bf16_t* Cb, int64_t ldcb,
                    int M, int N, int K) {
  const TraceScope ts("gemm_hh_shadow");
  LoadKh a; a.p = A; a.ld = lda; a.rows = M; a.K = K;
  LoadKh b; b.p = B; b.ld = ldb; b.rows = N; b.K = K;
  EpStore e = make_store(C, ldc, M, N, nullptr, nullptr, 0); e.Cb = Cb; e.ldcb = ldcb;
  if (!getenv("AOCR_NO_HH_NARROW") && !dma_disabled() && (M % 256 == 0 || (M >= 256 && !env_is_1("AOCR_HH_NARROW_FULL_ONLY"))) && N % 128 == 0 && K % 32 == 0 && cdiv(M, 256) * (N / 128) >= 200) {
    if (!env_is_1("AOCR_NO_NARROW_STAGED")) e.C = nullptr;
    launch_dma_narrow(s, a, b, e, M, N, K); return;
  }
  if (dma128_eligible(M, N, K, 32)) { launch_dma128(s, a, b, e, M, N, K); return; }
  launch_lds(s, a, b, e, M, N, K, 1);
}

template <class LD, class KERNEL>
static void grouped_launch(hipStream_t s, const WGradProblem* const* q, int cnt, int slots, bool shadows, KERNEL kernel) {
  int64_t tiles = 0;
  for (int i = 0; i < cnt; ++i) tiles += (int64_t)cdiv(q[i]->M, 128) * cdiv(q[i]->N, 128);
  int ks = (int)(slots / tiles); if (ks < 1) ks = 1;
  GroupArgs<LD, LD, EpStore> g; g.n = cnt; int first = 0;
  for (int i = 0; i < cnt; ++i) {
    auto& P = g.p[i];
    int ksplit = ks, kper; split_k(q[i]->K, 32, ksplit, kper);
    if constexpr (std::is_same<LD, LoadMNh>::value) {
      P.a.p = q[i]->Ab; P.a.ld = q[i]->lda; P.a.rows = q[i]->M; P.a.K = q[i]->K;
      P.b.p = q[i]->Bb; P.b.ld = q[i]->ldb; P.b.rows = q[i]->N; P.b.K = q[i]->K;
    } else {
      P.a = make_loadmn(q[i]->A, q[i]->lda, q[i]->M, q[i]->K); P.b = make_loadmn(q[i]->B, q[i]->ldb, q[i]->N, q[i]->K);
    }
    P.ep = make_store(q[i]->C, q[i]->ldc, q[i]->M, q[i]->N, nullptr, nullptr, ksplit > 1 ? EP_ATOMIC : EP_ACCUM);
    P.K = q[i]->K; P.kper = kper; P.gx = cdiv(q[i]->N, 128); P.ksplit = ksplit; P.first = first;
    first += cdiv(q[i]->M, 128) * P.gx * ksplit;
  }
  g.total = first; (void)shadows;
  for (int i = 0; i < cnt; ++i) trace_launch(shadows ? "wgrad_tr_grouped_kernel" : "gemm_lds_grouped_kernel", "", q[i]->M, q[i]->N, q[i]->K);
  hipLaunchKernelGGL(kernel, dim3(first), dim3(256), 0, s, g);
}

static int grouped_launch_dma(hipStream_t s, const WGradProblem* const* q, int cnt, float* part, size_t part_floats) {
  if (cnt <= 0 || !part) return 0;
  if (cnt > 8) cnt = 8;
  long long tiles = 0; int kmin = 1 << 30;
  for (int i = 0; i < cnt; ++i) { tiles += (long long)(q[i]->M / 256) * (q[i]->N / 256); kmin = std::min(kmin, q[i]->K); }
  const char* tg = getenv("AOCR_WGRAD_DMA_WGS");
  int ks = (int)((tg ? atoi(tg) : 256) / tiles); if (ks < 1) ks = 1;
  ks = std::min(ks, std::max(1, kmin / 768));
  while (ks > 1 && (size_t)tiles * 65536 * ks > part_floats) --ks;
  if ((size_t)tiles * 65536 * ks > part_floats) return 0;
  WgDmaArgs g; g.n = cnt; int first = 0; long long f4 = 0; size_t off = 0;
  for (int i = 0; i < cnt; ++i) {
    WgDmaProblem& P = g.p[i];
    int ksplit = ks, kper; split_k(q[i]->K, 32, ksplit, kper);
    P.A = q[i]->Ab; P.B = q[i]->Bb; P.lda = q[i]->lda; P.ldb = q[i]->ldb; P.M = q[i]->M; P.N = q[i]->N; P.K = q[i]->K;
    P.gx = q[i]->N / 256; P.tiles = (q[i]->M / 256) * P.gx; P.ks = ksplit; P.kper = kper; P.first = first; first += P.tiles * ksplit;
    P.part = part + off; off += (size_t)P.M * P.N * ksplit;
    P.C = q[i]->C; P.ldc = q[i]->ldc; P.f4first = f4; f4 += (long long)P.M * (P.N / 4);
  }
  g.total = first; g.f4total = f4;
  for (int i = 0; i < cnt; ++i) trace_launch("wgrad_dma_grouped_kernel", "slab_reduce", q[i]->M, q[i]->N, q[i]->K);
  hipLaunchKernelGGL((wgrad_dma_grouped_kernel<0>), dim3(first), dim3(512), 0, s, g, zero_page());
  hipLaunchKernelGGL((wgrad_slab_reduce_kernel<0>), dim3((unsigned)((f4 + 255) / 256)), dim3(256), 0, s, g);
  return cnt;
}
void grouped_wgrad(hipStream_t s, bool bf16, const WGradProblem* p, int n, float* part, size_t part_floats) {
  const TraceScope ts("grouped_wgrad");
  if (!bf16) {
    for (int i = 0; i < n; ++i)
      gemm(s, false, p[i].A, p[i].lda, false, p[i].B, p[i].ldb, false, p[i].C, p[i].ldc, p[i].M, p[i].N, p[i].K, nullptr, nullptr, EP_ATOMIC);
    return;
  }
  const WGradProblem* hs[16]; const WGradProblem* fs[16]; const WGradProblem* ds[16]; int nh = 0, nf = 0, nd = 0;
  const bool dma_ok = part && !dma_disabled() && !env_is_1("AOCR_NO_WGRAD_DMA_GROUPED");
  const char* dmk = getenv("AOCR_WGRAD_DMA_MINK"); const int dma_mink = dmk ? atoi(dmk) : 2048;
  for (int i = 0; i < n && i < 16; ++i) {
    const bool ok = p[i].Ab && p[i].Bb && p[i].M % 8 == 0 && p[i].N % 8 == 0 && p[i].lda % 8 == 0 && p[i].ldb % 8 == 0;
    const bool deep = ok && dma_ok && p[i].M % 256 == 0 && p[i].N % 256 == 0 && p[i].K % 32 == 0 && p[i].K >= dma_mink &&
                      ((reinterpret_cast<uintptr_t>(p[i].Ab) | reinterpret_cast<uintptr_t>(p[i].Bb)) & 15) == 0;
    if (deep && nd < 8) ds[nd++] = &p[i]; else if (ok) hs[nh++] = &p[i]; else fs[nf++] = &p[i];
  }
  if (nd > 0 && grouped_launch_dma(s, ds, nd, part, part_floats) != nd)
    for (int i = 0; i < nd; ++i) hs[nh++] = ds[i];
  for (int base = 0; base < nh; base += 8)
    grouped_launch<LoadMNh>(s, hs + base, std::min(8, nh - base), 1024, true, wgrad_tr_grouped_kernel<EpStore>);
  for (int base = 0; base < nf; base += 8)
    grouped_launch<LoadMN>(s, fs + base, std::min(8, nf - base), 768, false, gemm_lds_grouped_kernel<LoadMN, LoadMN, EpStore>);
}

static LoadConvK make_convk(const float* src, int B, int Hs, int Ws, int C, int ks, int sgn, int off, int Hr, int Wr, int pool) {
  LoadConvK a; a.src = src; a.H = Hs; a.W = Ws; a.C = C; a.KW = ks; a.sgn = sgn; a.off = off; a.Hr = Hr; a.Wr = Wr;
  a.pmode = pool; a.Hp = Hr / 2; a.Wp = Wr / 2;
  if (pool == 1) a.rows = B * a.Hp * a.Wp * 4; else if (pool == 2) a.rows = B * a.Hp * Wr * 2; else a.rows = B * Hr * Wr;
  a.K = ks * ks * C;
  return a;
}

void conv_forward(hipStream_t s, bool bf16, const float* x, const float* w, const float* bias, float* y, uint8_t* idx, int B,
                  int H, int W, int Cin, int Cout, int ks, int pad, int relu, int pool, const bf16_t* xb, const bf16_t* wb,
                  bf16_t* yb, int profile_tag, const float* bn_save, const float* bn_w, const float* bn_b, double* bn_part, int* bn_chunks, int* y_bf16) {
  const TraceScope ts("conv_forward");
  const int Ho = H + 2 * pad - ks + 1, Wo = W + 2 * pad - ks + 1;
  LoadConvK a = make_convk(x, B, H, W, Cin, ks, 1, -pad, Ho, Wo, pool);
  EpConv ep; ep.y = y; ep.idx = idx; ep.bias = bias; ep.Cout = Cout; ep.rows = a.rows; ep.pmode = pool; ep.relu = relu; ep.yb = yb;
  ep.bn_save = bn_save; ep.bn_w = bn_w; ep.bn_b = bn_b;
  if (bn_chunks) *bn_chunks = 0;
  if (y_bf16) *y_bf16 = 0;
  if (bf16 && xb && wb) {
    LoadConvKh ah; ah.src = xb; ah.g = a;
    LoadKh bh; bh.p = wb; bh.ld = a.K; bh.rows = Cout; bh.K = a.K;
    if (bn_part && bn_chunks && y && !yb && !bn_save && pool == 0 && dma_eligible(a.rows, Cout, a.K, Cin) && a.rows % 256 == 0 && a.rows / 256 <= 512 && !getenv("AOCR_NO_BN_STATS_FUSE")) {
      const char* const so = getenv("AOCR_HALO4_STAGED");
      const bool staged = ((so ? atoi(so) : 7) & 2) != 0;
      const bool halo = pad == 1 && halo_eligible(a, Cout, 256, 256);
      if (staged && !(halo && getenv("AOCR_HALO8"))) {
        ep.bn_part = bn_part; *bn_chunks = a.rows / 256;
        if (y_bf16 && getenv("AOCR_BN_Y16") && Cout % 4 == 0 && !getenv("AOCR_BN_PARTIAL_OLD")) {
          ep.y16 = reinterpret_cast<bf16_t*>(y); ep.y = nullptr; *y_bf16 = 1; }
      }
    }
    if (dma_eligible(a.rows, Cout, a.K, Cin) && pad == 1 && halo_eligible(a, Cout, 256, 256)) launch_halo<1, 256, 256>(s, ah, bh, ep, a.rows, Cout, profile_tag);
    else if (dma_eligible(a.rows, Cout, a.K, Cin)) launch_dma(s, ah, bh, ep, a.rows, Cout, a.K, profile_tag);
    else if (dma_narrow_eligible(a.rows, Cout, a.K, Cin) || dma_mid_eligible(a.rows, Cout, a.K, Cin)) launch_dma_narrow(s, ah, bh, ep, a.rows, Cout, a.K);
    else if (dma128_eligible(a.rows, Cout, a.K, Cin)) launch_dma128(s, ah, bh, ep, a.rows, Cout, a.K);
    else launch_lds(s, ah, bh, ep, a.rows, Cout, a.K, 1);
  } else {
    launch_conv_fwd(s, bf16, a, make_loadk(w, a.K, Cout, a.K), ep, a.rows, Cout, a.K);
  }
}

void conv_backward_data(hipStream_t s, bool bf16, const float* dy, const float* w, float* dx, int B, int H, int W, int Cin,
                        int Cout, int ks, int pad, const bf16_t* dyb, const bf16_t* wtb, const float* wtf, int* dx16, const BnBwdFuse* bnb, int* bnb_chunks) {
  const TraceScope ts("conv_backward_data");
  const int Ho = H + 2 * pad - ks + 1, Wo = W + 2 * pad - ks + 1;
  LoadConvK a = make_convk(dy, B, Ho, Wo, Cout, ks, -1, pad, H, W, 0);
  EpStore ep = make_store(dx, Cin, a.rows, Cin);
  if (dx16) *dx16 = 0;
  if (bnb_chunks) *bnb_chunks = 0;
  if (bf16 && dyb && wtb) {
    LoadConvKh ah; ah.src = dyb; ah.g = a;
    LoadKh bh; bh.p = wtb; bh.ld = a.K; bh.rows = Cin; bh.K = a.K;
    if (dx16 && dma_eligible(a.rows, Cin, a.K, Cout) && a.rows % 256 == 0 && Cin % 256 == 0 && env_is_1("AOCR_DX16") && !getenv("AOCR_BN_PARTIAL_OLD") && !getenv("AOCR_UNPOOL4")) {
      const char* const so = getenv("AOCR_HALO4_STAGED");
      const bool halo = pad == 1 && halo_eligible(a, Cin, 256, 256);
      if (((so ? atoi(so) : 7) & 1) && !(halo && getenv("AOCR_HALO8"))) { ep.C = nullptr; ep.Cb = reinterpret_cast<bf16_t*>(dx); ep.ldcb = Cin; *dx16 = 1; }
    }
    if (bnb && bnb_chunks && ep.C && dma_eligible(a.rows, Cin, a.K, Cout) && a.rows % 256 == 0 && Cin % 256 == 0 && a.rows / 256 <= 512 && env_is_1("AOCR_BNB_FUSE")) {
      const char* const so = getenv("AOCR_HALO4_STAGED");
      const bool halo = pad == 1 && halo_eligible(a, Cin, 256, 256);
      if (((so ? atoi(so) : 7) & 1) && !(halo && getenv("AOCR_HALO8"))) {
        ep.bnb_x = bnb->x; ep.bnb_yb = bnb->yb; ep.bnb_save = bnb->save; ep.bnb_part = bnb->part; *bnb_chunks = a.rows / 256;
      }
    }
    if (dma_eligible(a.rows, Cin, a.K, Cout) && pad == 1 && halo_eligible(a, Cin, 256, 256)) launch_halo<-1, 256, 256>(s, ah, bh, ep, a.rows, Cin);
    else if (dma_eligible(a.rows, Cin, a.K, Cout)) launch_dma(s, ah, bh, ep, a.rows, Cin, a.K);
    else if (dma_narrow_eligible(a.rows, Cin, a.K, Cout)) launch_dma_narrow(s, ah, bh, ep, a.rows, Cin, a.K);
    else if (dma128_eligible(a.rows, Cin, a.K, Cout)) launch_dma128(s, ah, bh, ep, a.rows, Cin, a.K);
    else launch_lds(s, ah, bh, ep, a.rows, Cin, a.K, 1);
  } else if (wtf) {
    launch_big(s, bf16, a, make_loadk(wtf, a.K, Cin, a.K), ep, a.rows, Cin, a.K, 1);
  } else {
    LoadConvWT b; b.w = w; b.Cin = Cin; b.Cout = Cout; b.KK = ks * ks; b.K = a.K;
    launch_conv_dgrad(s, bf16, a, b, ep, a.rows, Cin, a.K);
  }
}

void conv_backward_filter(hipStream_t s, bool bf16, const float* x, const float* dy, float* dw, float* dbias, int B, int H,
                          int W, int Cin, int Cout, int ks, int pad, const bf16_t* xb, const bf16_t* dyb, float* part, size_t part_floats, int profile_tag) {
  const TraceScope ts("conv_backward_filter");
  const int Ho = H + 2 * pad - ks + 1, Wo = W + 2 * pad - ks + 1;
  const int P = B * Ho * Wo, N = ks * ks * Cin;
  LoadConvXcol b; b.x = x; b.H = H; b.W = W; b.Cin = Cin; b.KW = ks; b.pad = pad; b.Ho = Ho; b.Wo = Wo; b.N = N; b.K = P;
  EpStore ep = make_store(dw, N, Cout, N, nullptr, nullptr, EP_ATOMIC);
  const int ksplit = pick_ksplit(Cout, N, P, bf16, (bf16 && xb && dyb) ? 1024 : 768);
  if (bf16 && xb && dyb) {
    LoadMNh ah; ah.p = dyb; ah.ld = Cout; ah.rows = Cout; ah.K = P;
    LoadConvXcolh bh; bh.x = xb; bh.g = b;
    const int tiles = cdiv(N, 256) * (Cout / 256);
    const int hmt = Cout % 256 == 0 ? 256 : 128;
    const int spr = (W + 31) / 32;
    const bool ragged_ok = W % 32 == 0 || (!env_is_0("AOCR_WGRAD_HALO_RAGGED") && W * 4 >= spr * 32 * 3);
    if (ks == 3 && pad == 1 && ragged_ok && Cout % hmt == 0 && Cin % 32 == 0 && part && !dma_disabled() && !env_is_1("AOCR_NO_WGRAD_HALO") && !getenv("AOCR_WGRAD_ATOMIC") &&
        (dma_forced() || (P >= 8192 && N >= wgrad_halo_min_n()))) {
      const int htiles = (Cin / 32) * (Cout / hmt), S = B * H * spr;
      int ksh = htiles >= 256 ? 1 : 256 / htiles; if (ksh > S) ksh = S;
      { const char* ms = getenv("AOCR_WGRAD_HALO_MINSTEPS"); const int minsteps = ms ? atoi(ms) : 0;
        if (minsteps > 0 && S / ksh < minsteps) ksh = std::max(1, S / minsteps); }
      const int per = cdiv(S, ksh); ksh = cdiv(S, per);
      const size_t mn = (size_t)Cout * N;
      if (mn * ksh <= part_floats) {
#define AOCR_WGH(TAGV, MGV, RGV, IMV, THREADS, MTV) hipLaunchKernelGGL((conv_wgrad_halo_kernel<TAGV, MGV, RGV, IMV>), dim3(htiles * ksh), dim3(THREADS), 0, s, dyb, xb, part, (long long)mn, B, H, W, Cin, Cout, Cin / 32, Cout / MTV, ksh, per, zero_page())
        const bool im = !env_is_1("AOCR_NO_WGRAD_ISSUE_MID");
        { char inst[48]; snprintf(inst, sizeof inst, "%d,%s,%s", hmt, W % 32 ? "ragged" : "whole", im ? "issue_mid" : "no_issue_mid");
          trace_launch("conv_wgrad_halo_kernel", inst, Cout, N, P); }
        if (W % 32) {
          if (hmt == 128) { if (im) AOCR_WGH(0, 2, true, true, 256, 128); else AOCR_WGH(0, 2, true, false, 256, 128); }
          else { if (im) AOCR_WGH(0, 4, true, true, 512, 256); else AOCR_WGH(0, 4, true, false, 512, 256); }
        }
        else if (hmt == 128) { if (im) AOCR_WGH(0, 2, false, true, 256, 128); else AOCR_WGH(0, 2, false, false, 256, 128); }
        else if (profile_tag) { if (im) AOCR_WGH(1, 4, false, true, 512, 256); else AOCR_WGH(1, 4, false, false, 512, 256); }
        else { if (im) AOCR_WGH(0, 4, false, true, 512, 256); else AOCR_WGH(0, 4, false, false, 512, 256); }
#undef AOCR_WGH
        splitk_reduce(s, part, ksh, mn, dw);
        if (dbias) colsum_accum(s, dy, Cout, P, Cout, dbias);
        return;
      }
    }
    if (Cout % 256 == 0 && Cin % 8 == 0 && !dma_disabled() && (dma_forced() || (P >= 8192 && tiles <= 256 && N % 256 == 0 && N >= 2304))) {
      int ks2 = tiles >= 128 ? (tiles >= 200 ? 1 : 2) : 256 / tiles, kper2; split_k(P, 32, ks2, kper2);
      const size_t mn = (size_t)Cout * N;
      float* const slab = (part && ks2 > 1 && mn * ks2 <= part_floats && !getenv("AOCR_WGRAD_ATOMIC")) ? part : nullptr;
      trace_launch("conv_wgrad_dma_kernel", slab ? "slab" : "atomic", Cout, N, P);
      if (profile_tag)
        hipLaunchKernelGGL((conv_wgrad_dma_kernel<EpStore, 256>), dim3(tiles * ks2), dim3(512), 0, s, ah, bh, ep, P, kper2, cdiv(N, 256), Cout / 256, zero_page(), ks2, slab, (long long)mn);
      else
        hipLaunchKernelGGL((conv_wgrad_dma_kernel<EpStore>), dim3(tiles * ks2), dim3(512), 0, s, ah, bh, ep, P, kper2, cdiv(N, 256), Cout / 256, zero_page(), ks2, slab, (long long)mn);
      if (slab) splitk_reduce(s, slab, ks2, mn, dw);
      if (dbias) colsum_accum(s, dy, Cout, P, Cout, dbias);
      return;
    }
    int ks = ksplit, kper; split_k(P, 32, ks, kper);
    const int gx = cdiv(N, 128), gy = cdiv(Cout, 128);
    const size_t mn = (size_t)Cout * N;
    float* const slab = (part && ks > 1 && mn * ks <= part_floats && !getenv("AOCR_WGRAD_ATOMIC")) ? part : nullptr;
    trace_launch("conv_wgrad_tr_kernel", slab ? "slab" : "atomic", Cout, N, P);
    hipLaunchKernelGGL((conv_wgrad_tr_kernel<EpStore>), dim3(gx * gy * ks), dim3(256), 0, s, ah, bh, ep, P, kper, gx, gy, ks, slab, (long long)mn);
    if (slab) splitk_reduce(s, slab, ks, mn, dw);
  } else {
    launch_conv_wgrad(s, bf16, make_loadmn(dy, Cout, Cout, P), b, ep, Cout, N, P, ksplit);
  }
  if (dbias) colsum_accum(s, dy, Cout, P, Cout, dbias);
}

}
```

Baseline: 54210 image-lines/s.

## Fuse max-unpool and ReLU backward into conv dgrad GEMM epilogue

Adds an EpUnpool epilogue for the data-gradient conv GEMMs. It applies the ReLU mask, scatters each value into the unpooled bf16 gradient map by the saved pool index, and writes per-tile column sums for the bias gradient. This removes the separate unpool_relu_backward kernel, along with the fp32 write and re-read of the intermediate dx, for conv layers 7, 5 and 3. It alternates the gradient map buffers and adds debug stop points, at the cost of more complex epilogues with scattered bf16 stores and new eligibility logic.

```diff
diff --git a/torch-attention-ocr_amd/csrc/capi.hip b/torch-attention-ocr_amd/csrc/capi.hip
--- a/torch-attention-ocr_amd/csrc/capi.hip
+++ b/torch-attention-ocr_amd/csrc/capi.hip
@@ -445,9 +445,10 @@
   else if (n == "dc_times") { REQUIRE(m->cl_err, "no cluster kernels in this configuration"); *ptr_dev = m->cl_err + 16 + 2048; *ndim = 1; shape[0] = 32 * 4 * 16 * 2; }
   else if (n == "g0") {
     const char* e = getenv("AOCR_DBG_STOP"); const int stop = e ? atoi(e) : 0;
-    const int64_t cnt = stop == 1 ? (int64_t)d.B * d.T * 512 : (int64_t)d.B * d.H4 * d.W2 * 512;
-    if (m->bf16) bf16_to_f32(m->s, m->G0b, m->G0, cnt);
-    *ptr_dev = m->G0; *ndim = 4; shape[0] = d.B; shape[1] = stop == 1 ? d.Ho7 : d.H4; shape[2] = stop == 1 ? d.Wo7 : d.W2; shape[3] = 512;
+    const int hh = stop == 1 ? d.Ho7 : stop == 3 ? d.H2 : stop == 4 ? d.H1 : d.H4, ww = stop == 1 ? d.Wo7 : stop == 4 ? d.W1 : d.W2, cc = stop == 3 ? 256 : stop == 4 ? 128 : 512;
+    const int64_t cnt = (int64_t)d.B * hh * ww * cc;
+    if (m->bf16) bf16_to_f32(m->s, m->dbg_map ? m->dbg_map : m->G0b, m->G0, cnt);
+    *ptr_dev = m->G0; *ndim = 4; shape[0] = d.B; shape[1] = hh; shape[2] = ww; shape[3] = cc;
   }
   else return fail("unknown tensor '%s'", name);
   return 0;
diff --git a/torch-attention-ocr_amd/csrc/epilogues.h b/torch-attention-ocr_amd/csrc/epilogues.h
--- a/torch-attention-ocr_amd/csrc/epilogues.h
+++ b/torch-attention-ocr_amd/csrc/epilogues.h
@@ -148,6 +148,131 @@
       }
     }
     __syncthreads();
+  }
+  return true;
+}
+
+struct EpUnpool {
+  bf16_t* dyb; const bf16_t* pooledb; const uint8_t* idx; float* part;
+  int M, N, Wp, pool;
+  __device__ __forceinline__ int64_t out_row(int row, int pos) const {
+    const int q = row / Wp, px = row - q * Wp;
+    return pool == 1 ? (int64_t)(2 * q + (pos >> 1)) * (2 * Wp) + 2 * px + (pos & 1) : (int64_t)(2 * q + pos) * Wp + px;
+  }
+  template <int NT> __device__ __forceinline__ void quad(int m, int n, int nstep, const float (&v)[NT][4]) const {
+    const int npos = pool == 1 ? 4 : 2;
+#pragma unroll
+    for (int ni = 0; ni < NT; ++ni) {
+      const int col = n + nstep * ni;
+      if (col >= N) continue;
+#pragma unroll
+      for (int i = 0; i < 4; ++i) {
+        const int row = m + i;
+        if (row >= M) continue;
+        const int64_t go = (int64_t)row * N + col;
+        const float g = (float)pooledb[go] > 0.f ? v[ni][i] + 0.f : 0.f;
+        const int sel = idx[go];
+        for (int pos = 0; pos < npos; ++pos) dyb[out_row(row, pos) * N + col] = (bf16_t)(sel == pos ? g : 0.f);
+      }
+    }
+  }
+};
+
+template <class EPT>
+__device__ __forceinline__ void unpool_piece8(const EPT& ep, const unsigned char* src32, int grow, int col, int npos, float (&ps)[8]) {
+  const int64_t go = (int64_t)grow * ep.N + col;
+  const bf16x8 pv = *reinterpret_cast<const bf16x8*>(ep.pooledb + go);
+  const uint2 ii = *reinterpret_cast<const uint2*>(ep.idx + go);
+  const float4 g0 = *reinterpret_cast<const float4*>(src32), g1 = *reinterpret_cast<const float4*>(src32 + 16);
+  const float g[8] = {g0.x, g0.y, g0.z, g0.w, g1.x, g1.y, g1.z, g1.w};
+  float gv[8]; int iv[8];
+#pragma unroll
+  for (int k = 0; k < 8; ++k) {
+    gv[k] = (float)pv[k] > 0.f ? g[k] : 0.f;
+    iv[k] = (int)(((k < 4 ? ii.x : ii.y) >> (8 * (k & 3))) & 255u);
+    ps[k] += gv[k];
+  }
+  for (int pos = 0; pos < npos; ++pos) {
+    bf16x8 hb;
+#pragma unroll
+    for (int k = 0; k < 8; ++k) hb[k] = (bf16_t)(iv[k] == pos ? gv[k] : 0.f);
+    *reinterpret_cast<bf16x8*>(ep.dyb + ep.out_row(grow, pos) * ep.N + col) = hb;
+  }
+}
+
+template <int NI, int NTH, class EPT>
+__device__ __forceinline__ void tile256_store_unpool(const EPT& ep, const f32x16 (&acc)[4][NI], unsigned char* lds, int m_blk, int n_blk, int wm, int wn, int r, int h, int tid) {
+  constexpr int PITCH = 1024;
+  const int c = tid & 31, npos = ep.pool == 1 ? 4 : 2;
+  float ps[8] = {0.f, 0.f, 0.f, 0.f, 0.f, 0.f, 0.f, 0.f};
+  __syncthreads();
+  for (int p = 0; p < 2; ++p) {
+    if (wm == p) {
+#pragma unroll
+      for (int mi = 0; mi < 4; ++mi)
+#pragma unroll
+        for (int ni = 0; ni < NI; ++ni)
+#pragma unroll
+          for (int q = 0; q < 4; ++q)
+#pragma unroll
+            for (int i = 0; i < 4; ++i)
+              *reinterpret_cast<float*>(lds + (mi * 32 + 8 * q + 4 * h + i) * PITCH + (wn * 32 * NI + ni * 32 + r) * 4) = acc[mi][ni][4 * q + i] + 0.f;
+    }
+    __syncthreads();
+#pragma unroll 2
+    for (int it = 0; it < 4096 / NTH; ++it) {
+      const int row = (it * NTH + tid) >> 5;
+      unpool_piece8(ep, lds + row * PITCH + c * 32, m_blk + p * 128 + row, n_blk + c * 8, npos, ps);
+    }
+    __syncthreads();
+  }
+  float* const red = reinterpret_cast<float*>(lds);
+#pragma unroll
+  for (int k = 0; k < 8; ++k) red[(tid >> 5) * 256 + c * 8 + k] = ps[k];
+  __syncthreads();
+  if (tid < 256) {
+    float s = 0.f;
+    for (int g = 0; g < NTH / 32; ++g) s += red[g * 256 + tid];
+    ep.part[(int64_t)(m_blk >> 8) * ep.N + n_blk + tid] = s;
+  }
+}
+
+template <int NT, class EPT>
+__device__ __forceinline__ bool narrow_store_unpool(const EPT& ep, const f32x16 (&acc)[2][NT], unsigned char* lds, int m_blk, int n_blk, int wm, int wn, int r, int h, int tid) {
+  constexpr int BN = 64 * NT, PITCH = BN * 4, CPR = BN / 8;
+  if (n_blk + BN > ep.N) return false;
+  const int c = tid % CPR, npos = ep.pool == 1 ? 4 : 2;
+  float ps[8] = {0.f, 0.f, 0.f, 0.f, 0.f, 0.f, 0.f, 0.f};
+  __syncthreads();
+  for (int p = 0; p < 2; ++p) {
+    if ((wm >> 1) == p) {
+#pragma unroll
+      for (int mi = 0; mi < 2; ++mi)
+#pragma unroll
+        for (int ni = 0; ni < NT; ++ni)
+#pragma unroll
+          for (int q = 0; q < 4; ++q)
+#pragma unroll
+            for (int i = 0; i < 4; ++i)
+              *reinterpret_cast<float*>(lds + ((wm & 1) * 64 + mi * 32 + 8 * q + 4 * h + i) * PITCH + (wn * 32 * NT + ni * 32 + r) * 4) = acc[mi][ni][4 * q + i] + 0.f;
+    }
+    __syncthreads();
+    const int row_base = m_blk + p * 128;
+#pragma unroll 2
+    for (int it = 0; it < (128 * CPR) / 512; ++it) {
+      const int row = (it * 512 + tid) / CPR;
+      if (row_base + row < ep.M) unpool_piece8(ep, lds + row * PITCH + c * 32, row_base + row, n_blk + c * 8, npos, ps);
+    }
+    __syncthreads();
+  }
+  float* const red = reinterpret_cast<float*>(lds);
+#pragma unroll
+  for (int k = 0; k < 8; ++k) red[(tid / CPR) * BN + c * 8 + k] = ps[k];
+  __syncthreads();
+  if (tid < BN) {
+    float s = 0.f;
+    for (int g = 0; g < 512 / CPR; ++g) s += red[g * BN + tid];
+    ep.part[(int64_t)(m_blk >> 8) * ep.N + n_blk + tid] = s;
   }
   return true;
 }
diff --git a/torch-attention-ocr_amd/csrc/mfma_gemm.h b/torch-attention-ocr_amd/csrc/mfma_gemm.h
--- a/torch-attention-ocr_amd/csrc/mfma_gemm.h
+++ b/torch-attention-ocr_amd/csrc/mfma_gemm.h
@@ -952,7 +952,7 @@
   lds_tile<BK>(a, b, ep, (bid / gx) * 128, (bid % gx) * 128, kbeg, min(K, kbeg + kper), lds);
 }
 
-struct EpConv; struct EpStore;
+struct EpConv; struct EpStore; struct EpUnpool;
 template <int NI, int NTH>
 __device__ __forceinline__ void tile256_store_f32(float* dst, int64_t ldc, const float* bias, bool relu, const f32x16 (&acc)[4][NI], unsigned char* lds,
                                                   int m_blk, int n_blk, int wm, int wn, int r, int h, int tid, double* part = nullptr, int C = 0, const float* bias2 = nullptr,
@@ -1115,6 +1115,8 @@
     }
   }
 }
+template <int NI, int NTH, class EPT>
+__device__ __forceinline__ void tile256_store_unpool(const EPT& ep, const f32x16 (&acc)[4][NI], unsigned char* lds, int m_blk, int n_blk, int wm, int wn, int r, int h, int tid);
 template <int NI, int NTH, class EP>
 __device__ __forceinline__ bool tile256_store_staged(const EP& ep, const f32x16 (&acc)[4][NI], unsigned char* lds, int m_blk, int n_blk, int wm, int wn, int r, int h, int tid, int opt) {
   if constexpr (std::is_same<EP, EpConv>::value) {
@@ -1133,11 +1135,17 @@
     if (ep.bnb_part) tile256_store_f32<NI, NTH>(ep.C, ep.ldc, nullptr, false, acc, lds, m_blk, n_blk, wm, wn, r, h, tid, ep.bnb_part, ep.N, nullptr, ep.bnb_x, ep.bnb_yb, ep.bnb_save);
     else tile256_store_f32<NI, NTH>(ep.C, ep.ldc, nullptr, false, acc, lds, m_blk, n_blk, wm, wn, r, h, tid);
     return true;
+  } else if constexpr (std::is_same<EP, EpUnpool>::value) {
+    if (!(opt & 1) || m_blk + 256 > ep.M || n_blk + 256 > ep.N) return false;
+    tile256_store_unpool<NI, NTH, EP>(ep, acc, lds, m_blk, n_blk, wm, wn, r, h, tid);
+    return true;
   } else return false;
 }
 
 template <int NT, class EPT>
 __device__ __forceinline__ bool narrow_store_staged(const EPT& ep, const f32x16 (&acc)[2][NT], unsigned char* lds, int m_blk, int n_blk, int wm, int wn, int r, int h, int tid);
+template <int NT, class EPT>
+__device__ __forceinline__ bool narrow_store_unpool(const EPT& ep, const f32x16 (&acc)[2][NT], unsigned char* lds, int m_blk, int n_blk, int wm, int wn, int r, int h, int tid);
 
 __device__ __forceinline__ void dma16(const void* g, unsigned char* l) {
   __builtin_amdgcn_global_load_lds((const __attribute__((address_space(1))) void*)g, (__attribute__((address_space(3))) void*)l, 16, 0, 0);
@@ -1719,6 +1727,8 @@
   asm volatile("s_waitcnt vmcnt(0)" ::: "memory");
   if constexpr (std::is_same<EP, EpStore>::value) {
     if (staged && narrow_store_staged<NT, EP>(ep, acc, lds, m_blk, n_blk, wm, wn, r, h, tid)) return;
+  } else if constexpr (std::is_same<EP, EpUnpool>::value) {
+    if (staged && narrow_store_unpool<NT, EP>(ep, acc, lds, m_blk, n_blk, wm, wn, r, h, tid)) return;
   }
   const int m0 = m_blk + wm * 64, n0 = n_blk + wn * 32 * NT;
 #pragma unroll
diff --git a/torch-attention-ocr_amd/csrc/model.h b/torch-attention-ocr_amd/csrc/model.h
--- a/torch-attention-ocr_amd/csrc/model.h
+++ b/torch-attention-ocr_amd/csrc/model.h
@@ -62,6 +62,7 @@
   uint16_t* route1 = nullptr; bool route1_valid = false;
   float *G0, *G1, *dX; size_t gmax = 0;
   aocr::bf16_t *A1b, *A2b, *A3b, *A4b, *A5b, *A6b, *G0b, *G2b = nullptr;
+  const aocr::bf16_t* dbg_map = nullptr;
   hipEvent_t cw_map[2] = {nullptr, nullptr}, cw_done[2] = {nullptr, nullptr}, cw_main = nullptr;
   aocr::bf16_t *wb[8], *wtb[8];
   float* wtf[8];
diff --git a/torch-attention-ocr_amd/csrc/model.hip b/torch-attention-ocr_amd/csrc/model.hip
--- a/torch-attention-ocr_amd/csrc/model.hip
+++ b/torch-attention-ocr_amd/csrc/model.hip
@@ -363,10 +363,18 @@
   const bool ws = !stop && cnn_wgrad_on_side(m);
   hipStream_t sw = ws ? m->side : s;
   const bool wg_after = ws && env_on("AOCR_CNN_WGRAD_AFTER_DGRAD");
-  if (!ws) Gb[1] = Gb[0];
+  const bool fz = bf && m->G2b && !wg_after;
+  const UnpoolFuse u6{1, m->A6b, m->idx6, d.H4, d.W2, 2, nullptr, m->conv[6].db, nullptr, nullptr};
+  const UnpoolFuse u4{2, m->A4b, m->idx4, d.H2, d.W2, 2, nullptr, m->conv[4].db, nullptr, nullptr};
+  const UnpoolFuse u2{4, m->A2b, m->idx2, d.H1, d.W1, 1, nullptr, m->conv[2].db, nullptr, nullptr};
+  auto fusable = [&](UnpoolFuse u, int H, int W, int Cin, int Cout, int ks, int pad) { u.partial = G0; return fz && conv_dgrad_unpool_ok(u, B, H, W, Cin, Cout, ks, pad); };
+  const bool f6 = fusable(u6, d.H6, d.W2, 512, 512, 2, 0), f4 = fusable(u4, d.H4, d.W2, 256, 512, 3, 1), f2 = fusable(u2, d.H2, d.W2, 128, 256, 3, 1);
+  const bool alt = ws || f6 || f4 || f2;
+  if (!alt) Gb[1] = Gb[0];
+  m->dbg_map = nullptr;
   auto map_ready = [&]() { if (ws) { hipEventRecord(m->cw_map[gp], s); hipStreamWaitEvent(sw, m->cw_map[gp], 0); } };
   auto wgrad_done = [&]() { if (ws) hipEventRecord(m->cw_done[gp], sw); };
-  auto next_map = [&]() { if (ws) { gp ^= 1; hipStreamWaitEvent(s, m->cw_done[gp], 0); } };
+  auto next_map = [&]() { if (alt) gp ^= 1; if (ws) hipStreamWaitEvent(s, m->cw_done[gp], 0); };
   int bnbc = 0;
   int g16 = 0; const bf16_t* const G1h = reinterpret_cast<const bf16_t*>(G1);
   constexpr size_t SLAB = (size_t)4 << 20;
@@ -375,12 +383,14 @@
   auto slab = [&](int k) { return defer ? G0 + (size_t)k * SLAB : G0; };
   prof_mark(m, AOCR_PROF_BN); bn_relu_backward(s, m->Y7, m->X, m->dX, m->bn[7].w, m->bn[7].save, bf ? nullptr : G0, m->bn[7].dw, m->bn[7].db, m->bn_scratch,
                    (int64_t)B * d.T, 512, B, Gb[gp], bf ? m->Xb : nullptr, bf ? m->conv[7].db : nullptr, bf ? slab(0) : nullptr, bsync, defer);
-  if (stop == 1) { if (defer) colsum_flush(s, cj); return; }
+  if (stop == 1) { m->dbg_map = Gb[gp]; if (defer) colsum_flush(s, cj); return; }
   { auto W = [&]() { prof_mark(m, AOCR_PROF_CONV_WGRAD); conv_backward_filter(sw, bf, m->A6, G0, m->conv[7].dw, bf ? nullptr : m->conv[7].db, B, d.H6, d.W2, 512, 512, 2, 0, m->A6b, Gb[gp], m->wg_part, m->wg_part_floats); };
     auto D = [&]() { prof_mark(m, AOCR_PROF_CONV_DGRAD); conv_backward_data(s, bf, G0, m->conv[7].w, G1, B, d.H6, d.W2, 512, 512, 2, 0, Gb[gp], m->wtb[7], m->wtf[7], bf ? &g16 : nullptr); };
-    if (wg_after) { D(); map_ready(); W(); wgrad_done(); } else { map_ready(); W(); wgrad_done(); D(); } }
-  next_map(); prof_mark(m, AOCR_PROF_POOL_CONV1); unpool_relu_backward(s, G1, m->A6, m->idx6, bf ? nullptr : G0, B, d.H4, d.W2, 512, 2, Gb[gp], bf ? m->conv[6].db : nullptr, bf ? slab(1) : nullptr, bf ? m->A6b : nullptr, defer, g16 ? G1h : nullptr);
-  if (stop == 2) { if (defer) colsum_flush(s, cj); return; }
+    if (f6) { map_ready(); W(); wgrad_done(); const bf16_t* const src = Gb[gp]; next_map(); UnpoolFuse u = u6; u.dyb = Gb[gp]; u.partial = slab(1); u.defer = defer; g16 = 0;
+              prof_mark(m, AOCR_PROF_CONV_DGRAD); conv_backward_data(s, bf, G0, m->conv[7].w, G1, B, d.H6, d.W2, 512, 512, 2, 0, src, m->wtb[7], m->wtf[7], nullptr, nullptr, nullptr, &u); }
+    else if (wg_after) { D(); map_ready(); W(); wgrad_done(); } else { map_ready(); W(); wgrad_done(); D(); } }
+  if (!f6) { next_map(); prof_mark(m, AOCR_PROF_POOL_CONV1); unpool_relu_backward(s, G1, m->A6, m->idx6, bf ? nullptr : G0, B, d.H4, d.W2, 512, 2, Gb[gp], bf ? m->conv[6].db : nullptr, bf ? slab(1) : nullptr, bf ? m->A6b : nullptr, defer, g16 ? G1h : nullptr); }
+  if (stop == 2) { m->dbg_map = Gb[gp]; if (defer) colsum_flush(s, cj); return; }
   { auto W = [&]() { prof_mark(m, AOCR_PROF_CONV_WGRAD); conv_backward_filter(sw, bf, m->A5, G0, m->conv[6].dw, bf ? nullptr : m->conv[6].db, B, d.H4, d.W2, 512, 512, 3, 1, m->A5b, Gb[gp], m->wg_part, m->wg_part_floats); };
     auto D = [&]() { prof_mark(m, AOCR_PROF_CONV_DGRAD); { const BnBwdFuse bf5{m->Y5, m->A5b, m->bn[5].save, (double*)m->bn_scratch}; conv_backward_data(s, bf, G0, m->conv[6].w, G1, B, d.H4, d.W2, 512, 512, 3, 1, Gb[gp], m->wtb[6], m->wtf[6], bf ? &g16 : nullptr, (bf && !m->y16[1]) ? &bf5 : nullptr, &bnbc); } };
     if (wg_after) { D(); map_ready(); W(); wgrad_done(); } else { map_ready(); W(); wgrad_done(); D(); } }
@@ -392,8 +402,11 @@
   if (defer) colsum_flush(s, cj);
   if (ws) { hipEventRecord(m->cw_main, s); hipStreamWaitEvent(sw, m->cw_main, 0); hipEventRecord(m->grad_ev[2], sw); }
   else hipEventRecord(m->grad_ev[2], s);
-    if (!wg_after) D(); }
-  next_map(); prof_mark(m, AOCR_PROF_POOL_CONV1); unpool_relu_backward(s, G1, m->A4, m->idx4, bf ? nullptr : G0, B, d.H2, d.W2, 256, 2, Gb[gp], bf ? m->conv[4].db : nullptr, bf ? slab(3) : nullptr, bf ? m->A4b : nullptr, defer, g16 ? G1h : nullptr);
+    if (f4) { const bf16_t* const src = Gb[gp]; next_map(); UnpoolFuse u = u4; u.dyb = Gb[gp]; u.partial = slab(3); u.defer = defer; g16 = 0;
+              prof_mark(m, AOCR_PROF_CONV_DGRAD); conv_backward_data(s, bf, G0, m->conv[5].w, G1, B, d.H4, d.W2, 256, 512, 3, 1, src, m->wtb[5], m->wtf[5], nullptr, nullptr, nullptr, &u); }
+    else if (!wg_after) D(); }
+  if (!f4) { next_map(); prof_mark(m, AOCR_PROF_POOL_CONV1); unpool_relu_backward(s, G1, m->A4, m->idx4, bf ? nullptr : G0, B, d.H2, d.W2, 256, 2, Gb[gp], bf ? m->conv[4].db : nullptr, bf ? slab(3) : nullptr, bf ? m->A4b : nullptr, defer, g16 ? G1h : nullptr); }
+  if (stop == 3) { m->dbg_map = Gb[gp]; if (defer) colsum_flush(s, cj); return; }
   { auto W = [&]() { prof_mark(m, AOCR_PROF_CONV_WGRAD); conv_backward_filter(sw, bf, m->A3, G0, m->conv[4].dw, bf ? nullptr : m->conv[4].db, B, d.H2, d.W2, 256, 256, 3, 1, m->A3b, Gb[gp], m->wg_part, m->wg_part_floats); };
     auto D = [&]() { prof_mark(m, AOCR_PROF_CONV_DGRAD); { const BnBwdFuse bf3{m->Y3, m->A3b, m->bn[3].save, (double*)m->bn_scratch}; conv_backward_data(s, bf, G0, m->conv[4].w, G1, B, d.H2, d.W2, 256, 256, 3, 1, Gb[gp], m->wtb[4], m->wtf[4], bf ? &g16 : nullptr, (bf && !m->y16[0]) ? &bf3 : nullptr, &bnbc); } };
     if (wg_after) { D(); map_ready(); W(); wgrad_done(); } else { map_ready(); W(); wgrad_done(); D(); } }
@@ -401,8 +414,11 @@
                    (int64_t)B * d.H2 * d.W2, 256, 0, Gb[gp], bf ? m->A3b : nullptr, bf ? m->conv[3].db : nullptr, bf ? slab(4) : nullptr, bsync, defer, m->y16[0] ? reinterpret_cast<const bf16_t*>(m->Y3) : nullptr, g16 ? G1h : nullptr, bnbc); bnbc = 0;
   { auto W = [&]() { prof_mark(m, AOCR_PROF_CONV_WGRAD); conv_backward_filter(sw, bf, m->A2, G0, m->conv[3].dw, bf ? nullptr : m->conv[3].db, B, d.H2, d.W2, 128, 256, 3, 1, m->A2b, Gb[gp], m->wg_part, m->wg_part_floats); };
     auto D = [&]() { prof_mark(m, AOCR_PROF_CONV_DGRAD); conv_backward_data(s, bf, G0, m->conv[3].w, G1, B, d.H2, d.W2, 128, 256, 3, 1, Gb[gp], m->wtb[3], m->wtf[3]); };
-    if (wg_after) { D(); map_ready(); W(); wgrad_done(); } else { map_ready(); W(); wgrad_done(); D(); } }
-  next_map(); prof_mark(m, AOCR_PROF_POOL_CONV1); unpool_relu_backward(s, G1, m->A2, m->idx2, bf ? nullptr : G0, B, d.H1, d.W1, 128, 1, Gb[gp], bf ? m->conv[2].db : nullptr, bf ? slab(5) : nullptr, bf ? m->A2b : nullptr, defer);
+    if (f2) { map_ready(); W(); wgrad_done(); const bf16_t* const src = Gb[gp]; next_map(); UnpoolFuse u = u2; u.dyb = Gb[gp]; u.partial = slab(5); u.defer = defer;
+              prof_mark(m, AOCR_PROF_CONV_DGRAD); conv_backward_data(s, bf, G0, m->conv[3].w, G1, B, d.H2, d.W2, 128, 256, 3, 1, src, m->wtb[3], m->wtf[3], nullptr, nullptr, nullptr, &u); }
+    else if (wg_after) { D(); map_ready(); W(); wgrad_done(); } else { map_ready(); W(); wgrad_done(); D(); } }
+  if (!f2) { next_map(); prof_mark(m, AOCR_PROF_POOL_CONV1); unpool_relu_backward(s, G1, m->A2, m->idx2, bf ? nullptr : G0, B, d.H1, d.W1, 128, 1, Gb[gp], bf ? m->conv[2].db : nullptr, bf ? slab(5) : nullptr, bf ? m->A2b : nullptr, defer); }
+  if (stop == 4) { m->dbg_map = Gb[gp]; if (defer) colsum_flush(s, cj); return; }
   { auto W = [&]() { prof_mark(m, AOCR_PROF_CONV_WGRAD); conv_backward_filter(sw, bf, m->A1, G0, m->conv[2].dw, bf ? nullptr : m->conv[2].db, B, d.H1, d.W1, 64, 128, 3, 1, m->A1b, Gb[gp], m->wg_part, m->wg_part_floats); };
     auto D = [&]() { prof_mark(m, AOCR_PROF_CONV_DGRAD); conv_backward_data(s, bf, G0, m->conv[2].w, G1, B, d.H1, d.W1, 64, 128, 3, 1, Gb[gp], m->wtb[2], m->wtf[2]); };
     if (wg_after) { D(); map_ready(); W(); wgrad_done(); } else { map_ready(); W(); wgrad_done(); D(); } }
diff --git a/torch-attention-ocr_amd/csrc/ops.h b/torch-attention-ocr_amd/csrc/ops.h
--- a/torch-attention-ocr_amd/csrc/ops.h
+++ b/torch-attention-ocr_amd/csrc/ops.h
@@ -95,10 +95,14 @@
                   double* bn_part = nullptr, int* bn_chunks = nullptr, int* y_bf16 = nullptr);
 void bn_eval_prepare(hipStream_t s, const float* rm, const float* rv, float* save, int C);
 struct BnBwdFuse { const float* x; const bf16_t* yb; const float* save; double* part; };
+struct ColsumJobs;
+struct UnpoolFuse { int layer; const bf16_t* pooledb; const uint8_t* idx; int Ho, Wo, pool; bf16_t* dyb; float* dbias; float* partial; ColsumJobs* defer; };
+bool conv_dgrad_unpool_ok(const UnpoolFuse& u, int B, int H, int W, int Cin, int Cout, int ks, int pad);
 void conv_backward_data(hipStream_t s, bool bf16, const float* dy, const float* w, float* dx, int B, int H, int W, int Cin,
                         int Cout, int ks, int pad, const bf16_t* dyb = nullptr, const bf16_t* wtb = nullptr, const float* wtf = nullptr,
                         int* dx16 = nullptr ,
-                        const struct BnBwdFuse* bnb = nullptr, int* bnb_chunks = nullptr );
+                        const struct BnBwdFuse* bnb = nullptr, int* bnb_chunks = nullptr ,
+                        const UnpoolFuse* up = nullptr );
 void conv_backward_filter(hipStream_t s, bool bf16, const float* x, const float* dy, float* dw, float* dbias, int B, int H,
                           int W, int Cin, int Cout, int ks, int pad, const bf16_t* xb = nullptr, const bf16_t* dyb = nullptr,
                           float* part = nullptr, size_t part_floats = 0, int profile_tag = 0);
diff --git a/torch-attention-ocr_amd/csrc/ops_gemm.hip b/torch-attention-ocr_amd/csrc/ops_gemm.hip
--- a/torch-attention-ocr_amd/csrc/ops_gemm.hip
+++ b/torch-attention-ocr_amd/csrc/ops_gemm.hip
@@ -705,14 +705,53 @@
   }
 }
 
+static int unpool_fuse_mask() {
+  if (env_is_1("AOCR_NO_UNPOOL_FUSE")) return 0;
+  const char* const e = getenv("AOCR_UNPOOL_FUSE");
+  return e ? atoi(e) : 7;
+}
+bool conv_dgrad_unpool_ok(const UnpoolFuse& u, int B, int H, int W, int Cin, int Cout, int ks, int pad) {
+  if (!(unpool_fuse_mask() & u.layer) || !u.pooledb || !u.idx || !u.dbias || !u.partial) return false;
+  if (env_is_1("AOCR_DX16") || getenv("AOCR_UNPOOL4")) return false;
+  if ((u.Ho & 1) || u.Ho / 2 != H || (u.pool == 1 ? ((u.Wo & 1) || u.Wo / 2 != W) : (u.pool != 2 || u.Wo != W))) return false;
+  if (Cin % 8) return false;
+  const int Ho = H + 2 * pad - ks + 1, Wo = W + 2 * pad - ks + 1;
+  const LoadConvK a = make_convk(nullptr, B, Ho, Wo, Cout, ks, -1, pad, H, W, 0);
+  if (cdiv(a.rows, 256) > 2048) return false;
+  if (dma_eligible(a.rows, Cin, a.K, Cout)) {
+    const char* const so = getenv("AOCR_HALO4_STAGED");
+    const bool halo = pad == 1 && halo_eligible(a, Cin, 256, 256);
+    return a.rows % 256 == 0 && Cin % 256 == 0 && ((so ? atoi(so) : 7) & 1) && !(halo && getenv("AOCR_HALO8"));
+  }
+  if (dma_narrow_eligible(a.rows, Cin, a.K, Cout)) return !env_is_1("AOCR_NO_NARROW_STAGED");
+  return false;
+}
+
 void conv_backward_data(hipStream_t s, bool bf16, const float* dy, const float* w, float* dx, int B, int H, int W, int Cin,
-                        int Cout, int ks, int pad, const bf16_t* dyb, const bf16_t* wtb, const float* wtf, int* dx16, const BnBwdFuse* bnb, int* bnb_chunks) {
+                        int Cout, int ks, int pad, const bf16_t* dyb, const bf16_t* wtb, const float* wtf, int* dx16, const BnBwdFuse* bnb, int* bnb_chunks, const UnpoolFuse* up) {
   const TraceScope ts("conv_backward_data");
   const int Ho = H + 2 * pad - ks + 1, Wo = W + 2 * pad - ks + 1;
   LoadConvK a = make_convk(dy, B, Ho, Wo, Cout, ks, -1, pad, H, W, 0);
   EpStore ep = make_store(dx, Cin, a.rows, Cin);
   if (dx16) *dx16 = 0;
   if (bnb_chunks) *bnb_chunks = 0;
+  if (up && bf16 && dyb && wtb && !dx16 && !bnb && up->dyb && up->dyb != dyb && conv_dgrad_unpool_ok(*up, B, H, W, Cin, Cout, ks, pad)) {
+    LoadConvKh ah; ah.src = dyb; ah.g = a;
+    LoadKh bh; bh.p = wtb; bh.ld = a.K; bh.rows = Cin; bh.K = a.K;
+    EpUnpool eu; eu.dyb = up->dyb; eu.pooledb = up->pooledb; eu.idx = up->idx; eu.part = up->partial; eu.M = a.rows; eu.N = Cin; eu.Wp = W; eu.pool = up->pool;
+    trace_launch("unpool_epilogue", up->pool == 1 ? "2x2" : "2x1", a.rows, Cin, a.K);
+    if (dma_eligible(a.rows, Cin, a.K, Cout) && pad == 1 && halo_eligible(a, Cin, 256, 256)) launch_halo<-1, 256, 256>(s, ah, bh, eu, a.rows, Cin);
+    else if (dma_eligible(a.rows, Cin, a.K, Cout)) launch_dma(s, ah, bh, eu, a.rows, Cin, a.K);
+    else launch_dma_narrow(s, ah, bh, eu, a.rows, Cin, a.K);
+    const int tiles = cdiv(a.rows, 256);
+    if (up->defer) colsum_defer(*up->defer, up->partial, Cin, tiles, Cin, up->dbias); else colsum_accum(s, up->partial, Cin, tiles, Cin, up->dbias);
+    return;
+  }
+  if (up) {
+    conv_backward_data(s, bf16, dy, w, dx, B, H, W, Cin, Cout, ks, pad, dyb, wtb, wtf, dx16, bnb, bnb_chunks, nullptr);
+    unpool_relu_backward(s, dx, nullptr, up->idx, nullptr, B, up->Ho, up->Wo, Cin, up->pool, up->dyb, up->dbias, up->partial, up->pooledb, up->defer, (dx16 && *dx16) ? reinterpret_cast<const bf16_t*>(dx) : nullptr);
+    return;
+  }
   if (bf16 && dyb && wtb) {
     LoadConvKh ah; ah.src = dyb; ah.g = a;
     LoadKh bh; bh.p = wtb; bh.ld = a.K; bh.rows = Cin; bh.K = a.K;
```

Result: no change. 54400 image-lines/s, median of 6 (+0.3%).
